# paninski-lab/deepgraphpose

Hardware: AMD Instinct MI355X
Metric: frames_per_sec (higher is better)
Workload: dtype f32

## Files before the change

deepgraphpose_amd/_lib.py:

```python
from __future__ import annotations

import ctypes as C
import os

_HERE = os.path.dirname(os.path.abspath(__file__))
LIB_PATH = os.environ.get("DGP_HIP_LIB") or os.path.join(_HERE, "libdgp_hip.so")


class DgpNetDesc(C.Structure):
    _fields_ = [("depth", C.c_int32), ("num_joints", C.c_int32), ("in_h", C.c_int32), ("in_w", C.c_int32),
                ("max_batch", C.c_int32), ("with_locref", C.c_int32), ("mean_pixel", C.c_float * 3),
                ("bn_eps", C.c_float)]


class DgpTensorView(C.Structure):
    _fields_ = [("name", C.c_char_p), ("data", C.POINTER(C.c_float)), ("ndim", C.c_int32),
                ("shape", C.c_int64 * 4)]


class DgpLossDesc(C.Structure):
    _fields_ = [(n, C.c_int32) for n in ("nt", "H", "W", "nj", "nl", "n_visible", "n_hidden", "gm2", "gm3",
                                          "gauss_len", "huber")] + \
               [(n, C.c_float) for n in ("gamma", "lengthscale", "stride", "wn_visible", "wn_hidden",
                                         "locref_loss_weight", "n_frames_total", "n_visible_frames_total")] + \
               [(n, C.c_int32) for n in ("use_wt", "Hin", "Win")] + [("wt_max", C.c_float)]


class DgpFlowParams(C.Structure):
    _fields_ = [("pyr_scale", C.c_double), ("levels", C.c_int32), ("winsize", C.c_int32), ("iterations", C.c_int32),
                ("poly_n", C.c_int32), ("poly_sigma", C.c_double), ("flags", C.c_int32)]


class DgpConvDesc(C.Structure):
    _fields_ = [(n, C.c_int32) for n in (
        "N", "H", "W", "Cin", "Cout", "KH", "KW", "stride", "rate", "pad_t", "pad_l", "Ho", "Wo", "relu",
        "res_stride", "res_H", "res_W")]


_vp, _i32, _f32, _sz = C.c_void_p, C.c_int32, C.c_float, C.c_size_t
SYMBOLS = {
    "dgp_version": (C.c_int, []),
    "dgp_tuning_build": (C.c_int, []),
    "dgp_crc32c": (C.c_uint32, [C.c_void_p, C.c_size_t, C.c_uint32]),
    "dgp_last_error": (C.c_char_p, []),
    "dgp_net_create": (C.c_int, [C.POINTER(DgpNetDesc), C.POINTER(_vp)]),
    "dgp_net_destroy": (None, [_vp]),
    "dgp_net_set_input_size": (C.c_int, [_vp, _i32, _i32]),
    "dgp_dlc_loss_fwd_bwd": (C.c_int, [_vp, _vp, _vp, _vp, _vp, _vp, _i32, _i32, _i32, _i32, C.c_float, _i32, _vp, _vp, _vp,
                                       _vp, _sz, _vp]),
    "dgp_net_load_weights": (C.c_int, [_vp, C.POINTER(DgpTensorView), _i32]),
    "dgp_net_workspace_bytes": (C.c_int, [_vp, _i32, C.POINTER(_sz)]),
    "dgp_net_output_dims": (C.c_int, [_vp] + [C.POINTER(_i32)] * 4),
    "dgp_net_stats": (C.c_int, [_vp, _i32, C.POINTER(_i32), C.POINTER(C.c_double)]),
    "dgp_forward": (C.c_int, [_vp, _vp, _i32, _vp, _sz, _vp, _vp, _vp, _vp]),
    "dgp_soft_argmax": (C.c_int, [_vp, _i32, _i32, _i32, _i32, _f32, _i32, _vp, _vp, _vp, _vp, _vp]),
    "dgp_soft_argmax_locref": (C.c_int, [_vp, _vp, _i32, _i32, _i32, _i32, _f32, _i32, _vp, _vp, _vp, _vp, _vp, _vp]),
    "dgp_hard_argmax": (C.c_int, [_vp, _vp, _i32, _i32, _i32, _i32, _vp, _vp, _vp, _vp]),
    "dgp_pmap_threshold": (C.c_int, [_vp, _i32, _i32, _i32, _i32, _f32, _vp, _vp]),
    "dgp_infer": (C.c_int, [_vp, _vp, _i32, _vp, _sz, _f32, _i32, _vp, _vp, _vp, _vp, _vp]),
    "dgp_infer_packed": (C.c_int, [_vp, _vp, _i32, _vp, _sz, _f32, _i32, _vp, _vp, _vp]),
    "dgp_infer_packed_locref": (C.c_int, [_vp, _vp, _i32, _vp, _sz, _f32, _i32, _i32, _vp, _vp, _vp, _vp]),
    "dgp_net_profile_begin": (C.c_int, [_vp, _i32]),
    "dgp_net_profile_end": (C.c_int, [_vp, C.POINTER(_i32), C.POINTER(_i32)]),
    "dgp_net_profile_launch": (C.c_int, [_vp, _i32, C.c_char_p, _i32, C.POINTER(C.c_double), C.POINTER(C.c_double)]),
    "dgp_loss_scratch_bytes": (C.c_int, [C.POINTER(DgpLossDesc), C.POINTER(_sz)]),
    "dgp_loss_fwd_bwd": (C.c_int, [C.POINTER(DgpLossDesc)] + [_vp] * 18 + [_sz, _vp]),
    "dgp_trainer_create": (C.c_int, [_vp, C.POINTER(_vp)]),
    "dgp_trainer_destroy": (None, [_vp]),
    "dgp_trainer_num_tensors": (C.c_int, [_vp, C.POINTER(_i32), C.POINTER(C.c_int64), C.POINTER(C.c_int64)]),
    "dgp_trainer_tensor_info": (C.c_int, [_vp, _i32, C.c_char_p, _i32, C.POINTER(C.c_int64), C.POINTER(C.c_int64),
                                          C.POINTER(_i32)]),
    "dgp_trainer_buffer": (_vp, [_vp, _i32]),
    "dgp_trainer_upload": (C.c_int, [_vp, _i32, C.c_int64, _vp, C.c_int64]),
    "dgp_trainer_download": (C.c_int, [_vp, _i32, C.c_int64, _vp, C.c_int64]),
    "dgp_trainer_workspace_bytes": (C.c_int, [_vp, _i32, C.POINTER(_sz)]),
    "dgp_trainer_sync_weights": (C.c_int, [_vp, _vp]),
    "dgp_train_forward": (C.c_int, [_vp, _vp, _i32, _vp, _sz, C.POINTER(_vp), C.POINTER(_vp), _vp]),
    "dgp_train_backward": (C.c_int, [_vp, _i32, _vp, _sz, _vp, _vp, _vp]),
    "dgp_sgd_momentum_clip": (C.c_int, [_vp, _f32, _f32, _f32, C.POINTER(_f32), _vp]),
    "dgp_adam_clip": (C.c_int, [_vp, _f32, _f32, _f32, _f32, _f32, C.POINTER(_f32), _vp]),
    "dgp_packed_weight_floats": (_sz, [_i32, _i32, _i32, _i32]),
    "dgp_pack_conv_weights": (C.c_int, [_vp, _i32, _i32, _i32, _i32, _vp]),
    "dgp_conv2d": (C.c_int, [C.POINTER(DgpConvDesc), _vp, _vp, _vp, _vp, _vp, _vp, _vp]),
    "dgp_conv2d_ranged": (C.c_int, [C.POINTER(DgpConvDesc), _vp, _vp, _vp, _vp, _vp, _vp, _vp, _vp, _vp, _vp]),
    "dgp_tensor_absmax": (C.c_int, [_vp, _sz, _vp, _vp]),
    "dgp_f32_to_h2": (C.c_int, [_vp, _sz, _i32, _vp, _vp]),
    "dgp_h2_to_f32": (C.c_int, [_vp, _sz, _i32, _vp, _vp]),
    "dgp_conv2d_h2": (C.c_int, [C.POINTER(DgpConvDesc), _vp, _i32, _vp, _vp, _vp, _vp, _vp, _i32, _i32, _vp, _i32, _i32, _vp, _vp, _vp]),
    "dgp_net_set_tier": (C.c_int, [_vp, _i32]),
    "dgp_net_get_tier": (C.c_int, [_vp]),
    "dgp_f32_to_h1": (C.c_int, [_vp, _sz, _i32, _vp, _vp]),
    "dgp_h1_to_f32": (C.c_int, [_vp, _sz, _i32, _vp, _vp]),
    "dgp_conv2d_h1": (C.c_int, [C.POINTER(DgpConvDesc), _vp, _i32, _vp, _vp, _vp, _vp, _vp, _i32, _vp, _i32, _i32, _vp, _vp, _vp]),
    "dgp_chain_h2": (C.c_int, [_i32] * 9 + [_vp, _i32, _vp, _i32] + [_vp] * 6 + [_vp, _i32, _vp, _i32, _vp, _vp, _vp]),
    "dgp_unit_h2": (C.c_int, [_i32] * 7 + [_vp, _i32, _vp, _i32] + [_vp] * 3 + [_i32] + [_vp] * 6 + [_vp, _i32, _vp, _i32, _vp, _vp, _vp, _vp]),
    "dgp_chain_h1": (C.c_int, [_i32] * 9 + [_vp, _i32, _vp, _i32] + [_vp] * 6 + [_vp, _i32, _vp, _i32, _vp, _vp, _vp]),
    "dgp_unit_h1": (C.c_int, [_i32] * 7 + [_vp, _i32, _vp, _i32] + [_vp] * 3 + [_i32] + [_vp] * 6 + [_vp, _i32, _vp, _i32, _vp, _vp, _vp, _vp]),
    "dgp_net_range_status": (C.c_int, [_vp, C.POINTER(_i32), C.POINTER(_i32), _vp]),
    "dgp_net_recalibrate": (C.c_int, [_vp]),
    "dgp_net_reset_scales": (C.c_int, [_vp]),
    "dgp_net_copy_scales": (C.c_int, [_vp, _vp, _vp]),
    "dgp_net_widen": (C.c_int, [_vp]),
    "dgp_conv2d_wgrad": (C.c_int, [C.POINTER(DgpConvDesc), _vp, _vp, _vp, _vp, _vp, _vp, _vp]),
    "dgp_conv2d_wgrad_shadow": (C.c_int, [C.POINTER(DgpConvDesc), _vp, _vp, _vp, _vp, _vp, _vp, _vp, _vp, _vp, _vp]),
    "dgp_trainer_set_tier": (C.c_int, [_vp, C.c_int32]),
    "dgp_trainer_get_tier": (C.c_int, [_vp]),
    "dgp_trainer_grad_groups": (C.c_int, [_vp, C.c_int32, C.POINTER(C.c_int32), C.POINTER(C.c_int64), C.POINTER(C.c_int64)]),
    "dgp_trainer_grad_group_wait": (C.c_int, [_vp, C.c_int32, _vp]),
    "dgp_trainer_step_status": (C.c_int, [_vp, _vp, C.c_int32, C.POINTER(C.c_float), C.POINTER(C.c_float), C.POINTER(C.c_int32),
                                               C.POINTER(C.c_int32), _vp]),
    "dgp_trainer_fast_mode": (C.c_int, [_vp, C.c_int32]),
    "dgp_trainer_fast_status": (C.c_int, [_vp, C.POINTER(C.c_int32), C.POINTER(C.c_int32)]),
    "dgp_conv2d_dgrad_scratch_bytes": (_sz, [C.POINTER(DgpConvDesc)]),
    "dgp_conv2d_dgrad": (C.c_int, [C.POINTER(DgpConvDesc), _vp, _vp, _vp, _vp, _vp, _i32, _vp, _vp, _i32, _vp]),
    "dgp_motion_energy": (C.c_int, [_vp, C.c_int64, C.c_int32, _vp, _vp, _vp]),
    "dgp_maxpool_3x3s2_same": (C.c_int, [_vp, _i32, _i32, _i32, _i32, _vp, _vp]),
    "dgp_preprocess_u8": (C.c_int, [_vp, C.c_int64, C.POINTER(_f32), _vp, _vp]),
    "dgp_optical_flow_scratch_bytes": (C.c_int, [_i32, _i32, _i32, C.POINTER(DgpFlowParams), C.POINTER(_sz), C.POINTER(_i32)]),
    "dgp_optical_flow": (C.c_int, [_vp, _i32, _i32, _i32, C.POINTER(DgpFlowParams), _vp, _vp, _vp, _sz, _vp]),
    "dgp_resize_plan_size": (C.c_int, [_i32, _i32, C.POINTER(_i32)]),
    "dgp_resize_plan": (C.c_int, [_i32, _i32, _vp, _vp]),
    "dgp_resize_crop_u8": (C.c_int, [_vp, _i32, _i32, _i32, _i32, _i32, C.POINTER(_i32), _vp, _vp, _vp, _i32, _i32, _vp]),
    "dgp_resize_plan_size_f": (C.c_int, [_i32, _i32, _i32, C.POINTER(_i32)]),
    "dgp_resize_plan_f": (C.c_int, [_i32, _i32, _i32, _vp, _vp]),
    "dgp_window_resize_u8": (C.c_int, [_vp, _i32, _i32, _i32, _i32, _i32, _i32, _i32, _i32, _i32, _i32, _vp, _vp, _vp, _i32, _i32, _vp]),
    "dgp_target_maps": (C.c_int, [_vp, _vp, _vp, _vp, _i32, _i32, _i32, _i32, C.c_double, C.c_double, C.c_double, C.c_double, _i32,
                                  _vp, _vp, _vp, _vp, _vp]),
    "dgp_gather_frames_u8": (C.c_int, [_vp, C.c_int64, C.c_int64, _vp, _i32, _vp, _i32, C.c_int64, _vp, _vp]),
    "dgp_aug_affine_u8": (C.c_int, [_vp, _vp, _i32, _i32, C.POINTER(C.c_double), _vp]),
    "dgp_aug_blur3_u8": (C.c_int, [_vp, _vp, _i32, _i32, C.POINTER(_f32), _vp]),
    "dgp_aug_dropout_u8": (C.c_int, [_vp, _vp, _i32, _i32, _vp, _i32, _i32, _vp]),
    "dgp_aug_elastic_u8": (C.c_int, [_vp, _vp, _i32, _i32, _vp, _i32, _i32, _vp]),
    "dgp_aug_noise_u8": (C.c_int, [_vp, _vp, _i32, _i32, _f32, _i32, C.c_uint64, _vp]),
}

_lib = None


class DgpError(RuntimeError):
    pass


def load():
    global _lib
    if _lib is not None:
        return _lib
    if not os.path.exists(LIB_PATH):
        raise DgpError(
            "libdgp_hip.so not found at %s -- build it with `python -m deepgraphpose_amd.build` "
            "(hipcc --offload-arch=gfx950); deepgraphpose_amd has no CPU fallback" % LIB_PATH)
    try:
        import torch
    except ImportError:
        pass
    lib = C.CDLL(LIB_PATH)
    for name, (res, args) in SYMBOLS.items():
        fn = getattr(lib, name)
        fn.restype = res
        fn.argtypes = args
    _lib = lib
    return lib


def check(rc: int, what: str = ""):
    if rc != 0:
        msg = load().dgp_last_error()
        raise DgpError("%s failed (%d): %s" % (what or "dgp call", rc, (msg or b"").decode()))
```

deepgraphpose_amd/arch.py:

```python
from __future__ import annotations

import math
from dataclasses import dataclass
from typing import List, Tuple

BLOCKS = {
    50: [(64, 3, 2), (128, 4, 2), (256, 6, 2), (512, 3, 1)],
    101: [(64, 3, 2), (128, 4, 2), (256, 23, 2), (512, 3, 1)],
    152: [(64, 3, 2), (128, 8, 2), (256, 36, 2), (512, 3, 1)],
}

MEAN_PIXEL = (123.68, 116.779, 103.939)
BN_EPS = 1e-5


@dataclass
class UnitPlan:
    scope: str
    depth_in: int
    depth: int
    depth_bottleneck: int
    stride: int
    rate: int
    has_shortcut_conv: bool


def resnet_units(depth: int = 50, output_stride: int = 16) -> List[UnitPlan]:
    if depth not in BLOCKS:
        raise ValueError("unsupported resnet depth %r" % (depth,))
    name = "resnet_v1_%d" % depth
    target = output_stride // 4
    current_stride, rate = 1, 1
    units: List[UnitPlan] = []
    depth_in = 64
    for bi, (base, n_units, block_stride) in enumerate(BLOCKS[depth], start=1):
        for ui in range(1, n_units + 1):
            s = block_stride if ui == n_units else 1
            d_out = base * 4
            if current_stride == target:
                unit_stride, unit_rate = 1, rate
                rate *= s
            else:
                unit_stride, unit_rate = s, 1
                current_stride *= s
            units.append(UnitPlan(
                scope="%s/block%d/unit_%d/bottleneck_v1" % (name, bi, ui),
                depth_in=depth_in, depth=d_out, depth_bottleneck=base,
                stride=unit_stride, rate=unit_rate,
                has_shortcut_conv=(depth_in != d_out)))
            depth_in = d_out
    return units


def same_out(n: int, s: int) -> int:
    return -(-n // s)


def feature_hw(h: int, w: int, depth: int = 50) -> Tuple[int, int]:
    for _ in range(4):
        h, w = same_out(h, 2), same_out(w, 2)
    return h, w


def scoremap_hw(h: int, w: int, deconv_stride: int = 2) -> Tuple[int, int]:
    fh, fw = feature_hw(h, w)
    return fh * deconv_stride, fw * deconv_stride


def conv_macs_per_frame(h: int, w: int, depth: int = 50, nj: int = 4,
                        with_locref: bool = False) -> int:
    h1, w1 = same_out(h, 2), same_out(w, 2)
    macs = h1 * w1 * 7 * 7 * 3 * 64
    hh, ww = same_out(h1, 2), same_out(w1, 2)
    for u in resnet_units(depth):
        ho, wo = same_out(hh, u.stride), same_out(ww, u.stride)
        if u.has_shortcut_conv:
            macs += ho * wo * u.depth_in * u.depth
        macs += hh * ww * u.depth_in * u.depth_bottleneck
        macs += ho * wo * 9 * u.depth_bottleneck * u.depth_bottleneck
        macs += ho * wo * u.depth_bottleneck * u.depth
        hh, ww = ho, wo
    heads = nj * (3 if with_locref else 1)
    macs += hh * ww * 9 * 2048 * heads
    return macs


def launch_algorithmic_bytes(name: str, h: int, w: int, depth: int = 50, batch: int = 1, elem_bytes: float = 4.0) -> float:
    body = name.split("|")[0]
    if not body.startswith("conv:"):
        return 0.0
    if body.endswith("/conv1+pool"):
        h1, w1 = same_out(h, 2), same_out(w, 2)
        return float(batch * h * w * 3 + elem_bytes * batch * same_out(h1, 2) * same_out(w1, 2) * 64 + 4 * 7 * 7 * 3 * 64)
    toks = body[5:].split("+")
    units = {u.scope: (i, u) for i, u in enumerate(resnet_units(depth))}
    plan = resnet_units(depth)
    h1, w1 = same_out(h, 2), same_out(w, 2)
    hh, ww = same_out(h1, 2), same_out(w1, 2)
    geo = []
    for u in plan:
        ho, wo = same_out(hh, u.stride), same_out(ww, u.stride)
        geo.append((batch * hh * ww, batch * ho * wo))
        hh, ww = ho, wo
    convs = []
    for t in toks:
        if t == "shortcut":
            convs.append((convs[-1][0], "shortcut"))
            continue
        scope, _, which = t.rpartition("/")
        if scope not in units:
            return 0.0
        convs.append((units[scope][0], which))
    have = set(convs)
    total = 0.0
    for ui, which in convs:
        u = plan[ui]
        pin, pout = geo[ui]
        if which == "conv1":
            total += u.depth_in * u.depth_bottleneck
            total += pin * u.depth_bottleneck
            if (ui - 1, "conv3") not in have:
                total += pin * u.depth_in
        elif which == "conv2":
            total += 9 * u.depth_bottleneck * u.depth_bottleneck
            total += pin * u.depth_bottleneck
            if (ui, "conv3") not in have:
                total += pout * u.depth_bottleneck
        elif which == "conv3":
            total += u.depth_bottleneck * u.depth + pout * u.depth
            if (ui, "conv2") not in have:
                total += pout * u.depth_bottleneck
            if (ui, "shortcut") in have:
                total += pin * u.depth_in
            elif u.has_shortcut_conv:
                total += pout * u.depth
            else:
                total += (pin if u.stride == 1 else pout) * u.depth
        elif which == "shortcut":
            total += u.depth_in * u.depth
            if (ui, "conv3") not in have:
                total += pin * u.depth_in + pout * u.depth
    return elem_bytes * total


def conv_algorithmic_bytes(h: int, w: int, depth: int = 50, batch: int = 1) -> dict:
    name = "resnet_v1_%d" % depth
    out = {}
    h1, w1 = same_out(h, 2), same_out(w, 2)
    out["conv:%s/conv1" % name] = 4.0 * (batch * h * w * 4 + batch * h1 * w1 * 64 + 7 * 7 * 4 * 64)
    hh, ww = same_out(h1, 2), same_out(w1, 2)
    for u in resnet_units(depth):
        ho, wo = same_out(hh, u.stride), same_out(ww, u.stride)
        pin, pout = batch * hh * ww, batch * ho * wo
        if u.has_shortcut_conv:
            out["conv:%s/shortcut" % u.scope] = 4.0 * (pin * u.depth_in + pout * u.depth + u.depth_in * u.depth)
        out["conv:%s/conv1" % u.scope] = 4.0 * (pin * u.depth_in + pin * u.depth_bottleneck + u.depth_in * u.depth_bottleneck)
        out["conv:%s/conv2" % u.scope] = 4.0 * (pin * u.depth_bottleneck + pout * u.depth_bottleneck +
                                                9 * u.depth_bottleneck * u.depth_bottleneck)
        res = pout * u.depth if u.has_shortcut_conv else (pin if u.stride == 1 else pout) * u.depth
        out["conv:%s/conv3" % u.scope] = 4.0 * (pout * u.depth_bottleneck + pout * u.depth + res + u.depth_bottleneck * u.depth)
        hh, ww = ho, wo
    return out
```

deepgraphpose_amd/csrc/dgp_chain.hip:

```cpp
#include "dgp_internal.h"
#include "dgp_device.h"

#include <cstdio>
#include <cstdlib>
#include <type_traits>

namespace dgp {

typedef float floatx4 __attribute__((ext_vector_type(4)));
typedef __attribute__((address_space(3))) void lds_void;

__device__ __forceinline__ floatx4 mma16(const uint4& a, const uint4& b, floatx4 c) {
    return __builtin_amdgcn_mfma_f32_16x16x32_f16(__builtin_bit_cast(half8, a), __builtin_bit_cast(half8, b), c, 0, 0, 0);
}
__device__ __forceinline__ uint4 ld16nt(__amdgpu_buffer_rsrc_t r, unsigned voff, int soff) {
    return __builtin_bit_cast(uint4, __builtin_amdgcn_raw_buffer_load_b128(r, (int)voff, soff, 2));
}
__device__ __forceinline__ void st16nt(__amdgpu_buffer_rsrc_t r, const uint4& v, unsigned voff, int soff) {
    __builtin_amdgcn_raw_buffer_store_b128(__builtin_bit_cast(u32x4, v), r, (int)voff, soff, 2);
}
__device__ __forceinline__ uint4 ld16(__amdgpu_buffer_rsrc_t r, unsigned voff, int soff) {
    return __builtin_bit_cast(uint4, __builtin_amdgcn_raw_buffer_load_b128(r, (int)voff, soff, 0));
}
__device__ __forceinline__ void st16(__amdgpu_buffer_rsrc_t r, const uint4& v, unsigned voff, int soff) {
    __builtin_amdgcn_raw_buffer_store_b128(__builtin_bit_cast(u32x4, v), r, (int)voff, soff, 0);
}

#ifdef DGP_DIAG
__device__ unsigned long long g_unit_diag[16];
#define UD_STAMP(x)                                                                     \
    do {                                                                                \
        __builtin_amdgcn_sched_barrier(0);                                              \
        asm volatile("s_memtime %0\n\ts_waitcnt lgkmcnt(0)" : "=s"(x)::"memory");       \
        __builtin_amdgcn_sched_barrier(0);                                              \
    } while (0)
#define UD_PARAM , unsigned long long (&ud)[12]
#define UD_ARG , ud
#else
#define UD_STAMP(x)
#define UD_PARAM
#define UD_ARG
#endif

template <int RES, int RB, bool H1 = false>
__device__ __forceinline__ void chain_fetch_res(const ChainArgs& p, uint4 (&res)[RB][2], const unsigned (&roff)[RB],
                                                const __amdgpu_buffer_rsrc_t rs_s2, int jp) {
    if constexpr (RES != 0) {
#pragma unroll
        for (int rb = 0; rb < RB; ++rb) {
            if constexpr (H1) {
                res[rb][0] = (p.nt & 1) ? ld16nt(rs_s2, roff[rb], jp * 64) : ld16(rs_s2, roff[rb], jp * 64);
            } else if (p.nt & 1) {
                res[rb][0] = ld16nt(rs_s2, roff[rb], jp * 128);
                res[rb][1] = ld16nt(rs_s2, roff[rb], jp * 128 + 16);
            } else {
                res[rb][0] = ld16(rs_s2, roff[rb], jp * 128);
                res[rb][1] = ld16(rs_s2, roff[rb], jp * 128 + 16);
            }
        }
    }
}
template <int RES, int RB, int PD, bool H1 = false>
__device__ __forceinline__ void chain_prefetch(const ChainArgs& p, uint4 (&res)[PD][RB][2], const unsigned (&roff)[RB],
                                               const __amdgpu_buffer_rsrc_t rs_s2) {
#pragma unroll
    for (int u = 0; u < PD - 1; ++u) chain_fetch_res<RES, RB, H1>(p, res[u], roff, rs_s2, u);
}

template <int C, int C1, int CIN2, int RES, int RB, int NS, int PD, int CHUNK, int WR, bool H1 = false>
__device__ __forceinline__ void chain_tail(const ChainArgs& p, const uint4* ring, int& slot, const uint4 (&ph)[RB][(C + CIN2) / 32],
                                           const uint4 (&pl)[RB][(C + CIN2) / 32], const unsigned (&xoff)[RB], const unsigned (&roff)[RB],
                                           const unsigned (&r1off)[RB], const __amdgpu_buffer_rsrc_t rs_s2, const __amdgpu_buffer_rsrc_t rs_xo,
                                           const __amdgpu_buffer_rsrc_t rs_r1, float& amax_x, float& amax_r1, const int lane,
                                           uint4 (&res)[PD][RB][2] UD_PARAM) {
#ifdef DGP_DIAG
    unsigned long long c0 = 0, c1 = 0, c2 = 0, c3 = 0, c4 = 0;
#endif
    constexpr int C4 = 4 * C, KS1 = (C + CIN2) / 32, NJP = C4 / 32, NCB = C1 / 16;
    constexpr int PL = H1 ? 1 : 2;
    constexpr int F1 = KS1 * 2 * PL, F2 = NCB * PL;
    static_assert(WR >= 2 && WR % 2 == 0, "weight fragments in flight: pairs share the ring");
    static_assert(NJP % PD == 0 && PD >= 2, "chunk loop is unrolled PD times");
    const int g = lane >> 4;
    floatx4 a2[RB][NCB];
#pragma unroll
    for (int rb = 0; rb < RB; ++rb)
#pragma unroll
        for (int cb = 0; cb < NCB; ++cb) a2[rb][cb] = floatx4{0.f, 0.f, 0.f, 0.f};
    auto fetch_res = [&](int jp, int buf) { chain_fetch_res<RES, RB, H1>(p, res[buf], roff, rs_s2, jp); };
    constexpr int CB = H1 ? 64 : 128;
    for (int jp0 = 0; jp0 < NJP; jp0 += PD) {
#pragma unroll
        for (int u = 0; u < PD; ++u) {
            const int jp = jp0 + u;
            if (jp + PD - 1 < NJP) fetch_res(jp + PD - 1, (u + PD - 1) % PD);
            UD_STAMP(c0);
            const uint4* Wc = ring + slot * (CHUNK / 16);
            const uint4* W = Wc + lane;
            floatx4 a1[RB][2];
#pragma unroll
            for (int rb = 0; rb < RB; ++rb) { a1[rb][0] = floatx4{0.f, 0.f, 0.f, 0.f}; a1[rb][1] = floatx4{0.f, 0.f, 0.f, 0.f}; }
            uint4 wq[WR];
#pragma unroll
            for (int f = 0; f < WR && f < F1 + F2; ++f) wq[f] = W[f * 64];
            __builtin_amdgcn_sched_barrier(0);
#pragma unroll
            for (int s = 0; s < KS1; ++s)
#pragma unroll
                for (int b = 0; b < 2; ++b) {
                    const int f0 = (s * 2 + b) * PL;
                    const uint4 wh = wq[f0 % WR], wl = wq[(f0 + PL - 1) % WR];
                    if constexpr (!H1) {
#pragma unroll
                    for (int rb = 0; rb < RB; ++rb) a1[rb][b] = mma16(wl, ph[rb][s], a1[rb][b]);
#pragma unroll
                    for (int rb = 0; rb < RB; ++rb) a1[rb][b] = mma16(wh, pl[rb][s], a1[rb][b]);
                    }
#pragma unroll
                    for (int rb = 0; rb < RB; ++rb) a1[rb][b] = mma16(wh, ph[rb][s], a1[rb][b]);
                    __builtin_amdgcn_sched_barrier(0);
                    if (f0 + WR < F1 + F2) wq[f0 % WR] = W[(f0 + WR) * 64];
                    if (PL == 2 && f0 + 1 + WR < F1 + F2) wq[(f0 + 1) % WR] = W[(f0 + 1 + WR) * 64];
                    __builtin_amdgcn_sched_barrier(0);
                }
            UD_STAMP(c1);
            const float4 sa = __builtin_bit_cast(float4, Wc[(F1 + F2) * 64 + 2 * g]), sb = __builtin_bit_cast(float4, Wc[(F1 + F2) * 64 + 2 * g + 1]);
            const float4 ba = __builtin_bit_cast(float4, Wc[(F1 + F2) * 64 + 8 + 2 * g]), bb = __builtin_bit_cast(float4, Wc[(F1 + F2) * 64 + 8 + 2 * g + 1]);
            const float sc[8] = {sa.x * p.post1, sa.y * p.post1, sa.z * p.post1, sa.w * p.post1,
                                 sb.x * p.post1, sb.y * p.post1, sb.z * p.post1, sb.w * p.post1};
            const float bi[8] = {ba.x, ba.y, ba.z, ba.w, bb.x, bb.y, bb.z, bb.w};
            uint4 xh[RB], xl[RB];
#pragma unroll
            for (int rb = 0; rb < RB; ++rb) {
                float o[8], r[8] = {0.f, 0.f, 0.f, 0.f, 0.f, 0.f, 0.f, 0.f};
                if constexpr (RES != 0) {
                    if constexpr (H1) h1_unpack8(res[u][rb][0], p.res_inv_scale, r);
                    else h2_unpack8(res[u][rb][0], res[u][rb][1], p.res_inv_scale, r);
                }
#pragma unroll
                for (int k = 0; k < 8; ++k) {
                    o[k] = a1[rb][k >> 2][k & 3] * sc[k] + bi[k] + r[k];
                    o[k] = fmaxf(o[k], 0.f);
                }
                if constexpr (H1) { xh[rb] = h1_pack8(o, p.xout_scale); xl[rb] = xh[rb]; }
                else h2_pack8(o, p.xout_scale, xh[rb], xl[rb]);
                if (p.nt & 2) {
                    st16nt(rs_xo, xh[rb], xoff[rb], jp * CB);
                    if constexpr (!H1) st16nt(rs_xo, xl[rb], xoff[rb], jp * CB + 16);
                } else {
                    st16(rs_xo, xh[rb], xoff[rb], jp * CB);
                    if constexpr (!H1) st16(rs_xo, xl[rb], xoff[rb], jp * CB + 16);
                }
                if (xoff[rb] != OOB) {
#pragma unroll
                    for (int k = 0; k < 8; ++k) amax_x = fmaxf(amax_x, o[k]);
                }
            }
            UD_STAMP(c2);
            __builtin_amdgcn_sched_barrier(0);
#pragma unroll
            for (int cb = 0; cb < NCB; ++cb) {
                const int f0 = F1 + cb * PL;
                const uint4 wh = wq[f0 % WR], wl = wq[(f0 + PL - 1) % WR];
                if constexpr (!H1) {
#pragma unroll
                for (int rb = 0; rb < RB; ++rb) a2[rb][cb] = mma16(wl, xh[rb], a2[rb][cb]);
#pragma unroll
                for (int rb = 0; rb < RB; ++rb) a2[rb][cb] = mma16(wh, xl[rb], a2[rb][cb]);
                }
#pragma unroll
                for (int rb = 0; rb < RB; ++rb) a2[rb][cb] = mma16(wh, xh[rb], a2[rb][cb]);
                __builtin_amdgcn_sched_barrier(0);
                if (f0 + WR < F1 + F2) wq[f0 % WR] = W[(f0 + WR) * 64];
                if (PL == 2 && f0 + 1 + WR < F1 + F2) wq[(f0 + 1) % WR] = W[(f0 + 1 + WR) * 64];
                __builtin_amdgcn_sched_barrier(0);
            }
            slot = slot + 1 == NS ? 0 : slot + 1;
            UD_STAMP(c3);
            asm volatile("s_waitcnt lgkmcnt(0)" ::: "memory");
            __builtin_amdgcn_s_barrier();
            UD_STAMP(c4);
#ifdef DGP_DIAG
            ud[4] += c1 - c0; ud[5] += c2 - c1; ud[6] += c3 - c2; ud[7] += c4 - c3;
#endif
        }
    }
    UD_STAMP(c0);
#pragma unroll
    for (int q = 0; q < NCB / 2; ++q) {
        const float4 s0 = *reinterpret_cast<const float4*>(p.sc1 + 32 * q + 8 * g), s1 = *reinterpret_cast<const float4*>(p.sc1 + 32 * q + 8 * g + 4);
        const float4 b0 = *reinterpret_cast<const float4*>(p.bi1 + 32 * q + 8 * g), b1 = *reinterpret_cast<const float4*>(p.bi1 + 32 * q + 8 * g + 4);
        const float sc[8] = {s0.x * p.post2, s0.y * p.post2, s0.z * p.post2, s0.w * p.post2,
                             s1.x * p.post2, s1.y * p.post2, s1.z * p.post2, s1.w * p.post2};
        const float bi[8] = {b0.x, b0.y, b0.z, b0.w, b1.x, b1.y, b1.z, b1.w};
#pragma unroll
        for (int rb = 0; rb < RB; ++rb) {
            float o[8];
#pragma unroll
            for (int k = 0; k < 8; ++k) o[k] = fmaxf(a2[rb][2 * q + (k >> 2)][k & 3] * sc[k] + bi[k], 0.f);
            if constexpr (H1) {
                st16(rs_r1, h1_pack8(o, p.r1_scale), r1off[rb], q * CB);
            } else {
            uint4 hi, lo;
            h2_pack8(o, p.r1_scale, hi, lo);
            st16(rs_r1, hi, r1off[rb], q * 128);
            st16(rs_r1, lo, r1off[rb], q * 128 + 16);
            }
            if (r1off[rb] != OOB) {
#pragma unroll
                for (int k = 0; k < 8; ++k) amax_r1 = fmaxf(amax_r1, o[k]);
            }
        }
    }
    UD_STAMP(c1);
#ifdef DGP_DIAG
    ud[8] += c1 - c0;
#endif
}

template <int C, int C1, int CIN2, int RES, int RB, int NCW, int NLW, int NS, int PD, int WR, bool H1 = false>
__global__ __launch_bounds__(64 * (NCW + NLW)) void chain_kernel(const ChainArgs p) {
    constexpr int C4 = 4 * C;
    constexpr int EB = H1 ? 2 : 4;
    constexpr int KSA = C / 32, KSB = CIN2 / 32, KS1 = KSA + KSB;
    constexpr int NJP = C4 / 32;
    constexpr int NCB = C1 / 16;
    constexpr int PL = H1 ? 1 : 2;
    constexpr int F1 = KS1 * 2 * PL, F2 = NCB * PL, NF = F1 + F2 + 1;
    constexpr int CHUNK = NF * 1024;
    constexpr int TILE = 16 * RB * NCW;
    static_assert(NJP % PD == 0 && PD >= 2, "chunk loop is unrolled PD times");
    static_assert(RES == 0 || CIN2 == 0, "residual or K-concatenated shortcut, not both");
    static_assert(NS == 2 || NS == 3, "ring protocols of the loader below");
    extern __shared__ __attribute__((aligned(16))) char smem[];
    const int lane = threadIdx.x & 63;
    const int wave = __builtin_amdgcn_readfirstlane(threadIdx.x >> 6);
    const int my_tiles = (p.ntiles - (int)blockIdx.x + (int)gridDim.x - 1) / (int)gridDim.x;
    const int total = my_tiles * NJP;

    if (wave >= NCW) {
        const int lw = wave - NCW;
        const __amdgpu_buffer_rsrc_t rs_w = __builtin_amdgcn_make_buffer_rsrc(const_cast<void*>(p.wfrag), 0, (int)p.w_bytes, 0x00020000);
        int jp = 0, slot = 0;
        auto run = [&](auto niw) {
            constexpr int NIW = decltype(niw)::value;
            auto issue = [&]() {
                char* dst = smem + slot * CHUNK;
                const int gbase = jp * CHUNK;
#pragma unroll
                for (int i = 0; i < NIW; ++i) {
                    const int f = lw + i * NLW;
                    __builtin_amdgcn_raw_ptr_buffer_load_lds(rs_w, (lds_void*)(dst + f * 1024), 16, lane * 16, gbase + f * 1024, 0, 0);
                }
                jp = jp + 1 == NJP ? 0 : jp + 1;
                slot = slot + 1 == NS ? 0 : slot + 1;
            };
            if constexpr (NS == 3) {
                if (total > 0) issue();
                if (total > 1) { issue(); asm volatile("s_waitcnt vmcnt(%0)" ::"n"(NIW) : "memory"); }
                else asm volatile("s_waitcnt vmcnt(0)" ::: "memory");
                __builtin_amdgcn_s_barrier();
                for (int it = 0; it < total; ++it) {
                    if (it + 2 < total) { issue(); asm volatile("s_waitcnt vmcnt(%0)" ::"n"(NIW) : "memory"); }
                    else asm volatile("s_waitcnt vmcnt(0)" ::: "memory");
                    __builtin_amdgcn_s_barrier();
                }
            } else {
                if (total > 0) issue();
                asm volatile("s_waitcnt vmcnt(0)" ::: "memory");
                __builtin_amdgcn_s_barrier();
                for (int it = 0; it < total; ++it) {
                    if (it + 1 < total) issue();
                    asm volatile("s_waitcnt vmcnt(0)" ::: "memory");
                    __builtin_amdgcn_s_barrier();
                }
            }
        };
        constexpr int NI_HI = (NF + NLW - 1) / NLW, NI_LO = NF / NLW;
        if (lw < NF % NLW || NI_HI == NI_LO) run(std::integral_constant<int, NI_HI>());
        else run(std::integral_constant<int, NI_LO>());
        return;
    }

    const int l15 = lane & 15, g = lane >> 4;
    const __amdgpu_buffer_rsrc_t rs_r2 = __builtin_amdgcn_make_buffer_rsrc(const_cast<void*>(p.r2), 0, (int)p.r2_bytes, 0x00020000);
    const __amdgpu_buffer_rsrc_t rs_s2 = __builtin_amdgcn_make_buffer_rsrc(const_cast<void*>(p.src2 ? p.src2 : p.r2), 0,
                                                                            p.src2 ? (int)p.src2_bytes : 0, 0x00020000);
    const __amdgpu_buffer_rsrc_t rs_xo = __builtin_amdgcn_make_buffer_rsrc(p.xout, 0, (int)p.xout_bytes, 0x00020000);
    const __amdgpu_buffer_rsrc_t rs_r1 = __builtin_amdgcn_make_buffer_rsrc(p.r1out, 0, (int)p.r1_bytes, 0x00020000);
    const uint4* ring = reinterpret_cast<const uint4*>(smem);
    int slot = 0;
    float amax_x = 0.f, amax_r1 = 0.f;
    __builtin_amdgcn_s_barrier();
    for (int t = blockIdx.x; t < p.ntiles; t += gridDim.x) {
        unsigned xoff[RB], roff[RB], r1off[RB];
        uint4 ph[RB][KS1], pl[RB][KS1];
#pragma unroll
        for (int rb = 0; rb < RB; ++rb) {
            const int m = t * TILE + (wave * RB + rb) * 16 + l15;
            const bool ok = m < p.M;
            xoff[rb] = ok ? (unsigned)m * (unsigned)(C4 * EB) + (unsigned)(g * 8 * EB) : OOB;
            r1off[rb] = ok ? (unsigned)m * (unsigned)(C1 * EB) + (unsigned)(g * 8 * EB) : OOB;
            if (RES == 2) {
                const int n = m / p.HoWo, rem = m - n * p.HoWo, ho = rem / p.Wo, wo = rem - ho * p.Wo;
                roff[rb] = ok ? (unsigned)((n * p.res_H + 2 * ho) * p.res_W + 2 * wo) * (unsigned)(C4 * EB) + (unsigned)(g * 8 * EB) : OOB;
            } else roff[rb] = xoff[rb];
            const unsigned aoff = ok ? (unsigned)m * (unsigned)(C * EB) + (unsigned)(g * 8 * EB) : OOB;
#pragma unroll
            for (int s = 0; s < KSA; ++s) {
                ph[rb][s] = ld16(rs_r2, aoff, s * 32 * EB);
                if constexpr (H1) pl[rb][s] = ph[rb][s]; else pl[rb][s] = ld16(rs_r2, aoff, s * 128 + 16);
            }
            if constexpr (KSB > 0) {
                const unsigned boff = ok ? (unsigned)m * (unsigned)(CIN2 * EB) + (unsigned)(g * 8 * EB) : OOB;
#pragma unroll
                for (int s = 0; s < KSB; ++s) {
                    ph[rb][KSA + s] = ld16(rs_s2, boff, s * 32 * EB);
                    if constexpr (H1) pl[rb][KSA + s] = ph[rb][KSA + s]; else pl[rb][KSA + s] = ld16(rs_s2, boff, s * 128 + 16);
                }
            }
        }
        uint4 res[PD][RB][2];
        chain_prefetch<RES, RB, PD, H1>(p, res, roff, rs_s2);
#ifdef DGP_DIAG
        unsigned long long ud[12] = {0};
#endif
        chain_tail<C, C1, CIN2, RES, RB, NS, PD, CHUNK, WR, H1>(p, ring, slot, ph, pl, xoff, roff, r1off, rs_s2, rs_xo, rs_r1, amax_x, amax_r1, lane, res UD_ARG);
#ifdef DGP_DIAG
        if (wave == 0 && lane == 0) {
            for (int i = 4; i < 9; ++i) atomicAdd(&g_unit_diag[i], ud[i]);
            atomicAdd(&g_unit_diag[9], 1ull);
        }
#endif
    }
    if (p.xout_absmax) track_absmax(p.xout_absmax, amax_x, lane, (int)(blockIdx.x * 8u + (unsigned)wave));
    if (p.r1_absmax) track_absmax(p.r1_absmax, amax_r1, lane, (int)(blockIdx.x * 8u + (unsigned)wave) + 97);
}

template <int C, int C1, int CIN2, int RES, int NCW, int NLW, int PD, int WR, int HWV = 1, bool H1 = false>
__global__ __launch_bounds__(64 * (NCW + NLW + HWV)) void unit_kernel(const ChainArgs p) {
    constexpr int NS = 3;
    constexpr int TH = NCW, TW = 16, HW = TW + 2, HPIX = (TH + 2) * HW;
    constexpr int EB = H1 ? 2 : 4;
    constexpr int PIXB = C * EB;
    constexpr int PPI = 1024 / PIXB;
    static_assert(C == 64, "one pixel of R1 = 16 (H1: 8) slots of 16 bytes (the bank swizzle)");
    constexpr int NHI = (HPIX * PIXB + 1023) / 1024;
    constexpr int HALO_BYTES = NHI * 1024;
    static_assert(NLW == 1 || NLW == 2 || NLW == 4, "one, two or four weight-loader waves");
    static_assert(HWV == 0 || HWV == 1, "at most one halo wave");
    constexpr int NHW = HWV ? 1 : NLW;
    constexpr int C4 = 4 * C, KS1 = (C + CIN2) / 32, NJP = C4 / 32, NCB = C1 / 16;
    constexpr int PL = H1 ? 1 : 2;
    constexpr int NFJ = (KS1 * 2 + NCB) * PL + 1;
    constexpr int KS2 = C / 32, NCB2 = C / 16, NF2 = KS2 * NCB2 * PL + 1;
    constexpr int NFMAX = NFJ > NF2 ? NFJ : NF2, CHUNK = NFMAX * 1024;
    constexpr int STEPS = 9 + NJP;
    constexpr int HSTEPS = HWV ? NJP - 1 : NJP;
    constexpr int HPP = (NHI + HSTEPS - 1) / HSTEPS;
    extern __shared__ __attribute__((aligned(16))) char smem[];
    char* halo = smem;
    char* ringb = smem + HALO_BYTES;
    const int lane = threadIdx.x & 63;
    const int wave = __builtin_amdgcn_readfirstlane(threadIdx.x >> 6);
    const int G = (int)gridDim.x, b = (int)blockIdx.x;
    const int vwg = (G & 7) == 0 ? (b & 7) * (G >> 3) + (b >> 3) : b;
    const int my_tiles = vwg < p.ntiles ? (p.ntiles - vwg + G - 1) / G : 0;
    const int total = my_tiles * STEPS;
    const int tpf = p.TY * p.TX;

    if (wave >= NCW) {
        auto halo_issue = [&](int tile, int i0, int i1, int hl) {
            const __amdgpu_buffer_rsrc_t rs_in = __builtin_amdgcn_make_buffer_rsrc(const_cast<void*>(p.r1in), 0, (int)p.r1in_bytes, 0x00020000);
            const int f = tile / tpf, rem = tile - f * tpf, ty = rem / p.TX, tx = rem - ty * p.TX;
            for (int i = i0 + hl; i < i1; i += NHW) {
                const int hp = PPI * i + (H1 ? (lane >> 3) : (lane >> 4));
                const int hy = (hp * 57) >> 10, hx = hp - HW * hy;
                const int gy = ty * TH - 1 + hy, gx = tx * TW - 1 + hx;
                const bool ok = hp < HPIX && (unsigned)gy < (unsigned)p.H && (unsigned)gx < (unsigned)p.W;
                const unsigned cell = H1 ? (unsigned)((lane & 7) ^ ((hp >> 1) & 7)) : (unsigned)((lane & 15) ^ (hp & 15));
                const unsigned off = ok ? (unsigned)((f * p.H + gy) * p.W + gx) * (unsigned)PIXB + (cell << 4) : OOB;
                __builtin_amdgcn_raw_ptr_buffer_load_lds(rs_in, (lds_void*)(halo + i * 1024), 16, (int)off, 0, 0, 0);
            }
        };
        auto halo_step = [&](int cur_st, int tile, int hl) {
            if (cur_st >= 9 && tile + G < p.ntiles) {
                const int i0 = (cur_st - 9) * HPP, i1 = i0 + HPP < NHI ? i0 + HPP : NHI;
                halo_issue(tile + G, i0, i1, hl);
            }
        };
        const int lw_rt = wave - NCW;
        if (HWV && lw_rt == NLW) {
            if (total > 0) halo_issue(vwg, 0, NHI, 0);
            asm volatile("s_waitcnt vmcnt(0)" ::: "memory");
            __builtin_amdgcn_s_barrier();
            int cur_st = 0, tile = vwg;
            for (int it = 0; it < total; ++it) {
                halo_step(cur_st, tile, 0);
                if (cur_st == STEPS - 1) asm volatile("s_waitcnt vmcnt(0)" ::: "memory");
                __builtin_amdgcn_s_barrier();
                if (++cur_st == STEPS) { cur_st = 0; tile += G; }
            }
            return;
        }
        auto loader = [&](auto lw_c) {
        constexpr int lw = decltype(lw_c)::value;
        const __amdgpu_buffer_rsrc_t rs_w = __builtin_amdgcn_make_buffer_rsrc(const_cast<void*>(p.wfrag), 0, (int)p.w_bytes, 0x00020000);
        int st = 0, slot = 0;
        constexpr int N2 = lw < NF2 % NLW ? (NF2 + NLW - 1) / NLW : NF2 / NLW, NJ = lw < NFJ % NLW ? (NFJ + NLW - 1) / NLW : NFJ / NLW;
        auto issue = [&]() {
            char* dst = ringb + slot * CHUNK;
            const int st2 = st, stj = st - 9;
            if (st < 9) {
#pragma unroll
                for (int k = 0; k < N2; ++k)
                    __builtin_amdgcn_raw_ptr_buffer_load_lds(rs_w, (lds_void*)(dst + (lw + k * NLW) * 1024), 16, lane * 16, st2 * (NF2 * 1024) + (lw + k * NLW) * 1024, 0, 0);
            } else {
#pragma unroll
                for (int k = 0; k < NJ; ++k)
                    __builtin_amdgcn_raw_ptr_buffer_load_lds(rs_w, (lds_void*)(dst + (lw + k * NLW) * 1024), 16, lane * 16,
                                                             9 * (NF2 * 1024) + stj * (NFJ * 1024) + (lw + k * NLW) * 1024, 0, 0);
            }
            const bool was_conv2 = st < 9;
            st = st + 1 == STEPS ? 0 : st + 1;
            slot = slot + 1 == NS ? 0 : slot + 1;
            return was_conv2;
        };
        auto wait_all_but_newest = [&](bool conv2_chunk) {
            if (conv2_chunk) asm volatile("s_waitcnt vmcnt(%0)" ::"n"(N2) : "memory");
            else asm volatile("s_waitcnt vmcnt(%0)" ::"n"(NJ) : "memory");
        };
        if (total > 0) {
            if (!HWV) halo_issue(vwg, 0, NHI, lw);
            issue();
            wait_all_but_newest(issue());
        }
        __builtin_amdgcn_s_barrier();
        int cur_st = 0, tile = vwg;
#ifdef DGP_DIAG
        unsigned long long l0 = 0, l1 = 0, l2 = 0, l3 = 0, ul[3] = {0, 0, 0}, ul3 = 0;
#endif
        for (int it = 0; it < total; ++it) {
            UD_STAMP(l0);
            if (!HWV) halo_step(cur_st, tile, lw);
#ifdef DGP_DIAG
            bool c2_ = false;
            if (it + 2 < total) c2_ = issue();
            UD_STAMP(l1);
            if (it + 2 < total) wait_all_but_newest(c2_);
            else asm volatile("s_waitcnt vmcnt(0)" ::: "memory");
            UD_STAMP(l2);
#else
            if (it + 2 < total) wait_all_but_newest(issue());
            else asm volatile("s_waitcnt vmcnt(0)" ::: "memory");
#endif
            __builtin_amdgcn_s_barrier();
            UD_STAMP(l3);
#ifdef DGP_DIAG
            if (cur_st < 9) ul[0] += l1 - l0; else ul3 += l1 - l0;
            ul[1] += l2 - l1; ul[2] += l3 - l2;
#endif
            if (++cur_st == STEPS) { cur_st = 0; tile += G; }
        }
#ifdef DGP_DIAG
        if (lw == 0 && lane == 0) {
            atomicAdd(&g_unit_diag[12], ul[0]); atomicAdd(&g_unit_diag[13], ul[1]); atomicAdd(&g_unit_diag[14], ul[2]); atomicAdd(&g_unit_diag[11], ul3);
            atomicAdd(&g_unit_diag[15], (unsigned long long)total);
        }
#endif
        };
        if (lw_rt == 0) loader(std::integral_constant<int, 0>());
        else if (NLW > 1 && lw_rt == 1) loader(std::integral_constant<int, (NLW > 1 ? 1 : 0)>());
        else if (NLW > 2 && lw_rt == 2) loader(std::integral_constant<int, (NLW > 2 ? 2 : 0)>());
        else if (NLW > 3) loader(std::integral_constant<int, (NLW > 3 ? 3 : 0)>());
        return;
    }

    const int l15 = lane & 15, g = lane >> 4;
    const __amdgpu_buffer_rsrc_t rs_s2 = __builtin_amdgcn_make_buffer_rsrc(const_cast<void*>(p.src2), 0, (int)p.src2_bytes, 0x00020000);
    const __amdgpu_buffer_rsrc_t rs_xo = __builtin_amdgcn_make_buffer_rsrc(p.xout, 0, (int)p.xout_bytes, 0x00020000);
    const __amdgpu_buffer_rsrc_t rs_r1 = __builtin_amdgcn_make_buffer_rsrc(p.r1out, 0, (int)p.r1_bytes, 0x00020000);
    const uint4* ring = reinterpret_cast<const uint4*>(ringb);
    int slot = 0;
    float amax_x = 0.f, amax_r1 = 0.f, amax_r2 = 0.f;
    __builtin_amdgcn_s_barrier();
#ifdef DGP_DIAG
    unsigned long long ud[12] = {0}, u0 = 0, u1 = 0, u2 = 0, ubeg = 0, uend = 0;
    UD_STAMP(ubeg);
#endif
    for (int tile = vwg; tile < p.ntiles; tile += G) {
        UD_STAMP(u0);
        const int f = tile / tpf, rem = tile - f * tpf, ty = rem / p.TX, tx = rem - ty * p.TX;
        const int y = ty * TH + wave, x = tx * TW + l15;
        const bool ok = y < p.H && x < p.W;
        const int m = (f * p.H + y) * p.W + x;
        unsigned xoff[1], roff[1], r1off[1];
        xoff[0] = ok ? (unsigned)m * (unsigned)(C4 * EB) + (unsigned)(g * 8 * EB) : OOB;
        roff[0] = xoff[0];
        r1off[0] = ok ? (unsigned)m * (unsigned)(C1 * EB) + (unsigned)(g * 8 * EB) : OOB;
        uint4 ph[1][KS1], pl[1][KS1];
        if constexpr (CIN2 > 0) {
            const unsigned boff = ok ? (unsigned)m * (unsigned)(CIN2 * EB) + (unsigned)(g * 8 * EB) : OOB;
#pragma unroll
            for (int s = 0; s < CIN2 / 32; ++s) {
                ph[0][KS2 + s] = ld16(rs_s2, boff, s * 32 * EB);
                if constexpr (H1) pl[0][KS2 + s] = ph[0][KS2 + s]; else pl[0][KS2 + s] = ld16(rs_s2, boff, s * 128 + 16);
            }
        }
        uint4 res[PD][1][2];
        chain_prefetch<RES, 1, PD, H1>(p, res, roff, rs_s2);
        floatx4 acc[NCB2];
#pragma unroll
        for (int cb = 0; cb < NCB2; ++cb) acc[cb] = floatx4{0.f, 0.f, 0.f, 0.f};
        uint4 aff[KS2][4];
        UD_STAMP(u1);
#ifdef DGP_DIAG
        ud[3] += u1 - u0;
#endif
#pragma unroll
        for (int t = 0; t < 9; ++t) {
            UD_STAMP(u0);
            const uint4* Wc = ring + slot * (CHUNK / 16);
            const uint4* W = Wc + lane;
            const int hp = (wave + t / 3) * HW + l15 + t % 3;
            const char* hrow = halo + hp * PIXB;
            const int sw = H1 ? ((hp >> 1) & 7) : (hp & 15);
            uint4 ah[KS2], al[KS2];
#pragma unroll
            for (int ks = 0; ks < KS2; ++ks) {
                if constexpr (H1) {
                    ah[ks] = *reinterpret_cast<const uint4*>(hrow + (((4 * ks + g) ^ sw) << 4));
                    al[ks] = ah[ks];
                } else {
                const int sl = 2 * (4 * ks + g);
                ah[ks] = *reinterpret_cast<const uint4*>(hrow + ((sl ^ sw) << 4));
                al[ks] = *reinterpret_cast<const uint4*>(hrow + (((sl + 1) ^ sw) << 4));
                }
            }
            constexpr int NW2 = KS2 * NCB2 * PL;
            uint4 wq[WR];
#pragma unroll
            for (int f = 0; f < WR && f < NW2; ++f) wq[f] = W[f * 64];
            __builtin_amdgcn_sched_barrier(0);
#pragma unroll
            for (int ks = 0; ks < KS2; ++ks) {
#pragma unroll
                for (int cb = 0; cb < NCB2; ++cb) {
                    const int f0 = (ks * NCB2 + cb) * PL;
                    const uint4 wh = wq[f0 % WR], wl = wq[(f0 + PL - 1) % WR];
                    if constexpr (!H1) {
                    acc[cb] = mma16(wl, ah[ks], acc[cb]);
                    acc[cb] = mma16(wh, al[ks], acc[cb]);
                    }
                    acc[cb] = mma16(wh, ah[ks], acc[cb]);
                    __builtin_amdgcn_sched_barrier(0);
                    if (f0 + WR < NW2) wq[f0 % WR] = W[(f0 + WR) * 64];
                    if (PL == 2 && f0 + 1 + WR < NW2) wq[(f0 + 1) % WR] = W[(f0 + 1 + WR) * 64];
                    __builtin_amdgcn_sched_barrier(0);
                }
            }
            if (t == 8) {
#pragma unroll
                for (int q = 0; q < KS2; ++q) {
                    aff[q][0] = Wc[(NF2 - 1) * 64 + 8 * q + 2 * g]; aff[q][1] = Wc[(NF2 - 1) * 64 + 8 * q + 2 * g + 1];
                    aff[q][2] = Wc[(NF2 - 1) * 64 + 16 + 8 * q + 2 * g]; aff[q][3] = Wc[(NF2 - 1) * 64 + 16 + 8 * q + 2 * g + 1];
                }
            }
            slot = slot + 1 == NS ? 0 : slot + 1;
            UD_STAMP(u1);
            asm volatile("s_waitcnt lgkmcnt(0)" ::: "memory");
            __builtin_amdgcn_s_barrier();
            UD_STAMP(u2);
#ifdef DGP_DIAG
            ud[0] += u1 - u0; ud[1] += u2 - u1;
#endif
        }
        UD_STAMP(u0);
#pragma unroll
        for (int q = 0; q < KS2; ++q) {
            const float4 sa = __builtin_bit_cast(float4, aff[q][0]), sb = __builtin_bit_cast(float4, aff[q][1]);
            const float4 ba = __builtin_bit_cast(float4, aff[q][2]), bb = __builtin_bit_cast(float4, aff[q][3]);
            const float sc[8] = {sa.x * p.post0, sa.y * p.post0, sa.z * p.post0, sa.w * p.post0, sb.x * p.post0, sb.y * p.post0, sb.z * p.post0, sb.w * p.post0};
            const float bi[8] = {ba.x, ba.y, ba.z, ba.w, bb.x, bb.y, bb.z, bb.w};
            float o[8];
#pragma unroll
            for (int k = 0; k < 8; ++k) o[k] = fmaxf(acc[2 * q + (k >> 2)][k & 3] * sc[k] + bi[k], 0.f);
            if constexpr (H1) { ph[0][q] = h1_pack8(o, p.r2_scale); pl[0][q] = ph[0][q]; }
            else h2_pack8(o, p.r2_scale, ph[0][q], pl[0][q]);
            if (ok) {
#pragma unroll
                for (int k = 0; k < 8; ++k) amax_r2 = fmaxf(amax_r2, o[k]);
            }
        }
        UD_STAMP(u1);
#ifdef DGP_DIAG
        ud[2] += u1 - u0; ud[9] += 1;
#endif
        chain_tail<C, C1, CIN2, RES, 1, NS, PD, CHUNK, WR, H1>(p, ring, slot, ph, pl, xoff, roff, r1off, rs_s2, rs_xo, rs_r1, amax_x, amax_r1, lane, res UD_ARG);
    }
#ifdef DGP_DIAG
    UD_STAMP(uend);
    ud[10] = uend - ubeg;
    if (wave == 0 && lane == 0)
        for (int i = 0; i < 11; ++i) atomicAdd(&g_unit_diag[i], ud[i]);
#endif
    if (p.xout_absmax) track_absmax(p.xout_absmax, amax_x, lane, (int)(blockIdx.x * 8u + (unsigned)wave));
    if (p.r1_absmax) track_absmax(p.r1_absmax, amax_r1, lane, (int)(blockIdx.x * 8u + (unsigned)wave) + 97);
    if (p.r2_absmax) track_absmax(p.r2_absmax, amax_r2, lane, (int)(blockIdx.x * 8u + (unsigned)wave) + 41);
}

__global__ __launch_bounds__(256) void chain_pack_kernel(const float4* __restrict__ src, int n_chunks, int f1_pairs, int f2_pairs,
                                                         float s1, float s2, uint4* __restrict__ out, int planes) {
    const int pairs = f1_pairs + f2_pairs;
    const int nf = planes * pairs + 1;
    const long long src_chunk = (long long)pairs * 128 + 64;
    const long long total = (long long)n_chunks * (pairs + 1) * 64;
    for (long long i = (long long)blockIdx.x * blockDim.x + threadIdx.x; i < total; i += (long long)gridDim.x * blockDim.x) {
        const int ln = (int)(i & 63);
        const long long fp = i >> 6;
        const int ch = (int)(fp / (pairs + 1)), pr = (int)(fp % (pairs + 1));
        uint4* o = out + ((long long)ch * nf + planes * pr) * 64 + ln;
        if (pr == pairs) {
            o[0] = __builtin_bit_cast(uint4, src[ch * src_chunk + (long long)pairs * 128 + ln]);
            continue;
        }
        const float4* sp = src + ch * src_chunk + (long long)pr * 128 + ln * 2;
        uint2 h0, l0, h1, l1;
        const float sc = pr < f1_pairs ? s1 : s2;
        split2_f16(sp[0], sc, h0, l0);
        split2_f16(sp[1], sc, h1, l1);
        o[0] = make_uint4(h0.x, h0.y, h1.x, h1.y);
        if (planes == 2) o[64] = make_uint4(l0.x, l0.y, l1.x, l1.y);
    }
}

hipError_t launch_chain_pack(const float* src, int n_chunks, int f1_pairs, int f2_pairs, float s1, float s2, void* out, hipStream_t s, int planes) {
    const long long total = (long long)n_chunks * (f1_pairs + f2_pairs + 1) * 64;
    long long blocks = (total + 255) / 256;
    if (blocks > 4096) blocks = 4096;
    hipLaunchKernelGGL(chain_pack_kernel, dim3((unsigned)blocks), dim3(256), 0, s, reinterpret_cast<const float4*>(src), n_chunks, f1_pairs,
                       f2_pairs, s1, s2, reinterpret_cast<uint4*>(out), planes);
    return hipGetLastError();
}

namespace {

template <int C, int C1, int CIN2, int RES, int RB, int NCW, int NLW, int PD, int NS = 3, int WR = 4, bool H1 = false>
hipError_t launch_chain_t(const ChainArgs& a0, hipStream_t s) {
    constexpr int NF = ((C + CIN2) / 32 * 2 + C1 / 16) * (H1 ? 1 : 2) + 1;
    constexpr int LDS = NS * NF * 1024;
    static_assert(LDS <= 160 * 1024, "ring does not fit the LDS");
    auto kern = chain_kernel<C, C1, CIN2, RES, RB, NCW, NLW, NS, PD, WR, H1>;
    static bool attr_done[16] = {};
    static int wgs_per_cu[16] = {};
    const int dev = dgp_device_slot();
    if (!attr_done[dev]) {
        hipError_t e = hipFuncSetAttribute(reinterpret_cast<const void*>(kern), hipFuncAttributeMaxDynamicSharedMemorySize, LDS);
        if (e != hipSuccess) return e;
        int occ = 0;
        e = hipOccupancyMaxActiveBlocksPerMultiprocessor(&occ, kern, 64 * (NCW + NLW), LDS);
        if (e != hipSuccess) return e;
        static const int force = dgp_tune("DGP_CHAIN_WGS", 0);
        wgs_per_cu[dev] = force > 0 ? force : (occ < 1 ? 1 : occ);
        attr_done[dev] = true;
    }
    ChainArgs a = a0;
    static const int nt_env = dgp_tune("DGP_CHAIN_NT", 0);
    a.nt = nt_env;
    constexpr int TILE = 16 * RB * NCW;
    a.ntiles = (a.M + TILE - 1) / TILE;
    int ncu = 256;
    (void)hipDeviceGetAttribute(&ncu, hipDeviceAttributeMultiprocessorCount, dev);
    int grid = ncu * wgs_per_cu[dev];
    if (grid > a.ntiles) grid = a.ntiles;
    if (grid < 1) return hipSuccess;
#ifdef DGP_DIAG
    unsigned long long hz[16] = {0};
    (void)hipMemcpyToSymbol(HIP_SYMBOL(g_unit_diag), hz, sizeof(hz));
#endif
    hipLaunchKernelGGL(kern, dim3((unsigned)grid), dim3(64 * (NCW + NLW)), LDS, s, a);
#ifdef DGP_DIAG
    (void)hipStreamSynchronize(s);
    (void)hipMemcpyFromSymbol(hz, HIP_SYMBOL(g_unit_diag), sizeof(hz));
    const double nt = (double)hz[9] > 0 ? (double)hz[9] : 1.0, ns = (double)hz[15] > 0 ? (double)hz[15] : 1.0;
    printf("[diag chain C %d C1 %d CIN2 %d] grid %d tiles %d (%.1f per workgroup) | compute wave 0, cycles per TILE: prologue %.0f | conv2: 9 x (work %.0f + barrier %.0f) "
           "epilogue %.0f | chain: %d x (conv3 %.0f + epilogue %.0f + conv1 %.0f + barrier %.0f) conv1 epilogue %.0f | tile loop %.0f per tile | "
           "loader wave 0, cycles per STEP: issue %.0f (conv2 steps) / %.0f (pointwise steps), vmcnt wait %.0f, barrier %.0f\n", C, C1, CIN2, grid, a.ntiles, (double)a.ntiles / grid,
           hz[3] / nt, hz[0] / nt / 9.0, hz[1] / nt / 9.0, hz[2] / nt, 4 * C / 32, hz[4] / nt / (4 * C / 32), hz[5] / nt / (4 * C / 32), hz[6] / nt / (4 * C / 32),
           hz[7] / nt / (4 * C / 32), hz[8] / nt, hz[10] * (double)grid / nt / grid, hz[12] / (ns * 9.0 / (9.0 + 4 * C / 32)), hz[11] / (ns * (4 * C / 32) / (9.0 + 4 * C / 32)), hz[13] / ns, hz[14] / ns);
#endif
    return hipGetLastError();
}

template <int C, int C1, int CIN2, int RES, int NCW, int NLW, int PD, int WR = 4, int HWV = 1, bool H1 = false>
hipError_t launch_unit_t(const ChainArgs& a0, int N, hipStream_t s) {
    constexpr int NFJ = ((C + CIN2) / 32 * 2 + C1 / 16) * (H1 ? 1 : 2) + 1, NF2 = (C / 32) * (C / 16) * (H1 ? 1 : 2) + 1, NFMAX = NFJ > NF2 ? NFJ : NF2;
    constexpr int LDS = ((NCW + 2) * 18 * C * (H1 ? 2 : 4) + 1023) / 1024 * 1024 + 3 * NFMAX * 1024;
    static_assert(LDS <= 160 * 1024, "halo tile + ring do not fit the LDS");
    auto kern = unit_kernel<C, C1, CIN2, RES, NCW, NLW, PD, WR, HWV, H1>;
    static bool attr_done[16] = {};
    static int wgs_per_cu[16] = {};
    const int dev = dgp_device_slot();
    if (!attr_done[dev]) {
        hipError_t e = hipFuncSetAttribute(reinterpret_cast<const void*>(kern), hipFuncAttributeMaxDynamicSharedMemorySize, LDS);
        if (e != hipSuccess) return e;
        int occ = 0;
        e = hipOccupancyMaxActiveBlocksPerMultiprocessor(&occ, kern, 64 * (NCW + NLW + HWV), LDS);
        if (e != hipSuccess) return e;
        static const int force = dgp_tune("DGP_CHAIN_WGS", 0);
        wgs_per_cu[dev] = force > 0 ? force : (occ < 1 ? 1 : occ);
        attr_done[dev] = true;
    }
    ChainArgs a = a0;
    static const int nt_env = dgp_tune("DGP_CHAIN_NT", 0);
    a.nt = nt_env;
    a.TY = (a.H + NCW - 1) / NCW; a.TX = (a.W + 15) / 16;
    a.ntiles = N * a.TY * a.TX;
    int ncu = 256;
    (void)hipDeviceGetAttribute(&ncu, hipDeviceAttributeMultiprocessorCount, dev);
    int grid = ncu * wgs_per_cu[dev];
    if (grid > a.ntiles) grid = a.ntiles;
    if (grid < 1) return hipSuccess;
#ifdef DGP_DIAG
    unsigned long long hz[16] = {0};
    (void)hipMemcpyToSymbol(HIP_SYMBOL(g_unit_diag), hz, sizeof(hz));
#endif
    hipLaunchKernelGGL(kern, dim3((unsigned)grid), dim3(64 * (NCW + NLW + HWV)), LDS, s, a);
#ifdef DGP_DIAG
    (void)hipStreamSynchronize(s);
    (void)hipMemcpyFromSymbol(hz, HIP_SYMBOL(g_unit_diag), sizeof(hz));
    const double nt = (double)hz[9] > 0 ? (double)hz[9] : 1.0, ns = (double)hz[15] > 0 ? (double)hz[15] : 1.0;
    printf("[diag unit  C %d C1 %d CIN2 %d] grid %d tiles %d (%.1f per workgroup) | compute wave 0, cycles per TILE: prologue %.0f | conv2: 9 x (work %.0f + barrier %.0f) "
           "epilogue %.0f | chain: %d x (conv3 %.0f + epilogue %.0f + conv1 %.0f + barrier %.0f) conv1 epilogue %.0f | tile loop %.0f per tile | "
           "loader wave 0, cycles per STEP: issue %.0f (conv2 steps) / %.0f (pointwise steps), vmcnt wait %.0f, barrier %.0f\n", C, C1, CIN2, grid, a.ntiles, (double)a.ntiles / grid,
           hz[3] / nt, hz[0] / nt / 9.0, hz[1] / nt / 9.0, hz[2] / nt, 4 * C / 32, hz[4] / nt / (4 * C / 32), hz[5] / nt / (4 * C / 32), hz[6] / nt / (4 * C / 32),
           hz[7] / nt / (4 * C / 32), hz[8] / nt, hz[10] * (double)grid / nt / grid, hz[12] / (ns * 9.0 / (9.0 + 4 * C / 32)), hz[11] / (ns * (4 * C / 32) / (9.0 + 4 * C / 32)), hz[13] / ns, hz[14] / ns);
#endif
    return hipGetLastError();
}

}

bool chain_supported(int C, int C1, int CIN2, int res) {
    if (C == 64 && C1 == 64 && CIN2 == 0 && res == 1) return true;
    if (C == 64 && C1 == 64 && CIN2 == 64 && res == 0) return true;
    if (C == 64 && C1 == 128 && CIN2 == 0 && res == 2) return true;
    if (C == 128 && C1 == 128 && CIN2 == 0 && res == 1) return true;
    if (C == 128 && C1 == 256 && CIN2 == 0 && res == 2) return true;
    if (C == 256 && C1 == 256 && CIN2 == 0 && res == 1) return true;
    return false;
}
// ... 82 lines not shown
```

deepgraphpose_amd/csrc/dgp_internal.h:

```cpp
#pragma once
#include <hip/hip_runtime.h>
#include <stdint.h>
#include <stddef.h>
#include <stdlib.h>
#include <string.h>

namespace dgp {

constexpr int BK = 32;

struct ConvArgs {
    const float* in;
    const float* wpk;
    const float* scale;
    const float* bias;
    const float* res;
    const float* mask;
    float*       out;
    int N, H, W, Cin, log2cin4;
    int Ho, Wo, Cout, CoutP;
    int KH, KW, stride, dil, pad_t, pad_l;
    int ntaps, nk;
    int M;
    int res_s, res_H, res_W;
    int ksplit;
    long long split_stride;
    int up;
    int relu;
    int out_mode;
    int dc_nj;
    int mtiles, ntiles;
    int tap_minor;
    int stem;
    int tap_rows;
    float* slab;
    unsigned slab_bytes;
    int n_main, tail_ksplit;
    int epi_nt;
    int st_gn, st_mc, st_mb;
    const float* in2;
    const float* in2_absmax;
    unsigned in2_bytes;
    int cin_split;
    unsigned long long* dbg;
    unsigned in_bytes, w_bytes, res_bytes, out_bytes;
    const float* in_absmax;
    const float* w_absmax;
    const void*  wh3;
    unsigned     wh3_bytes;
    float*       out_absmax;
    int   in_fmt, out_fmt, res_fmt;
    float in_scale;
    float out_scale;
    float res_inv_scale;
    float*       shadow;
    const float* shadow_prev;
    int          shadow_fmt;
    const float* in_scale_dev;
    const float* out_scale_dev;
    const float* res_scale_dev;
    int mask_fmt;
};

constexpr int ABSMAX_SLOTS = 256;

enum TileCfg { TILE_128x128 = 0, TILE_128x64 = 1, TILE_64x64 = 2, TILE_128x32 = 3, TILE_128x128_W8 = 4, TILE_128x128_LS = 5, TILE_128x64_LS = 6, TILE_128x128_S6 = 7, TILE_128x128_S3 = 8, TILE_128x64_S6 = 9, TILE_128x128_S6K16 = 10, TILE_128x128_S3K16 = 11, TILE_128x128_S6K16W8 = 12, TILE_128x128_H3K16 = 13, TILE_128x128_H3K16W8 = 14, TILE_128x64_H3 = 15, TILE_128x128_H3K32 = 16 };

hipError_t launch_conv(const ConvArgs& a, int tile_cfg, hipStream_t s);
int        pick_tile(int M, int CoutP, int K, bool have_absmax = false);
hipError_t launch_pack_h3(const float* panel, int nk, int CoutP, const float* w_absmax, void* out, hipStream_t s);
hipError_t launch_pack_h1(const float* panel, int nk, int CoutP, const float* w_absmax, void* out, hipStream_t s);
hipError_t launch_f32_to_h1(const float* x, long long n_groups8, float scale, void* out, hipStream_t s);
hipError_t launch_h1_to_f32(const void* x, long long n_groups8, float inv_scale, float* out, hipStream_t s);
struct PackH3Desc { const float* panel; int nkg; int CoutP; const float* rng; void* out; };
hipError_t launch_pack_h3_all(const PackH3Desc* table_dev, int n, hipStream_t s);
hipError_t launch_pack_h1_all(const PackH3Desc* table_dev, int n, hipStream_t s);
hipError_t launch_absmax(const float* x, long long n, float* out_slots, hipStream_t s);
const char* conv_kernel_name(const ConvArgs& a, int tile_cfg);
hipError_t launch_reduce_slabs(const float* slabs, long long n, long long stride, int nsplit, float* out, hipStream_t s);
hipError_t launch_head_gather(const float* T, const float* bias, int B, int h, int w, int njt, int ldt, float* out, hipStream_t s);
hipError_t launch_maxpool(const float* x, int N, int H, int W, int C, float* y, hipStream_t s, float h2_scale = 0.f);
hipError_t launch_f32_to_h2(const float* x, long long n_groups8, float scale, void* out, hipStream_t s);
hipError_t launch_h2_to_f32(const void* x, long long n_groups8, float inv_scale, float* out, hipStream_t s);
hipError_t launch_h2_range_check(const float* amax_slots, const int* exps, int n_layers, int* flag, hipStream_t s);
hipError_t launch_stem_pool_fused(const unsigned char* frames, int B, int H, int W, const void* wcells, const float* w_absmax,
                                  const float* bn_scale, const float* bn_bias, float m0, float m1, float m2, float out_scale,
                                  float* out, float* out_absmax, hipStream_t s, int out_h1 = 0, const float* out_prev = nullptr,
                                  unsigned char* idx = nullptr);
hipError_t launch_preprocess(const uint8_t* f, long long npix, float m0, float m1, float m2,
                             float* out, hipStream_t s);
hipError_t launch_motion_energy(const uint8_t* frames, long long frame_bytes, int n_frames, const uint8_t* prev_frame,
                                unsigned long long* sums, hipStream_t s);
constexpr size_t SOFT_ARGMAX_LDS_LIMIT = 150 * 1024;
hipError_t launch_soft_argmax(const float* scmap, int B, int H, int W, int C, float gamma,
                              int gauss_len, float* mu, float* conf, int* idx, float* pmap,
                              hipStream_t s, int record_stride = 0);
hipError_t launch_soft_argmax_locref(const float* scmap, const float* locref, int B, int H, int W, int C, float gamma,
                                     int gauss_len, float* mu, float* conf, int* idx, float* offs, float* pmap,
                                     hipStream_t s, int record_stride = 0);
hipError_t launch_hard_argmax(const float* scmap, const float* locref, int B, int H, int W, int C,
                              int* idx, float* prob, float* offs, hipStream_t s, float* rec = nullptr, int record_stride = 0);
hipError_t launch_pmap_threshold(float* pmap, int B, int H, int W, int C, float th, float* mu, hipStream_t s);

struct LossArgs {
    const float* pred;
    const float* locref_pred;
    const float* mu;
    const float* targets;
    const float* locref_map;
    const float* locref_mask;
    const int* visible_marker; const int* hidden_marker; const int* visible_in_targets;
    const float* S0; const float* ws; const float* ws_max;
    float* dpred; float* dlocref;
    float* losses;
    float* t_all; float* dLdt; int* kind; float* stats; float* norm;
    int nt, H, W, nj, nl, n_v, n_h;
    int gm2, gm3, gauss_len, huber;
    float gamma, lengthscale, stride, hidden_scale, clique_scale, locref_weight;
    const float* vector_field; const float* wt_batch; float* wt_w;
    int use_wt, Hin, Win;
    float wt_max, temporal_scale;
};
constexpr size_t LOSS_LDS_LIMIT = 150 * 1024;
hipError_t launch_loss(const LossArgs& a, hipStream_t s);

struct DlcLossArgs {
    const float *pred, *part_targets, *part_weights;
    const float *locref_pred, *locref_targets, *locref_mask;
    float *dpred, *dlocref, *losses;
    double* acc;
    long long n_part, n_loc;
    float locref_loss_weight;
    int huber;
};
hipError_t launch_dlc_loss(const DlcLossArgs& a, hipStream_t s);

struct ChainArgs {
    const void* r2;
    const void* src2;
    void* xout;
    void* r1out;
    const void* wfrag;
    const float* sc1;
    const float* bi1;
    float post1, post2;
    float res_inv_scale, xout_scale, r1_scale;
    float* xout_absmax; float* r1_absmax;
    int M, HoWo, Wo, res_H, res_W;
    int ntiles;
    unsigned r2_bytes, src2_bytes, xout_bytes, r1_bytes, w_bytes;
    const void* r1in;
    unsigned r1in_bytes;
    int H, W, TY, TX;
    float post0, r2_scale;
    float* r2_absmax;
    int nt;
    int h1;
};
bool chain_supported(int C, int C1, int CIN2, int res);
int  chain_frags_per_chunk(int C, int C1, int CIN2, int planes = 2);
hipError_t launch_chain(const ChainArgs& a, int C, int C1, int CIN2, int res, hipStream_t s);
const char* chain_kernel_name(int C, int C1, int CIN2, int res);
bool unit_supported(int C, int C1, int CIN2, int res);
hipError_t launch_unit(const ChainArgs& a, int N, int C, int C1, int CIN2, int res, hipStream_t s);
hipError_t launch_chain_pack(const float* src, int n_chunks, int f1_pairs, int f2_pairs, float s1, float s2, void* out, hipStream_t s, int planes = 2);

inline int dgp_env(const char* name, int dflt) {
    const char* v = getenv(name);
    return v ? atoi(v) : dflt;
}
inline int dgp_tune(const char* name, int dflt) {
#ifdef DGP_TUNING
    return dgp_env(name, dflt);
#else
    (void)name;
    return dflt;
#endif
}
enum class ConvMode { F16x3, BF16x6, F32, F16, Other };
inline ConvMode conv_mode() {
    static const ConvMode m = [] {
        const char* v = getenv("DGP_CONV_MODE");
        if (!v || !strcmp(v, "f16x3")) return ConvMode::F16x3;
        return !strcmp(v, "bf16x6") ? ConvMode::BF16x6 : !strcmp(v, "f32") ? ConvMode::F32 : !strcmp(v, "f16") ? ConvMode::F16 : ConvMode::Other;
    }();
    return m;
}

inline int dgp_device_slot() { int d = 0; (void)hipGetDevice(&d); return d & 15; }
inline int round_up(int x, int m) { return (x + m - 1) / m * m; }
inline int ilog2(int x) { int l = 0; while ((1 << l) < x) ++l; return l; }

}
```

deepgraphpose_amd/csrc/dgp_net.hip:

```cpp
#include "dgp_engine.h"

using namespace dgp;

static thread_local std::string g_err;
namespace dgp {
int fail(int code, const std::string& msg) {
    g_err = msg;
    return code;
}

int coutp_for(int cout) {
    if (cout <= 32) return 32;
    if (cout <= 64) return 64;
    return round_up(cout, 128);
}
int head_pw_coutp(int cpw) { const int c = coutp_for(cpw); return c < 64 ? 64 : c; }
int nk_for(int kh, int kw, int cin) { return (kh * kw * (cin / 4) + 7) / 8; }

void tf_same(int n, int k, int s, int d, int* out, int* pad_before) {
    const int keff = (k - 1) * d + 1;
    *out = (n + s - 1) / s;
    int total = (*out - 1) * s + keff - n;
    if (total < 0) total = 0;
    *pad_before = total / 2;
// ... 507 lines not shown
    size_t o = 0;
    auto take = [&](size_t nfloats) { size_t r = o; o += align256(nfloats * sizeof(float)); return r; };
    p.off_p0 = take(p0); p.off_c1 = take(c1); p.off_x0 = take(x); p.off_x1 = take(x); p.off_sc = take(sc);
    p.off_r1 = take(r1); p.off_r2 = take(r2);
    p.off_scmap = take((size_t)B * 4 * net->fh * net->fw * d.num_joints);
    p.off_locref = take((size_t)B * 4 * net->fh * net->fw * 2 * d.num_joints);
    p.off_slabs = take((size_t)HEAD_KSPLIT_MAX * B * 4 * net->fh * net->fw * 2 * d.num_joints);
    p.off_tail = take(TAIL_SLAB_FLOATS);
    p.total = o;
    return p;
}

struct ProfScope {
    dgp_net* net; hipStream_t s; int li;
    ProfScope(dgp_net* n, hipStream_t st, const std::string& name, double flops) : net(n), s(st), li(-1) {
        if (!net->prof_on || net->prof_used >= net->prof_slots) return;
        li = net->prof_cursor++;
        if (li >= net->prof_launches) { li = -1; return; }
        if (net->prof_used == 0) { net->prof_names[li] = name; net->prof_flops[li] = flops; }
        (void)hipEventRecord(net->prof_ev[((size_t)net->prof_used * net->prof_launches + li) * 2], s);
    }
    ~ProfScope() {
        if (li >= 0) (void)hipEventRecord(net->prof_ev[((size_t)net->prof_used * net->prof_launches + li) * 2 + 1], s);
    }
};

double conv_flops_of(const ConvLayer& l, int M, bool is_head) {
    if (is_head) return 2.0 * M * 9.0 * l.Cin * (l.Cout / 4);
    const int cin = (l.KH == 7) ? 3 : l.Cin;
    return 2.0 * M * (double)l.KH * l.KW * cin * l.Cout;
}

struct H2Spec { int in_fmt = 0, in_exp = 0, out_fmt = 0, out_exp = 0, res_fmt = 0, res_exp = 0; };

void apply_h2(ConvArgs& a, const H2Spec& h) {
    a.in_fmt = h.in_fmt; a.out_fmt = h.out_fmt; a.res_fmt = h.res_fmt;
    a.in_scale = ldexpf(1.f, h.in_exp); a.out_scale = ldexpf(1.f, h.out_exp); a.res_inv_scale = ldexpf(1.f, -h.res_exp);
}

struct ConvCall {
    const float* in = nullptr;
    int H = 0, W = 0, Ho = 0, Wo = 0, pad_t = 0, pad_l = 0;
    const float* res = nullptr;
    int res_s = 0, res_H = 0, res_W = 0;
    bool relu = true;
    int out_mode = 0, dc_nj = 0;
    float *out = nullptr, *slabs = nullptr;
    const float* in_absmax = nullptr;
    H2Spec h2;
    ConvCall& grid(int ho, int wo, int pt = 0, int pl = 0) { Ho = ho; Wo = wo; pad_t = pt; pad_l = pl; return *this; }
    ConvCall& residual(const float* r, int s, int rH, int rW) { res = r; res_s = s; res_H = rH; res_W = rW; return *this; }
    ConvCall& range(const float* in_rng) { in_absmax = in_rng; return *this; }
    ConvCall& cells(const H2Spec& q) { h2 = q; return *this; }
    ConvCall& linear() { relu = false; return *this; }
};
ConvCall conv_call(const float* in, int H, int W, float* out) {
    ConvCall c;
    c.in = in; c.H = c.Ho = H; c.W = c.Wo = W; c.out = out;
    return c;
}

int run_conv(dgp_net* net, const ConvLayer& l, int N, const ConvCall& c, hipStream_t s) {
    ConvArgs a{};
    const int li = (int)(&l - net->layers.data());
    const float* in_absmax = net->wmax_valid ? c.in_absmax : nullptr;
    apply_h2(a, c.h2);
    const bool ranged = in_absmax || c.h2.in_fmt;
    a.in_absmax = in_absmax; a.w_absmax = ranged ? net->wmax(li) : nullptr;
    a.out_absmax = c.out_mode == 0 ? net->amax(li) : nullptr;
    a.slab = net->tail_slab; a.slab_bytes = net->tail_slab_bytes;
    a.in = c.in; a.wpk = l.d_w; a.scale = l.has_bn ? l.d_scale : nullptr; a.bias = l.d_bias; a.res = c.res; a.out = c.out;
    dgp_conv_desc d{};
    d.N = N; d.H = c.H; d.W = c.W; d.Cin = l.Cin; d.Cout = l.Cout; d.KH = l.KH; d.KW = l.KW; d.stride = l.stride; d.rate = l.rate;
    d.pad_t = c.pad_t; d.pad_l = c.pad_l; d.Ho = c.Ho; d.Wo = c.Wo; d.relu = c.relu; d.res_stride = c.res ? c.res_s : 0; d.res_H = c.res_H; d.res_W = c.res_W;
    if (int rc = fill_conv_geometry(a, d, TOO_BIG)) return rc;
    if (c.out_mode == 0 && (l.Cout & 3)) return fail(DGP_ERR_INVALID, "conv: Cout must be a multiple of 4");
    a.out_mode = c.out_mode; a.dc_nj = c.dc_nj;
    static const bool stem_rows = (dgp_tune("DGP_STEM_ROWS", 1) != 0);
    if (li == net->conv1 && l.d_w_rows && net->wmax_valid && stem_rows && conv_mode() != ConvMode::F32 && l.CoutP % 64 == 0) {
        a.stem = 1; a.tap_rows = 8; a.KH = 7; a.KW = 1; a.ntaps = 7; a.nk = 7; a.wpk = l.d_w_rows;
        a.w_bytes = (unsigned)((size_t)7 * 8 * l.CoutP * 16);
    }
    static const bool use_cells = (dgp_tune("DGP_PRESPLIT_WEIGHTS", 1) != 0);
    if (use_cells && ranged && l.d_wh3 && (li != net->conv1 || a.stem)) { a.wh3 = l.d_wh3; a.wh3_bytes = a.w_bytes; }
    if (c.h2.in_fmt == 2) { a.wh3 = l.d_wh1; a.wh3_bytes = a.w_bytes; }
    const int tile_cfg = pick_tile(a.M, a.CoutP, a.nk * BK, ranged && a.w_absmax);
    ProfScope ps(net, s, "conv:" + l.scope + "|" + conv_kernel_name(a, tile_cfg), conv_flops_of(l, a.M, c.out_mode == 1));
    const long long out_n = (long long)N * 4 * c.Ho * c.Wo * c.dc_nj;
    int ks = 1;
    if (c.out_mode == 1 && c.slabs && (out_n & 3) == 0)
        while (ks < HEAD_KSPLIT_MAX && (a.M + 127) / 128 * ks < 1024 && l.nk % (ks * 2) == 0) ks *= 2;
    if (ks > 1) { a.ksplit = ks; a.split_stride = out_n; a.out = c.slabs; }
    hipError_t e = launch_conv(a, tile_cfg, s);
    if (ks > 1 && e == hipSuccess) e = launch_reduce_slabs(c.slabs, out_n, out_n, ks, c.out, s);
    if (e != hipSuccess) return fail(DGP_ERR_HIP, std::string(ks > 1 ? "head conv (" : "conv launch (") + l.scope + "): " + hipGetErrorString(e));
    return DGP_OK;
}

int run_head_pointwise(dgp_net* net, const ConvLayer& l, const float* feat, int B, int h, int w, int njt, float* out, hipStream_t s,
                       float* T, const float* feat_absmax, const H2Spec& h2 = H2Spec()) {
    const int li = (int)(&l - net->layers.data());
    const int nl = (int)net->layers.size();
    ConvArgs a = head_pointwise_args(l, feat, B, h, w, T, feat_absmax, net->d_wmax + (size_t)(nl + li) * ABSMAX_SLOTS);
    apply_h2(a, h2);
    if (h2.in_fmt == 2) a.wh3 = l.d_wh1_pw;
    a.slab = net->tail_slab; a.slab_bytes = net->tail_slab_bytes;
    const int tile_cfg = pick_tile(a.M, a.CoutP, a.nk * BK, true);
    hipError_t e;
    {
        ProfScope ps(net, s, "conv:" + l.scope + "(pointwise+gather)|" + conv_kernel_name(a, tile_cfg), conv_flops_of(l, a.M, true));
        e = launch_conv(a, tile_cfg, s);
        if (e == hipSuccess) e = launch_head_gather(T, l.d_bias, B, h, w, njt, l.coutp_pw, out, s);
    }
    if (e != hipSuccess) return fail(DGP_ERR_HIP, std::string("head (") + l.scope + "): " + hipGetErrorString(e));
    return DGP_OK;
}

int run_conv_fused_shortcut(dgp_net* net, const Unit& u, const float* r2, const float* x, int N, int H, int W, float* out,
                            hipStream_t s, const float* r2_absmax, const float* x_absmax, const H2Spec& h2 = H2Spec()) {
    const ConvLayer& l = net->layers[u.c3];
    const ConvLayer& ls = net->layers[u.sc];
    const int nl = (int)net->layers.size();
    if (!net->wmax_valid) { r2_absmax = nullptr; x_absmax = nullptr; }
    ConvArgs a{};
    apply_h2(a, h2);
    a.in = r2; a.in2 = x; a.cin_split = l.Cin; a.Cin = l.Cin + l.cin2; a.log2cin4 = 0;
    a.wpk = l.d_w_fused; a.scale = nullptr; a.bias = l.d_bias_fused; a.res = nullptr; a.out = out;
    a.N = N; a.H = H; a.W = W; a.Ho = H; a.Wo = W; a.Cout = l.Cout; a.CoutP = l.CoutP;
    a.KH = 1; a.KW = 1; a.stride = 1; a.dil = 1; a.pad_t = 0; a.pad_l = 0; a.ntaps = 1; a.nk = l.nk_fused; a.M = N * H * W;
    a.relu = 1; a.out_mode = 0;
    const double inb = (double)a.M * l.Cin * 4, in2b = (double)a.M * l.cin2 * 4, outb = (double)a.M * l.Cout * 4;
    if (!fits_descriptor({inb, in2b, outb})) return fail(DGP_ERR_INVALID, TOO_BIG);
    a.in_bytes = (unsigned)inb; a.in2_bytes = (unsigned)in2b; a.out_bytes = (unsigned)outb;
    a.w_bytes = (unsigned)((size_t)l.nk_fused * 8 * l.CoutP * 16);
    if ((r2_absmax && x_absmax) || h2.in_fmt) {
        a.in_absmax = r2_absmax; a.in2_absmax = x_absmax; a.w_absmax = net->wmax(nl + u.c3);
        a.wh3 = h2.in_fmt == 2 ? l.d_wh1_fused : l.d_wh3_fused; a.wh3_bytes = a.w_bytes;
    }
    a.out_absmax = net->amax(u.c3);
    a.slab = net->tail_slab; a.slab_bytes = net->tail_slab_bytes;
    const int tile_cfg = pick_tile(a.M, a.CoutP, a.nk * BK, (a.in_absmax || a.in_fmt) && a.w_absmax);
    ProfScope ps(net, s, "conv:" + l.scope + "+shortcut|" + conv_kernel_name(a, tile_cfg),
                 conv_flops_of(l, a.M, false) + conv_flops_of(ls, a.M, false));
    hipError_t e = launch_conv(a, tile_cfg, s);
    if (e != hipSuccess) return fail(DGP_ERR_HIP, std::string("fused conv3+shortcut (") + l.scope + "): " + hipGetErrorString(e));
    return DGP_OK;
}

struct ChainIo {
    bool h1; int N, Ho, Wo, H, W;
    const void *r2, *src2, *r1in; void *xout, *r1out;
    int r1in_exp, r2_exp, src2_exp, xout_exp, r1out_exp;
    float *r2_absmax, *xout_absmax, *r1_absmax;
};

int fill_chain_args(ChainArgs& a, const ChainPlan& cp, const ChainIo& io) {
    a.h1 = io.h1 ? 1 : 0;
    const double EB = io.h1 ? 2.0 : 4.0;
    const bool unit = io.r1in != nullptr;
    const unsigned skip = unit ? 0 : io.h1 ? cp.head_bytes_h1 : cp.head_bytes;
    a.r2 = io.r2; a.src2 = io.src2; a.xout = io.xout; a.r1out = io.r1out; a.sc1 = cp.d_sc1; a.bi1 = cp.d_bi1;
    a.wfrag = (const char*)(io.h1 ? cp.d_frags_h1 : cp.d_frags) + skip;
    a.w_bytes = (io.h1 ? cp.frag_bytes_h1 : cp.frag_bytes) - skip;
    a.M = io.N * io.Ho * io.Wo; a.HoWo = io.Ho * io.Wo; a.Wo = io.Wo; a.res_H = io.H; a.res_W = io.W;
    if (unit) {
        a.r1in = io.r1in; a.H = io.H; a.W = io.W; a.r2_absmax = io.r2_absmax;
        a.post0 = ldexpf(1.f, -(io.r1in_exp + cp.w2_exp)); a.r2_scale = ldexpf(1.f, io.r2_exp);
    }
    a.post1 = ldexpf(1.f, -(io.r2_exp + cp.w3_exp)); a.post2 = ldexpf(1.f, -(io.xout_exp + cp.w1_exp));
    a.res_inv_scale = ldexpf(1.f, -io.src2_exp); a.xout_scale = ldexpf(1.f, io.xout_exp); a.r1_scale = ldexpf(1.f, io.r1out_exp);
    a.xout_absmax = io.xout_absmax; a.r1_absmax = io.r1_absmax;
    const double r2b = (double)a.M * cp.C * EB, xob = (double)a.M * cp.C * 4 * EB, r1b = (double)a.M * cp.C1 * EB;
    const double s2b = cp.res == 0 ? (double)a.M * cp.CIN2 * EB : (double)io.N * io.H * io.W * cp.C * 4 * EB;
    const double r1inb = unit ? (double)io.N * io.H * io.W * cp.C * EB : 0.0;
    if (!fits_descriptor({r2b, xob, r1b, s2b, r1inb})) return fail(DGP_ERR_INVALID, TOO_BIG);
    a.r2_bytes = (unsigned)r2b; a.xout_bytes = (unsigned)xob; a.r1_bytes = (unsigned)r1b; a.src2_bytes = (unsigned)s2b; a.r1in_bytes = (unsigned)r1inb;
    return DGP_OK;
}

int run_chain(dgp_net* net, int ui, const float* r2, const float* x, int N, float* xout, float* r1out, hipStream_t s, int x_exp,
              const float* r1in = nullptr) {
    const ChainPlan& cp = net->chains[ui];
    const Unit &u = net->units[ui], &un = net->units[ui + 1];
    const ConvLayer &l3 = net->layers[u.c3], &l1 = net->layers[un.c1];
    const ChainIo io{net->tier != 0, N, u.ho, u.wo, u.h, u.w, r2, x, r1in, xout, r1out,
                     net->act_exp[u.c1], net->act_exp[u.c2], x_exp, net->act_exp[u.c3], net->act_exp[un.c1],
                     net->amax(u.c2), net->amax(u.c3), net->amax(un.c1)};
    ChainArgs a{};
    if (int rc = fill_chain_args(a, cp, io)) return rc;
    double flops = conv_flops_of(l3, a.M, false) + conv_flops_of(l1, a.M, false);
    if (u.sc >= 0) flops += conv_flops_of(net->layers[u.sc], a.M, false);
    if (r1in) flops += conv_flops_of(net->layers[u.c2], a.M, false);
    std::string kname = chain_kernel_name(cp.C, cp.C1, cp.CIN2, cp.res);
    if (r1in) kname = "unit" + kname.substr(5);
    if (a.h1) kname = "h1_" + kname;
    ProfScope ps(net, s, "conv:" + (r1in ? net->layers[u.c2].scope + "+" : std::string()) + l3.scope + (u.sc >= 0 ? "+shortcut" : "") + "+" + l1.scope + "|" + kname, flops);
    hipError_t e = r1in ? launch_unit(a, N, cp.C, cp.C1, cp.CIN2, cp.res, s) : launch_chain(a, cp.C, cp.C1, cp.CIN2, cp.res, s);
    if (e != hipSuccess) return fail(DGP_ERR_HIP, std::string("chain launch (") + l3.scope + "): " + hipGetErrorString(e));
    return DGP_OK;
}

struct FwdCtx {
    dgp_net* net; hipStream_t s; int B; const uint8_t* frames;
    float *P0, *C1, *X[2], *SC, *R1, *R2, *scmap_ws, *slabs;
    bool h2, calib, stem_fused, f16_mode, head_pw, fuse_on, unit_on;
    int tier, FMT;
    bool chain_tier, chain_on;
    int cur, x_exp;
    const float* x_rng;
    float *Ra, *Rb;
    bool r1_ready;

    int exp_for(float mx) const {
        return (mx > 0.f && std::isfinite(mx)) ? pow2_exp_for_max(mx) - net->h2_head : 0;
    }
    int read_range(int li, float* mx) const {
        float host[ABSMAX_SLOTS];
        HIP_TRY(hipStreamSynchronize(s));
        HIP_TRY(hipMemcpy(host, net->amax(li), sizeof host, hipMemcpyDeviceToHost));
        *mx = 0.f;
        for (float v : host) *mx = (v > *mx || v != v) ? v : *mx;
        return DGP_OK;
    }
    template <class Launch>
    int layer(int li, Launch&& launch, int forced_exp = dgp_net::H2_NONE, bool* forced_ok = nullptr) const {
        int r = launch();
        if (r || !calib) return r;
        float mx = 0.f;
        if ((r = read_range(li, &mx))) return r;
        int e = exp_for(mx);
        if (forced_exp != dgp_net::H2_NONE) {
            const bool ok = forced_exp <= e + net->h2_head - 1 && forced_exp >= e - 6;
            if (forced_ok) *forced_ok = ok;
            if (ok) e = forced_exp;
        }
        if (e != net->act_exp[li]) {
            net->act_exp[li] = e;
            HIP_TRY(hipMemsetAsync(net->amax(li), 0, ABSMAX_SLOTS * sizeof(float), s));
            r = launch();
        }
        return r;
    }
    H2Spec spec(int in_exp, int out_li, bool with_res = false, int res_exp = 0) const {
        H2Spec q;
        q.in_fmt = FMT; q.in_exp = in_exp; q.out_fmt = FMT; q.out_exp = net->act_exp[out_li]; q.res_fmt = with_res ? FMT : 0; q.res_exp = res_exp;
        return q;
    }
    bool can_fuse(int ui) const {
        const Unit& u = net->units[ui];
        return fuse_on && u.sc >= 0 && net->layers[u.c3].d_w_fused && u.stride == 1 && u.ho == u.h && u.wo == u.w && net->layers[u.c3].CoutP % 64 == 0;
    }
    int conv(int li, const ConvCall& call) const { return run_conv(net, net->layers[li], B, call, s); }
};

int fwd_context(FwdCtx& c, dgp_net* net, const uint8_t* frames, int B, char* ws, const Plan& pl, hipStream_t s) {
    static const bool h2_env = (dgp_env("DGP_H2", 1) != 0);
    static const bool head_pw = (dgp_tune("DGP_HEAD_PW", 1) != 0);
    static const bool fuse_env = (dgp_env("DGP_FUSE_SHORTCUT", 1) != 0);
    static const bool cells_env = (dgp_tune("DGP_PRESPLIT_WEIGHTS", 1) != 0);
    static const bool stem_fused_env = (dgp_tune("DGP_STEM_FUSED", 1) != 0);
    static const bool chain_env = (dgp_env("DGP_CHAIN", 1) != 0);
    static const bool chain_h1_env = (dgp_env("DGP_CHAIN_H1", 1) != 0);
    static const bool unit_env = (dgp_tune("DGP_UNIT", 1) != 0);
    c = FwdCtx{};
    c.net = net; c.s = s; c.B = B; c.frames = frames;
    c.P0 = (float*)(ws + pl.off_p0); c.C1 = (float*)(ws + pl.off_c1); c.X[0] = (float*)(ws + pl.off_x0); c.X[1] = (float*)(ws + pl.off_x1);
    c.SC = (float*)(ws + pl.off_sc); c.R1 = (float*)(ws + pl.off_r1); c.R2 = (float*)(ws + pl.off_r2);
    c.scmap_ws = (float*)(ws + pl.off_scmap); c.slabs = (float*)(ws + pl.off_slabs);
    const ConvLayer& lpart = net->layers[net->head_part];
    const ConvLayer* lloc = net->head_locref < 0 ? nullptr : &net->layers[net->head_locref];
    c.f16_mode = conv_mode() == ConvMode::F16x3 || conv_mode() == ConvMode::F16;
    c.head_pw = head_pw; c.unit_on = unit_env;
    c.fuse_on = fuse_env && conv_mode() != ConvMode::F32 && net->wmax_valid;
    c.tier = net->tier; c.FMT = c.tier ? 2 : 1;
    c.h2 = h2_env && cells_env && c.f16_mode && head_pw && net->wmax_valid && net->d_exps && lpart.d_wh3_pw && (!lloc || lloc->d_wh3_pw) &&
           net->act_exp.size() == net->layers.size();
    if (c.tier) {
        bool ok = c.h2 && lpart.d_wh1_pw && (!lloc || lloc->d_wh1_pw);
        for (const Unit& u : net->units) {
            ok = ok && net->layers[u.c1].d_wh1 && net->layers[u.c2].d_wh1 && net->layers[u.c3].d_wh1 && (u.sc < 0 || net->layers[u.sc].d_wh1);
            if (u.sc >= 0 && net->layers[u.c3].d_w_fused && !net->layers[u.c3].d_wh1_fused) ok = false;
        }
        if (!ok) return fail(DGP_ERR_STATE, "dgp_forward: the 16-bit tier needs the H2 engine's switches at their defaults (DGP_H2, DGP_PRESPLIT_WEIGHTS, "
                                            "DGP_HEAD_PW, DGP_CONV_MODE unset or f16) and weights loaded by dgp_net_load_weights");
    }
    c.calib = c.h2 && !net->h2_calibrated;
    const ConvLayer& lstem = net->layers[net->conv1];
    c.stem_fused = c.h2 && (stem_fused_env || c.tier) && lstem.d_wh3 && lstem.d_w_rows && lstem.CoutP == 64 && lstem.d_scale && lstem.d_bias;
    if (c.tier && !c.stem_fused) return fail(DGP_ERR_STATE, "dgp_forward: the 16-bit tier needs the fused root block");
    c.chain_tier = chain_env && (!c.tier || chain_h1_env);
    c.chain_on = c.h2 && !c.calib && c.chain_tier && net->chains.size() == net->units.size();
    return DGP_OK;
}

int forward_root(FwdCtx& c) {
    dgp_net* net = c.net;
    const dgp_net_desc& d = net->desc;
    const ConvLayer& lstem = net->layers[net->conv1];
    int rc;
    if (c.stem_fused) {
        rc = c.layer(net->conv1, [&] {
            ProfScope ps(net, c.s, "conv:" + lstem.scope + "+pool|stem_pool_fused", conv_flops_of(lstem, c.B * net->h1 * net->w1, false));
            hipError_t e2 = launch_stem_pool_fused(c.frames, c.B, d.in_h, d.in_w, lstem.d_wh3, net->wmax(net->conv1), lstem.d_scale, lstem.d_bias,
                                                   d.mean_pixel[0], d.mean_pixel[1], d.mean_pixel[2],
                                                   ldexpf(1.f, net->act_exp[net->conv1]), c.X[0], net->amax(net->conv1), c.s, c.tier ? 1 : 0);
            return e2 == hipSuccess ? (int)DGP_OK : fail(DGP_ERR_HIP, std::string("stem + pool: ") + hipGetErrorString(e2));
        });
        if (rc) return rc;
    } else {
        hipError_t e;
        {
            ProfScope ps(net, c.s, "preprocess_u8", 0.0);
            e = launch_preprocess(c.frames, (long long)c.B * d.in_h * d.in_w, d.mean_pixel[0], d.mean_pixel[1], d.mean_pixel[2], c.P0, c.s);
        }
        if (e != hipSuccess) return fail(DGP_ERR_HIP, std::string("preprocess: ") + hipGetErrorString(e));
        if ((rc = c.conv(net->conv1, conv_call(c.P0, d.in_h, d.in_w, c.C1).grid(net->h1, net->w1, 3, 3).range(net->d_inmax)))) return rc;
        if (c.calib) {
            float mx = 0.f;
            if ((rc = c.read_range(net->conv1, &mx))) return rc;
            net->act_exp[net->conv1] = c.exp_for(mx);
        }
        {
            ProfScope ps(net, c.s, "maxpool3x3s2", 0.0);
            e = launch_maxpool(c.C1, c.B, net->h1, net->w1, 64, c.X[0], c.s, c.h2 ? ldexpf(1.f, net->act_exp[net->conv1]) : 0.f);
        }
        if (e != hipSuccess) return fail(DGP_ERR_HIP, std::string("maxpool: ") + hipGetErrorString(e));
    }
    c.cur = 0; c.Ra = c.R1; c.Rb = c.R2; c.r1_ready = false;
    c.x_rng = net->amax(net->conv1);
    c.x_exp = c.h2 ? net->act_exp[net->conv1] : 0;
    return DGP_OK;
}

int forward_unit_f32(FwdCtx& c, int ui) {
    dgp_net* net = c.net;
    const Unit& u = net->units[ui];
    const float *xin = c.X[c.cur], *r1_rng = net->amax(u.c1), *r2_rng = net->amax(u.c2);
    float* xout = c.X[c.cur ^ 1];
    const bool fuse = c.can_fuse(ui);
    ConvCall c3 = conv_call(c.R2, u.ho, u.wo, xout).range(r2_rng).residual(xin, u.stride, u.h, u.w);
    int rc = DGP_OK;
    if (u.sc >= 0 && !fuse) {
        rc = c.conv(u.sc, conv_call(xin, u.h, u.w, c.SC).grid(u.ho, u.wo).linear().range(c.x_rng));
        c3.residual(c.SC, 1, u.ho, u.wo);
    }
    if (!rc) rc = c.conv(u.c1, conv_call(xin, u.h, u.w, c.R1).range(c.x_rng));
    if (!rc) rc = c.conv(u.c2, conv_call(c.R1, u.h, u.w, c.R2).grid(u.ho, u.wo, u.pb_h, u.pb_w).range(r1_rng));
    if (!rc) rc = fuse ? run_conv_fused_shortcut(net, u, c.R2, xin, c.B, u.h, u.w, xout, c.s, r2_rng, c.x_rng) : c.conv(u.c3, c3);
    c.x_rng = net->amax(u.c3);
    c.cur ^= 1;
    return rc;
}

int forward_unit_cells(FwdCtx& c, int ui) {
    dgp_net* net = c.net;
    const Unit& u = net->units[ui];
    const float* xin = c.X[c.cur];
    float* xout = c.X[c.cur ^ 1];
    const int x_exp = c.x_exp;
    const bool can_fuse = c.can_fuse(ui);
    bool fuse = can_fuse && (c.calib || net->unit_fuse_ok[ui]);
    int rc;
    if (!c.r1_ready) {
        rc = c.layer(u.c1, [&] { return c.conv(u.c1, conv_call(xin, u.h, u.w, c.Ra).cells(c.spec(x_exp, u.c1))); });
        if (rc) return rc;
    }
    const bool chain_ok = c.chain_on && (size_t)ui + 1 < net->units.size() && net->chains[ui].ok;
    const bool unit_k = chain_ok && c.unit_on && net->chains[ui].unit && (net->chains[ui].res != 0 || fuse);
    bool share_ok = true;
    if (!unit_k) {
        rc = c.layer(u.c2, [&] { return c.conv(u.c2, conv_call(c.Ra, u.h, u.w, c.Rb).grid(u.ho, u.wo, u.pb_h, u.pb_w).cells(c.spec(net->act_exp[u.c1], u.c2))); },
                     (fuse && c.calib) ? x_exp : dgp_net::H2_NONE, &share_ok);
        if (rc) return rc;
    }
    if (c.calib && can_fuse) { net->unit_fuse_ok[ui] = share_ok ? 1 : 0; fuse = share_ok; }
    const bool chain = chain_ok && (net->chains[ui].res != 0 || fuse);
    ConvCall c3 = conv_call(c.Rb, u.ho, u.wo, xout).residual(xin, u.stride, u.h, u.w);
    int res_exp = x_exp;
    if (u.sc >= 0 && !fuse) {
        rc = c.layer(u.sc, [&] { return c.conv(u.sc, conv_call(xin, u.h, u.w, c.SC).grid(u.ho, u.wo).linear().cells(c.spec(x_exp, u.sc))); });
        if (rc) return rc;
        c3.residual(c.SC, 1, u.ho, u.wo);
        res_exp = net->act_exp[u.sc];
    }
    if (unit_k) rc = run_chain(net, ui, nullptr, xin, c.B, xout, c.Rb, c.s, x_exp, c.Ra);
    else if (chain) rc = run_chain(net, ui, c.Rb, xin, c.B, xout, c.Ra, c.s, x_exp);
    else if (fuse)
        rc = c.layer(u.c3, [&] { return run_conv_fused_shortcut(net, u, c.Rb, xin, c.B, u.h, u.w, xout, c.s, nullptr, nullptr, c.spec(x_exp, u.c3)); });
    else
        rc = c.layer(u.c3, [&] { return c.conv(u.c3, c3.cells(c.spec(net->act_exp[u.c2], u.c3, true, res_exp))); });
    if (unit_k) std::swap(c.Ra, c.Rb);
    c.r1_ready = unit_k || chain;
    c.x_exp = net->act_exp[u.c3];
    c.x_rng = net->amax(u.c3);
    c.cur ^= 1;
    return rc;
}

int forward_heads(const FwdCtx& c, float* scmap, float* locref, float* features) {
    dgp_net* net = c.net;
    const int B = c.B, h = net->fh, w = net->fw, nj = net->desc.num_joints;
    const float* feat = c.X[c.cur];
    if (features) {
        if (c.h2) {
            const hipError_t e = c.tier ? launch_h1_to_f32(feat, (long long)B * h * w * 2048 / 8, ldexpf(1.f, -c.x_exp), features, c.s)
                                        : launch_h2_to_f32(feat, (long long)B * h * w * 2048 / 8, ldexpf(1.f, -c.x_exp), features, c.s);
            if (e != hipSuccess) return fail(DGP_ERR_HIP, std::string("features: ") + hipGetErrorString(e));
        } else
            HIP_TRY(hipMemcpyAsync(features, feat, (size_t)B * h * w * 2048 * sizeof(float), hipMemcpyDeviceToDevice, c.s));
    }
    H2Spec hs;
    if (c.h2) { hs.in_fmt = c.FMT; hs.in_exp = c.x_exp; }
    const bool pw = c.h2 || (c.head_pw && c.f16_mode && net->wmax_valid && c.x_rng && net->layers[net->head_part].d_wh3_pw);
    auto head = [&](int li, int njt, float* out) {
        const ConvLayer& l = net->layers[li];
        if (pw && l.d_wh3_pw) return run_head_pointwise(net, l, feat, B, h, w, njt, out, c.s, c.R1, c.x_rng, hs);
        ConvCall hc = conv_call(feat, h, w, out).grid(h, w, 1, 1).linear();
        hc.out_mode = 1; hc.dc_nj = njt; hc.slabs = c.slabs;
        return c.conv(li, hc);
    };
    if (int rc = head(net->head_part, nj, scmap ? scmap : c.scmap_ws)) return rc;
    return locref ? head(net->head_locref, 2 * nj, locref) : (int)DGP_OK;
}

int upload_scales(dgp_net* net, hipStream_t s) {
    std::vector<int> ex(net->layers.size(), dgp_net::H2_NONE);
    ex[net->conv1] = net->act_exp[net->conv1];
    for (const Unit& u : net->units) {
        ex[u.c1] = net->act_exp[u.c1]; ex[u.c2] = net->act_exp[u.c2]; ex[u.c3] = net->act_exp[u.c3];
        if (u.sc >= 0) ex[u.sc] = net->act_exp[u.sc];
    }
    HIP_TRY(hipStreamSynchronize(s));
    HIP_TRY(hipMemcpy(net->d_exps, ex.data(), ex.size() * sizeof(int), hipMemcpyHostToDevice));
    net->h2_calibrated = true; ++net->h2_calibrations;
    return DGP_OK;
}

int freeze_scales(const FwdCtx& c) {
    if (!c.h2) return DGP_OK;
    if (c.calib) if (int rc = upload_scales(c.net, c.s)) return rc;
    const hipError_t e = launch_h2_range_check(c.net->d_amax, c.net->d_exps, (int)c.net->layers.size(), c.net->d_flag, c.s);
    if (e != hipSuccess) return fail(DGP_ERR_HIP, std::string("range check: ") + hipGetErrorString(e));
    return DGP_OK;
}

template <class X, class Y>
int convert_cells(const std::string& who, hipError_t (*launch)(X, long long, float, Y, hipStream_t), X x, size_t n_floats, float scale, Y out, void* stream) {
    if (!x || !out || (n_floats & 7)) return fail(DGP_ERR_INVALID, who + ": null argument / length not a multiple of 8");
    const hipError_t e = launch(x, (long long)(n_floats / 8), scale, out, (hipStream_t)stream);
    return e == hipSuccess ? (int)DGP_OK : fail(DGP_ERR_HIP, who + ": " + hipGetErrorString(e));
}

}

extern "C" {

int dgp_net_workspace_bytes(const dgp_net* net, int32_t batch, size_t* out_bytes) {
    if (!net || !out_bytes || batch < 1 || batch > net->desc.max_batch)
        return fail(DGP_ERR_INVALID, "dgp_net_workspace_bytes: bad argument (batch > max_batch?)");
    *out_bytes = make_plan(net, batch).total;
    return DGP_OK;
}

int dgp_net_output_dims(const dgp_net* net, int32_t* out_h, int32_t* out_w, int32_t* feat_h, int32_t* feat_w) {
    if (!net) return fail(DGP_ERR_INVALID, "dgp_net_output_dims: null net");
    if (out_h) *out_h = 2 * net->fh;
    if (out_w) *out_w = 2 * net->fw;
    if (feat_h) *feat_h = net->fh;
    if (feat_w) *feat_w = net->fw;
    return DGP_OK;
}

int dgp_net_stats(const dgp_net* net, int32_t batch, int32_t* n_launches, double* conv_flops) {
    if (!net) return fail(DGP_ERR_INVALID, "dgp_net_stats: null net");
    double macs = (double)net->h1 * net->w1 * 49 * 3 * 64;
    int launches = 3;
    for (const Unit& u : net->units) {
        if (u.sc >= 0) { macs += (double)u.ho * u.wo * u.depth_in * u.depth; ++launches; }
        macs += (double)u.h * u.w * u.depth_in * u.depth_bn;
        macs += (double)u.ho * u.wo * 9 * u.depth_bn * u.depth_bn;
        macs += (double)u.ho * u.wo * u.depth_bn * u.depth;
        launches += 3;
    }
    const int heads = net->desc.num_joints * (net->desc.with_locref ? 3 : 1);
    macs += (double)net->fh * net->fw * 9 * 2048 * heads;
    launches += net->desc.with_locref ? 2 : 1;
    if (n_launches) *n_launches = launches;
    if (conv_flops) *conv_flops = 2.0 * macs * batch;
    return DGP_OK;
}

int dgp_forward(dgp_net* net, const uint8_t* frames, int32_t batch, void* workspace, size_t workspace_bytes,
                float* scmap, float* locref, float* features, void* stream) {
    if (!net || !frames || !workspace) return fail(DGP_ERR_INVALID, "dgp_forward: null argument");
    if (!net->loaded) return fail(DGP_ERR_STATE, "dgp_forward: weights not loaded");
    if (batch < 1 || batch > net->desc.max_batch) return fail(DGP_ERR_INVALID, "dgp_forward: batch out of range");
    const Plan pl = make_plan(net, batch);
    if (workspace_bytes < pl.total) return fail(DGP_ERR_INVALID, "dgp_forward: workspace too small");
    if (locref && net->head_locref < 0) return fail(DGP_ERR_INVALID, "dgp_forward: net built without locref head");
    if (net->owner_sync) { const int rco = net->owner_sync(net->owner, stream); if (rco) return rco; }
    hipStream_t s = (hipStream_t)stream;
    char* ws = (char*)workspace;
    for (bool again = true; again;) {
        net->prof_cursor = 0;
        net->tail_slab = (float*)(ws + pl.off_tail); net->tail_slab_bytes = (unsigned)(TAIL_SLAB_FLOATS * sizeof(float));
        if (net->d_amax) HIP_TRY(hipMemsetAsync(net->d_amax, 0, net->layers.size() * ABSMAX_SLOTS * sizeof(float), s));
        FwdCtx c;
        int rc = fwd_context(c, net, frames, batch, ws, pl, s);
        if (!rc) rc = forward_root(c);
        for (int ui = 0; !rc && ui < (int)net->units.size(); ++ui) rc = c.h2 ? forward_unit_cells(c, ui) : forward_unit_f32(c, ui);
        if (!rc) rc = forward_heads(c, scmap, locref, features);
        if (!rc) rc = freeze_scales(c);
        if (rc) return rc;
        again = c.calib && c.chain_tier;
    }
    if (net->prof_on && net->prof_used < net->prof_slots && !net->prof_in_infer) ++net->prof_used;
    return DGP_OK;
}

int dgp_soft_argmax(const float* scmap, int32_t B, int32_t H, int32_t W, int32_t C, float gamma, int32_t gauss_len,
                    float* mu, float* conf, int32_t* idx, float* pmap, void* stream) {
    if (!scmap || !mu || !conf || !idx) return fail(DGP_ERR_INVALID, "dgp_soft_argmax: null argument");
    if (B < 0 || H < 1 || W < 1 || C < 1) return fail(DGP_ERR_INVALID, "dgp_soft_argmax: bad shape");
    if (gauss_len < 1 || gauss_len > 7)
        return fail(DGP_ERR_INVALID, "dgp_soft_argmax: gauss_len must be 1..7");
    if (B == 0) return DGP_OK;
    hipError_t e = launch_soft_argmax(scmap, B, H, W, C, gamma, gauss_len, mu, conf, idx, pmap, (hipStream_t)stream);
    if (e != hipSuccess) return fail(DGP_ERR_HIP, std::string("soft_argmax: ") + hipGetErrorString(e));
    return DGP_OK;
}

int dgp_soft_argmax_locref(const float* scmap, const float* locref, int32_t B, int32_t H, int32_t W, int32_t C, float gamma,
                           int32_t gauss_len, float* mu, float* conf, int32_t* idx, float* offs, float* pmap, void* stream) {
    if (!scmap || !locref || !mu || !conf || !idx || !offs) return fail(DGP_ERR_INVALID, "dgp_soft_argmax_locref: null argument");
    if (B < 0 || H < 1 || W < 1 || C < 1) return fail(DGP_ERR_INVALID, "dgp_soft_argmax_locref: bad shape");
    if (gauss_len < 1 || gauss_len > 7)
        return fail(DGP_ERR_INVALID, "dgp_soft_argmax_locref: gauss_len must be 1..7");
    if (reinterpret_cast<uintptr_t>(locref) & 7u)
        return fail(DGP_ERR_INVALID, "dgp_soft_argmax_locref: locref must be 8-byte aligned");
// ... 220 lines not shown
int dgp_tensor_absmax(const float* x, size_t n, float* absmax_dev, void* stream) {
    if (!x || !absmax_dev) return fail(DGP_ERR_INVALID, "dgp_tensor_absmax: null argument");
    hipError_t e = launch_absmax(x, (long long)n, absmax_dev, (hipStream_t)stream);
    if (e != hipSuccess) return fail(DGP_ERR_HIP, std::string("absmax: ") + hipGetErrorString(e));
    return DGP_OK;
}

int dgp_conv2d(const dgp_conv_desc* d, const float* x, const float* packed_w, const float* scale, const float* bias,
               const float* residual, float* y, void* stream) {
    return dgp_conv2d_ranged(d, x, packed_w, scale, bias, residual, y, nullptr, nullptr, nullptr, stream);
}

int dgp_conv2d_ranged(const dgp_conv_desc* d, const float* x, const float* packed_w, const float* scale, const float* bias,
                      const float* residual, float* y, const float* x_absmax, const float* w_absmax, float* y_absmax,
                      void* stream) {
    if (!d || !x || !packed_w || !y) return fail(DGP_ERR_INVALID, "dgp_conv2d: null argument");
    if (d->Cin < 4 || (d->Cin & 3) || ((d->Cin / 4) & (d->Cin / 4 - 1)))
        return fail(DGP_ERR_INVALID, "dgp_conv2d: Cin must be 4 * 2^k");
    if (d->res_stride > 0 && !residual) return fail(DGP_ERR_INVALID, "dgp_conv2d: residual missing");
    if (d->Cout & 3) return fail(DGP_ERR_INVALID, "dgp_conv2d: Cout must be a multiple of 4");
    ConvArgs a{};
    a.in = x; a.wpk = packed_w; a.scale = scale; a.bias = bias; a.res = d->res_stride > 0 ? residual : nullptr; a.out = y;
    if (int rc = fill_conv_geometry(a, *d, "dgp_conv2d: tensor exceeds 4 GiB")) return rc;
    a.in_absmax = x_absmax; a.w_absmax = w_absmax; a.out_absmax = y_absmax;
    static const bool cells_env = (dgp_env("DGP_CONV2D_CELLS", 0) != 0);
    if (cells_env && x_absmax && w_absmax && d->Cin >= 32) {
        static void* cells = nullptr;
        static size_t cells_bytes = 0;
        if (cells_bytes < a.w_bytes) {
            if (cells) { (void)hipDeviceSynchronize(); (void)hipFree(cells); }
            if (hipMalloc(&cells, a.w_bytes) != hipSuccess) return fail(DGP_ERR_HIP, "dgp_conv2d: cell scratch");
            cells_bytes = a.w_bytes;
        }
        hipError_t pe = launch_pack_h3(packed_w, a.nk, a.CoutP, w_absmax, cells, (hipStream_t)stream);
        if (pe != hipSuccess) return fail(DGP_ERR_HIP, std::string("dgp_conv2d: pack cells: ") + hipGetErrorString(pe));
        a.wh3 = cells; a.wh3_bytes = a.w_bytes;
    }
    hipError_t e = launch_conv(a, pick_tile(a.M, a.CoutP, a.nk * BK, x_absmax && w_absmax), (hipStream_t)stream);
    if (e != hipSuccess) return fail(DGP_ERR_HIP, std::string("dgp_conv2d: ") + hipGetErrorString(e));
    return DGP_OK;
}

int dgp_f32_to_h2(const float* x, size_t n_floats, int32_t scale_exp, void* out, void* stream) {
    return convert_cells("dgp_f32_to_h2", launch_f32_to_h2, x, n_floats, ldexpf(1.f, scale_exp), out, stream);
}
int dgp_h2_to_f32(const void* x, size_t n_floats, int32_t scale_exp, float* out, void* stream) {
    return convert_cells("dgp_h2_to_f32", launch_h2_to_f32, x, n_floats, ldexpf(1.f, -scale_exp), out, stream);
}
int dgp_f32_to_h1(const float* x, size_t n_floats, int32_t scale_exp, void* out, void* stream) {
    return convert_cells("dgp_f32_to_h1", launch_f32_to_h1, x, n_floats, ldexpf(1.f, scale_exp), out, stream);
}
int dgp_h1_to_f32(const void* x, size_t n_floats, int32_t scale_exp, float* out, void* stream) {
    return convert_cells("dgp_h1_to_f32", launch_h1_to_f32, x, n_floats, ldexpf(1.f, -scale_exp), out, stream);
}

static int conv2d_cells(int fmt, const dgp_conv_desc* d, const void* x_h2, int32_t x_exp, const float* packed_w, const float* w_absmax,
                        const float* scale, const float* bias, const void* residual, int32_t res_is_h2, int32_t res_exp, void* y,
                        int32_t y_is_h2, int32_t y_exp, float* y_absmax, void* cells_scratch, void* stream) {
    if (!d || !x_h2 || !packed_w || !w_absmax || !y || !cells_scratch) return fail(DGP_ERR_INVALID, "dgp_conv2d_h2: null argument");
    if (d->Cin < 32 || (d->Cin & 7) || ((d->Cin / 4) & (d->Cin / 4 - 1)) || (d->Cout & 7))
        return fail(DGP_ERR_INVALID, "dgp_conv2d_h2: Cin must be 4 * 2^k >= 32, Cout a multiple of 8");
    if (d->res_stride > 0 && !residual) return fail(DGP_ERR_INVALID, "dgp_conv2d_h2: residual missing");
    if (d->res_stride > 0 && res_is_h2 && !y_is_h2)
        return fail(DGP_ERR_INVALID, "dgp_conv2d_h2: an H2 residual needs an H2 output (the fp32-output epilogue adds fp32 residuals only)");
    ConvArgs a{};
    a.in = (const float*)x_h2; a.wpk = packed_w; a.scale = scale; a.bias = bias; a.res = d->res_stride > 0 ? (const float*)residual : nullptr;
    a.out = (float*)y;
    if (int rc = fill_conv_geometry(a, *d, "dgp_conv2d_h2: tensor exceeds 4 GiB")) return rc;
    H2Spec h; h.in_fmt = fmt; h.in_exp = x_exp; h.out_fmt = y_is_h2 ? fmt : 0; h.out_exp = y_exp; h.res_fmt = (a.res && res_is_h2) ? fmt : 0; h.res_exp = res_exp;
    apply_h2(a, h);
    a.w_absmax = w_absmax; a.out_absmax = y_absmax;
    hipError_t pe = fmt == 2 ? launch_pack_h1(packed_w, a.nk, a.CoutP, w_absmax, cells_scratch, (hipStream_t)stream)
                             : launch_pack_h3(packed_w, a.nk, a.CoutP, w_absmax, cells_scratch, (hipStream_t)stream);
    if (pe != hipSuccess) return fail(DGP_ERR_HIP, std::string("dgp_conv2d_h2: pack cells: ") + hipGetErrorString(pe));
    a.wh3 = cells_scratch; a.wh3_bytes = a.w_bytes;
    hipError_t e = launch_conv(a, pick_tile(a.M, a.CoutP, a.nk * BK, true), (hipStream_t)stream);
    if (e != hipSuccess) return fail(DGP_ERR_HIP, std::string("dgp_conv2d_h2: ") + hipGetErrorString(e));
    return DGP_OK;
}

int dgp_conv2d_h2(const dgp_conv_desc* d, const void* x_h2, int32_t x_exp, const float* packed_w, const float* w_absmax,
                  const float* scale, const float* bias, const void* residual, int32_t res_is_h2, int32_t res_exp, void* y,
                  int32_t y_is_h2, int32_t y_exp, float* y_absmax, void* cells_scratch, void* stream) {
    return conv2d_cells(1, d, x_h2, x_exp, packed_w, w_absmax, scale, bias, residual, res_is_h2, res_exp, y, y_is_h2, y_exp, y_absmax,
                        cells_scratch, stream);
}

int dgp_conv2d_h1(const dgp_conv_desc* d, const void* x_h1, int32_t x_exp, const float* packed_w, const float* w_absmax,
                  const float* scale, const float* bias, const void* residual_h1, int32_t res_exp, void* y,
                  int32_t y_is_h1, int32_t y_exp, float* y_absmax, void* cells_scratch, void* stream) {
    if (d && (d->Cin & 63)) return fail(DGP_ERR_INVALID, "dgp_conv2d_h1: Cin must be a multiple of 64 (a K-step is 64 channels)");
    return conv2d_cells(2, d, x_h1, x_exp, packed_w, w_absmax, scale, bias, residual_h1, 1, res_exp, y, y_is_h1, y_exp, y_absmax,
                        cells_scratch, stream);
}

struct LayerWeights { const float *w2, *scale2, *bias2, *w3cat, *scale3, *bias3, *w1, *scale1, *bias1; };
static int launch_layer(const std::string& who, const ChainIo& io, int C, int C1, int CIN2, int res_mode, const LayerWeights& w, hipStream_t s) {
    const bool unit = w.w2 != nullptr;
    if (!(unit ? io.r1in : io.r2) || !io.src2 || !w.w3cat || !w.w1 || !io.xout || !io.r1out) return fail(DGP_ERR_INVALID, who + ": null argument");
    if (!(unit ? unit_supported(C, C1, CIN2, res_mode) : chain_supported(C, C1, CIN2, res_mode)))
        return fail(DGP_ERR_INVALID, who + ": no kernel instance for this (C, C1, CIN2, res_mode)");
    if (res_mode == 0 && io.src2_exp != io.r2_exp) return fail(DGP_ERR_INVALID, who + ": the K-concatenated source must share R2's scale");
    if (unit && io.r1in == io.r1out) return fail(DGP_ERR_INVALID, who + ": r1out must not alias r1 (halo reads)");
    ChainPlan cp;
    int rc = build_chain_plan(cp, C, C1, CIN2, res_mode, w.w3cat, w.scale3, w.bias3, w.w1, w.scale1, w.bias1, w.w2, w.scale2, w.bias2);
    if (rc) return rc;
    ChainArgs a{};
    rc = fill_chain_args(a, cp, io);
    hipError_t e = hipSuccess;
    if (!rc) e = unit ? launch_unit(a, io.N, C, C1, CIN2, res_mode, s) : launch_chain(a, C, C1, CIN2, res_mode, s);
    if (!rc && e == hipSuccess) e = hipStreamSynchronize(s);
    free_chain_plan(cp);
    return e != hipSuccess ? fail(DGP_ERR_HIP, who + ": " + hipGetErrorString(e)) : rc;
}

int dgp_chain_h2(int32_t N, int32_t Ho, int32_t Wo, int32_t C, int32_t C1, int32_t CIN2, int32_t res_mode, int32_t res_H, int32_t res_W,
                 const void* r2_h2, int32_t r2_exp, const void* src2_h2, int32_t src2_exp,
                 const float* w3cat, const float* scale3, const float* bias3, const float* w1, const float* scale1, const float* bias1,
                 void* xout_h2, int32_t xout_exp, void* r1_h2, int32_t r1_exp, float* xout_absmax, float* r1_absmax, void* stream) {
    const ChainIo io{false, N, Ho, Wo, res_H, res_W, r2_h2, src2_h2, nullptr, xout_h2, r1_h2, 0, r2_exp, src2_exp, xout_exp, r1_exp,
                     nullptr, xout_absmax, r1_absmax};
    return launch_layer("dgp_chain_h2", io, C, C1, CIN2, res_mode, {nullptr, nullptr, nullptr, w3cat, scale3, bias3, w1, scale1, bias1}, (hipStream_t)stream);
}
int dgp_chain_h1(int32_t N, int32_t Ho, int32_t Wo, int32_t C, int32_t C1, int32_t CIN2, int32_t res_mode, int32_t res_H, int32_t res_W,
                 const void* r2_h1, int32_t r2_exp, const void* src2_h1, int32_t src2_exp,
                 const float* w3cat, const float* scale3, const float* bias3, const float* w1, const float* scale1, const float* bias1,
                 void* xout_h1, int32_t xout_exp, void* r1_h1, int32_t r1_exp, float* xout_absmax, float* r1_absmax, void* stream) {
    const ChainIo io{true, N, Ho, Wo, res_H, res_W, r2_h1, src2_h1, nullptr, xout_h1, r1_h1, 0, r2_exp, src2_exp, xout_exp, r1_exp,
                     nullptr, xout_absmax, r1_absmax};
    return launch_layer("dgp_chain_h1", io, C, C1, CIN2, res_mode, {nullptr, nullptr, nullptr, w3cat, scale3, bias3, w1, scale1, bias1}, (hipStream_t)stream);
}
int dgp_unit_h2(int32_t N, int32_t H, int32_t W, int32_t C, int32_t C1, int32_t CIN2, int32_t res_mode,
                const void* r1_h2, int32_t r1_exp, const void* src2_h2, int32_t src2_exp,
                const float* w2, const float* scale2, const float* bias2, int32_t r2_exp,
                const float* w3cat, const float* scale3, const float* bias3, const float* w1, const float* scale1, const float* bias1,
                void* xout_h2, int32_t xout_exp, void* r1out_h2, int32_t r1out_exp, float* r2_absmax, float* xout_absmax, float* r1_absmax,
                void* stream) {
    if (!w2) return fail(DGP_ERR_INVALID, "dgp_unit_h2: null argument");
    const ChainIo io{false, N, H, W, H, W, nullptr, src2_h2, r1_h2, xout_h2, r1out_h2, r1_exp, r2_exp, src2_exp, xout_exp, r1out_exp,
                     r2_absmax, xout_absmax, r1_absmax};
    return launch_layer("dgp_unit_h2", io, C, C1, CIN2, res_mode, {w2, scale2, bias2, w3cat, scale3, bias3, w1, scale1, bias1}, (hipStream_t)stream);
}
int dgp_unit_h1(int32_t N, int32_t H, int32_t W, int32_t C, int32_t C1, int32_t CIN2, int32_t res_mode,
                const void* r1_h1, int32_t r1_exp, const void* src2_h1, int32_t src2_exp,
                const float* w2, const float* scale2, const float* bias2, int32_t r2_exp,
                const float* w3cat, const float* scale3, const float* bias3, const float* w1, const float* scale1, const float* bias1,
                void* xout_h1, int32_t xout_exp, void* r1out_h1, int32_t r1out_exp, float* r2_absmax, float* xout_absmax, float* r1_absmax,
                void* stream) {
    if (!w2) return fail(DGP_ERR_INVALID, "dgp_unit_h1: null argument");
    const ChainIo io{true, N, H, W, H, W, nullptr, src2_h1, r1_h1, xout_h1, r1out_h1, r1_exp, r2_exp, src2_exp, xout_exp, r1out_exp,
                     r2_absmax, xout_absmax, r1_absmax};
    return launch_layer("dgp_unit_h1", io, C, C1, CIN2, res_mode, {w2, scale2, bias2, w3cat, scale3, bias3, w1, scale1, bias1}, (hipStream_t)stream);
}

int dgp_net_range_status(dgp_net* net, int32_t* overflow, int32_t* calibrations, void* stream) {
    if (!net) return fail(DGP_ERR_INVALID, "dgp_net_range_status: null net");
    int flag[2] = {0, 0};
    if (net->d_flag) {
        HIP_TRY(hipStreamSynchronize((hipStream_t)stream));
        HIP_TRY(hipMemcpy(flag, net->d_flag, sizeof flag, hipMemcpyDeviceToHost));
        if (flag[0]) {
            HIP_TRY(hipMemset(net->d_flag, 0, sizeof flag));
            net->h2_calibrated = false;
            net->h2_head = std::min(net->h2_head + 3, 12);
        }
    }
    if (overflow) *overflow = flag[0] ? 1 : 0;
    if (calibrations) *calibrations = net->h2_calibrations;
    return DGP_OK;
}

int dgp_net_recalibrate(dgp_net* net) {
    if (!net) return fail(DGP_ERR_INVALID, "dgp_net_recalibrate: null net");
    net->h2_calibrated = false;
    return DGP_OK;
}

int dgp_net_widen(dgp_net* net) {
    if (!net) return fail(DGP_ERR_INVALID, "dgp_net_widen: null net");
    net->h2_calibrated = false;
    net->h2_head = std::min(net->h2_head + 3, 12);
    return DGP_OK;
}

int dgp_net_copy_scales(dgp_net* dst, const dgp_net* src, void* stream) {
    if (!dst || !src) return fail(DGP_ERR_INVALID, "dgp_net_copy_scales: null net");
    if (!src->h2_calibrated) return fail(DGP_ERR_STATE, "dgp_net_copy_scales: the source engine is not calibrated");
    if (!dst->loaded || !dst->d_exps || dst->layers.size() != src->layers.size() || dst->units.size() != src->units.size() || dst->tier != src->tier ||
        dst->desc.in_h != src->desc.in_h || dst->desc.in_w != src->desc.in_w)
        return fail(DGP_ERR_INVALID, "dgp_net_copy_scales: the engines differ (layers, tier or frame size)");
    dst->act_exp = src->act_exp;
    dst->unit_fuse_ok = src->unit_fuse_ok;
    dst->h2_head = src->h2_head;
    return upload_scales(dst, (hipStream_t)stream);
}

int dgp_net_reset_scales(dgp_net* net) {
    if (!net) return fail(DGP_ERR_INVALID, "dgp_net_reset_scales: null net");
    net->h2_calibrated = false;
    net->h2_head = 4;
    return DGP_OK;
}

int dgp_maxpool_3x3s2_same(const float* x, int32_t N, int32_t H, int32_t W, int32_t C, float* y, void* stream) {
    if (!x || !y || (C & 3)) return fail(DGP_ERR_INVALID, "dgp_maxpool_3x3s2_same: bad argument (C % 4)");
    hipError_t e = launch_maxpool(x, N, H, W, C, y, (hipStream_t)stream);
    if (e != hipSuccess) return fail(DGP_ERR_HIP, std::string("maxpool: ") + hipGetErrorString(e));
    return DGP_OK;
}

int dgp_preprocess_u8(const uint8_t* frames, int64_t n_pixels, const float mean[3], float* out_nhwc4, void* stream) {
    if (!frames || !mean || !out_nhwc4) return fail(DGP_ERR_INVALID, "dgp_preprocess_u8: null argument");
    hipError_t e = launch_preprocess(frames, n_pixels, mean[0], mean[1], mean[2], out_nhwc4, (hipStream_t)stream);
    if (e != hipSuccess) return fail(DGP_ERR_HIP, std::string("preprocess: ") + hipGetErrorString(e));
    return DGP_OK;
}

int dgp_motion_energy(const uint8_t* frames, int64_t frame_bytes, int32_t n_frames, const uint8_t* prev_frame, uint64_t* sums,
                      void* stream) {
    if (!frames || !sums || frame_bytes <= 0 || n_frames <= 0) return fail(DGP_ERR_INVALID, "dgp_motion_energy: bad argument");
    hipError_t e = launch_motion_energy(frames, frame_bytes, n_frames, prev_frame, (unsigned long long*)sums, (hipStream_t)stream);
    if (e != hipSuccess) return fail(DGP_ERR_HIP, std::string("motion energy: ") + hipGetErrorString(e));
    return DGP_OK;
}

}
```

deepgraphpose_amd/engine.py:

```python
from __future__ import annotations

import ctypes as C
from typing import Dict, NamedTuple, Optional, Tuple

import numpy as np
import torch

from . import _lib
from .arch import MEAN_PIXEL, BN_EPS


def _ptr(t: Optional[torch.Tensor]):
    return None if t is None else C.c_void_p(t.data_ptr())


def _stream(device) -> C.c_void_p:
    return C.c_void_p(torch.cuda.current_stream(device).cuda_stream)


def _need_cuda(t: torch.Tensor, dtype, name: str):
    if not t.is_cuda:
        raise _lib.DgpError("%s must be a device (cuda/HIP) tensor" % name)
    if t.dtype != dtype:
        raise _lib.DgpError("%s must have dtype %s, got %s" % (name, dtype, t.dtype))
# ... 454 lines not shown
    d = _conv_desc(x.shape, (ksize, ksize, Cin, Cout), stride, rate, pad_t, pad_l, (Ho, Wo))
    dw = torch.empty((ksize, ksize, Cin, Cout), dtype=torch.float32, device=dev)
    cs = torch.empty(2 * Cout, dtype=torch.float32, device=dev)
    rng = torch.zeros((2, ABSMAX_SLOTS), dtype=torch.float32, device=dev)
    if ranged:
        _lib.check(lib.dgp_tensor_absmax(_ptr(x), x.numel(), _ptr(rng[0]), _stream(dev)), "dgp_tensor_absmax")
        _lib.check(lib.dgp_tensor_absmax(_ptr(dy), dy.numel(), _ptr(rng[1]), _stream(dev)), "dgp_tensor_absmax")
    _lib.check(lib.dgp_conv2d_wgrad(C.byref(d), _ptr(x), _ptr(dy), _ptr(rng[0]) if ranged else None,
                                    _ptr(rng[1]) if ranged else None, _ptr(dw), _ptr(cs), _stream(dev)), "dgp_conv2d_wgrad")
    return dw, cs[:Cout]


def conv2d_wgrad_shadow(x: torch.Tensor, dy: torch.Tensor, ksize: int, stride: int = 1, rate: int = 1, pad_t: int = 0, pad_l: int = 0,
                        prev_ratio: Tuple[float, float] = (1.0, 1.0)):
    lib = _lib.load()
    _need_cuda(x, torch.float32, "x")
    _need_cuda(dy, torch.float32, "dy")
    dev = x.device
    N, H, W, Cin = x.shape
    _, Ho, Wo, Cout = dy.shape
    d = _conv_desc(x.shape, (ksize, ksize, Cin, Cout), stride, rate, pad_t, pad_l, (Ho, Wo))
    dw = torch.empty((ksize, ksize, Cin, Cout), dtype=torch.float32, device=dev)
    cs = torch.empty(2 * Cout, dtype=torch.float32, device=dev)
    rng = torch.zeros((2, ABSMAX_SLOTS), dtype=torch.float32, device=dev)
    _lib.check(lib.dgp_tensor_absmax(_ptr(x), x.numel(), _ptr(rng[0]), _stream(dev)), "dgp_tensor_absmax")
    _lib.check(lib.dgp_tensor_absmax(_ptr(dy), dy.numel(), _ptr(rng[1]), _stream(dev)), "dgp_tensor_absmax")
    prev = torch.stack([rng[0] * float(prev_ratio[0]), rng[1] * float(prev_ratio[1])]).contiguous()
    scratch = torch.empty(x.numel() + dy.numel(), dtype=torch.float32, device=dev)
    _lib.check(lib.dgp_conv2d_wgrad_shadow(C.byref(d), _ptr(x), _ptr(dy), _ptr(rng[0]), _ptr(rng[1]), _ptr(prev[0]), _ptr(prev[1]),
                                           _ptr(scratch), _ptr(dw), _ptr(cs), _stream(dev)), "dgp_conv2d_wgrad_shadow")
    return dw, cs[:Cout]


def conv2d_dgrad(dy: torch.Tensor, w_hwio: torch.Tensor, x_hw: Tuple[int, int], stride: int = 1, rate: int = 1, pad_t: int = 0,
                 pad_l: int = 0, scale: Optional[torch.Tensor] = None, mask: Optional[torch.Tensor] = None,
                 dx_add: Optional[torch.Tensor] = None, add_mode: int = 1, ranged: bool = True, mask_h2: bool = False) -> torch.Tensor:
    lib = _lib.load()
    _need_cuda(dy, torch.float32, "dy")
    _need_cuda(w_hwio, torch.float32, "w_hwio")
    dev = dy.device
    N, Ho, Wo, Cout = dy.shape
    kh, kw, Cin, _ = w_hwio.shape
    H, W = x_hw
    d = _conv_desc((N, H, W, Cin), w_hwio.shape, stride, rate, pad_t, pad_l, (Ho, Wo))
    dx = torch.empty((N, H, W, Cin), dtype=torch.float32, device=dev)
    scratch = torch.empty(lib.dgp_conv2d_dgrad_scratch_bytes(C.byref(d)), dtype=torch.uint8, device=dev)
    flags = int(bool(ranged))
    if mask_h2 and mask is not None:
        mask = f32_to_h2(mask.contiguous(), h2_exp_for(float(mask.abs().max())))
        flags |= 2
    _lib.check(lib.dgp_conv2d_dgrad(C.byref(d), _ptr(dy), _ptr(w_hwio), _ptr(scale), _ptr(mask), _ptr(dx_add), add_mode, _ptr(dx),
                                    _ptr(scratch), flags, _stream(dev)), "dgp_conv2d_dgrad")
    return dx


def h2_exp_for(absmax: float, headroom_bits: int = 4) -> int:
    import math
    if not (absmax > 0) or not math.isfinite(absmax):
        return 0
    return (14 - headroom_bits) - (math.frexp(absmax)[1] - 1)


def f32_to_h2(x: torch.Tensor, scale_exp: int) -> torch.Tensor:
    lib = _lib.load()
    _need_cuda(x, torch.float32, "x")
    out = torch.empty_like(x)
    _lib.check(lib.dgp_f32_to_h2(_ptr(x), x.numel(), int(scale_exp), _ptr(out), _stream(x.device)), "dgp_f32_to_h2")
    return out


def h2_to_f32(x: torch.Tensor, scale_exp: int) -> torch.Tensor:
    lib = _lib.load()
    _need_cuda(x, torch.float32, "x")
    out = torch.empty_like(x)
    _lib.check(lib.dgp_h2_to_f32(_ptr(x), x.numel(), int(scale_exp), _ptr(out), _stream(x.device)), "dgp_h2_to_f32")
    return out


def conv2d_h2(x_h2: torch.Tensor, x_exp: int, w_hwio: np.ndarray, stride: int = 1, rate: int = 1, pad_t: int = 0, pad_l: int = 0,
              out_hw: Optional[Tuple[int, int]] = None, scale=None, bias=None, residual: Optional[torch.Tensor] = None,
              res_stride: int = 0, res_is_h2: bool = False, res_exp: int = 0, relu: bool = False, y_is_h2: bool = True,
              y_exp: int = 0):
    lib = _lib.load()
    _need_cuda(x_h2, torch.float32, "x_h2")
    N, H, W, Cin = x_h2.shape
    kh, kw, cin2, cout = w_hwio.shape
    assert cin2 == Cin
    dev = x_h2.device
    if out_hw is None:
        keh, kew = (kh - 1) * rate + 1, (kw - 1) * rate + 1
        out_hw = ((H + 2 * pad_t - keh) // stride + 1, (W + 2 * pad_l - kew) // stride + 1)
    Ho, Wo = out_hw
    wp = torch.from_numpy(pack_conv_weights(w_hwio)).to(dev)
    sc = None if scale is None else torch.as_tensor(scale, dtype=torch.float32).contiguous().to(dev)
    bi = None if bias is None else torch.as_tensor(bias, dtype=torch.float32).contiguous().to(dev)
    y = torch.empty((N, Ho, Wo, cout), dtype=torch.float32, device=dev)
    rh, rw = (residual.shape[1], residual.shape[2]) if residual is not None else (0, 0)
    d = _lib.DgpConvDesc(N, H, W, Cin, cout, kh, kw, stride, rate, pad_t, pad_l, Ho, Wo, int(relu),
                         res_stride if residual is not None else 0, rh, rw)
    rng = torch.zeros((2, ABSMAX_SLOTS), dtype=torch.float32, device=dev)
    _lib.check(lib.dgp_tensor_absmax(_ptr(wp), wp.numel(), _ptr(rng[0]), _stream(dev)), "dgp_tensor_absmax")
    cells = torch.empty(wp.numel(), dtype=torch.float32, device=dev)
    _lib.check(lib.dgp_conv2d_h2(C.byref(d), _ptr(x_h2), int(x_exp), _ptr(wp), _ptr(rng[0]), _ptr(sc), _ptr(bi), _ptr(residual),
                                 int(res_is_h2), int(res_exp), _ptr(y), int(y_is_h2), int(y_exp), _ptr(rng[1]), _ptr(cells),
                                 _stream(dev)), "dgp_conv2d_h2")
    return y, rng[1]


def f32_to_h1(x: torch.Tensor, scale_exp: int) -> torch.Tensor:
    _need_cuda(x, torch.float32, "x")
    out = torch.empty(x.shape, dtype=torch.float16, device=x.device)
    _lib.check(_lib.load().dgp_f32_to_h1(_ptr(x), x.numel(), int(scale_exp), _ptr(out), _stream(x.device)), "dgp_f32_to_h1")
    return out


def h1_to_f32(x: torch.Tensor, scale_exp: int) -> torch.Tensor:
    _need_cuda(x, torch.float16, "x")
    out = torch.empty(x.shape, dtype=torch.float32, device=x.device)
    _lib.check(_lib.load().dgp_h1_to_f32(_ptr(x), x.numel(), int(scale_exp), _ptr(out), _stream(x.device)), "dgp_h1_to_f32")
    return out


def conv2d_h1(x_h1: torch.Tensor, x_exp: int, w_hwio: np.ndarray, stride: int = 1, rate: int = 1, pad_t: int = 0, pad_l: int = 0,
              out_hw: Optional[Tuple[int, int]] = None, scale=None, bias=None, residual: Optional[torch.Tensor] = None,
              res_stride: int = 0, res_exp: int = 0, relu: bool = False, y_is_h1: bool = True, y_exp: int = 0):
    lib = _lib.load()
    _need_cuda(x_h1, torch.float16, "x_h1")
    N, H, W, Cin = x_h1.shape
    kh, kw, cin2, cout = w_hwio.shape
    assert cin2 == Cin
    dev = x_h1.device
    if out_hw is None:
        keh, kew = (kh - 1) * rate + 1, (kw - 1) * rate + 1
        out_hw = ((H + 2 * pad_t - keh) // stride + 1, (W + 2 * pad_l - kew) // stride + 1)
    Ho, Wo = out_hw
    wp = torch.from_numpy(pack_conv_weights(w_hwio)).to(dev)
    sc = None if scale is None else torch.as_tensor(scale, dtype=torch.float32).contiguous().to(dev)
    bi = None if bias is None else torch.as_tensor(bias, dtype=torch.float32).contiguous().to(dev)
    y = torch.empty((N, Ho, Wo, cout), dtype=torch.float16 if y_is_h1 else torch.float32, device=dev)
    if residual is not None:
        _need_cuda(residual, torch.float16, "residual")
    rh, rw = (residual.shape[1], residual.shape[2]) if residual is not None else (0, 0)
    d = _lib.DgpConvDesc(N, H, W, Cin, cout, kh, kw, stride, rate, pad_t, pad_l, Ho, Wo, int(relu),
                         res_stride if residual is not None else 0, rh, rw)
    rng = torch.zeros((2, ABSMAX_SLOTS), dtype=torch.float32, device=dev)
    _lib.check(lib.dgp_tensor_absmax(_ptr(wp), wp.numel(), _ptr(rng[0]), _stream(dev)), "dgp_tensor_absmax")
    cells = torch.empty(wp.numel(), dtype=torch.float16, device=dev)
    _lib.check(lib.dgp_conv2d_h1(C.byref(d), _ptr(x_h1), int(x_exp), _ptr(wp), _ptr(rng[0]), _ptr(sc), _ptr(bi), _ptr(residual),
                                 int(res_exp), _ptr(y), int(y_is_h1), int(y_exp), _ptr(rng[1]), _ptr(cells), _stream(dev)),
               "dgp_conv2d_h1")
    return y, rng[1]


def chain_h2(r2_h2: torch.Tensor, r2_exp: int, src2_h2: torch.Tensor, src2_exp: int, w3cat: np.ndarray, scale3, bias3,
             w1: np.ndarray, scale1, bias1, res_mode: int, xout_exp: int, r1_exp: int, h1: bool = False):
    lib = _lib.load()
    dt = torch.float16 if h1 else torch.float32
    _need_cuda(r2_h2, dt, "r2_h2")
    _need_cuda(src2_h2, dt, "src2_h2")
    N, Ho, Wo, Cc = r2_h2.shape
    K, C4 = w3cat.shape
    C1 = w1.shape[1]
    assert C4 == 4 * Cc and w1.shape[0] == C4
    cin2 = K - Cc
    dev = r2_h2.device
    xo = torch.empty((N, Ho, Wo, C4), dtype=dt, device=dev)
    r1 = torch.empty((N, Ho, Wo, C1), dtype=dt, device=dev)
    rng = torch.zeros((2, ABSMAX_SLOTS), dtype=torch.float32, device=dev)
    f = lambda a: None if a is None else np.ascontiguousarray(a, dtype=np.float32)
    w3c, s3, b3, w1c, s1, b1 = f(w3cat), f(scale3), f(bias3), f(w1), f(scale1), f(bias1)
    hp = lambda a: None if a is None else a.ctypes.data_as(C.c_void_p)
    _lib.check((lib.dgp_chain_h1 if h1 else lib.dgp_chain_h2)(N, Ho, Wo, Cc, C1, cin2, int(res_mode), src2_h2.shape[1], src2_h2.shape[2], _ptr(r2_h2), int(r2_exp),
                                _ptr(src2_h2), int(src2_exp), hp(w3c), hp(s3), hp(b3), hp(w1c), hp(s1), hp(b1), _ptr(xo), int(xout_exp),
                                _ptr(r1), int(r1_exp), _ptr(rng[0]), _ptr(rng[1]), _stream(dev)), "dgp_chain_h2")
    return xo, r1, rng[0], rng[1]


def unit_h2(r1_h2: torch.Tensor, r1_exp: int, src2_h2: torch.Tensor, src2_exp: int, w2: np.ndarray, scale2, bias2, r2_exp: int,
            w3cat: np.ndarray, scale3, bias3, w1: np.ndarray, scale1, bias1, res_mode: int, xout_exp: int, r1out_exp: int, h1: bool = False):
    lib = _lib.load()
    dt = torch.float16 if h1 else torch.float32
    _need_cuda(r1_h2, dt, "r1_h2")
    _need_cuda(src2_h2, dt, "src2_h2")
    N, H, W, Cc = r1_h2.shape
    K, C4 = w3cat.shape
    C1 = w1.shape[1]
    assert C4 == 4 * Cc and w1.shape[0] == C4 and w2.shape == (3, 3, Cc, Cc)
    cin2 = K - Cc
    dev = r1_h2.device
    xo = torch.empty((N, H, W, C4), dtype=dt, device=dev)
    r1o = torch.empty((N, H, W, C1), dtype=dt, device=dev)
    rng = torch.zeros((3, ABSMAX_SLOTS), dtype=torch.float32, device=dev)
    f = lambda a: None if a is None else np.ascontiguousarray(a, dtype=np.float32)
    arrs = [f(a) for a in (w2, scale2, bias2, w3cat, scale3, bias3, w1, scale1, bias1)]
    hp = lambda a: None if a is None else a.ctypes.data_as(C.c_void_p)
    _lib.check((lib.dgp_unit_h1 if h1 else lib.dgp_unit_h2)(N, H, W, Cc, C1, cin2, int(res_mode), _ptr(r1_h2), int(r1_exp), _ptr(src2_h2), int(src2_exp),
                               hp(arrs[0]), hp(arrs[1]), hp(arrs[2]), int(r2_exp), hp(arrs[3]), hp(arrs[4]), hp(arrs[5]), hp(arrs[6]),
                               hp(arrs[7]), hp(arrs[8]), _ptr(xo), int(xout_exp), _ptr(r1o), int(r1out_exp), _ptr(rng[0]), _ptr(rng[1]),
                               _ptr(rng[2]), _stream(dev)), "dgp_unit_h2")
    return xo, r1o, rng[0], rng[1], rng[2]


def maxpool_3x3s2_same(x: torch.Tensor) -> torch.Tensor:
    lib = _lib.load()
    _need_cuda(x, torch.float32, "x")
    N, H, W, Cn = x.shape
    y = torch.empty((N, (H + 1) // 2, (W + 1) // 2, Cn), dtype=torch.float32, device=x.device)
    _lib.check(lib.dgp_maxpool_3x3s2_same(_ptr(x), N, H, W, Cn, _ptr(y), _stream(x.device)), "dgp_maxpool")
    return y


def preprocess_u8(frames: torch.Tensor, mean=MEAN_PIXEL) -> torch.Tensor:
    lib = _lib.load()
    _need_cuda(frames, torch.uint8, "frames")
    out = torch.empty(tuple(frames.shape[:-1]) + (4,), dtype=torch.float32, device=frames.device)
    m = (C.c_float * 3)(*mean)
    _lib.check(lib.dgp_preprocess_u8(_ptr(frames), frames.numel() // 3, m, _ptr(out), _stream(frames.device)),
               "dgp_preprocess_u8")
    return out


def motion_energy(frames: torch.Tensor, prev: Optional[torch.Tensor] = None) -> np.ndarray:
    lib = _lib.load()
    _need_cuda(frames, torch.uint8, "frames")
    frames = frames.contiguous()
    T = frames.shape[0]
    fb = frames.numel() // max(T, 1)
    if T == 0:
        return np.zeros(0, dtype=np.float64)
    if prev is not None:
        _need_cuda(prev, torch.uint8, "prev")
        prev = prev.contiguous()
        if prev.numel() != fb:
            raise _lib.DgpError("motion_energy: prev has %d bytes, a frame has %d" % (prev.numel(), fb))
    sums = torch.empty(T, dtype=torch.int64, device=frames.device)
    _lib.check(lib.dgp_motion_energy(_ptr(frames), fb, T, _ptr(prev), _ptr(sums), _stream(frames.device)), "dgp_motion_energy")
    return sums.cpu().numpy().astype(np.float64) / float(fb)


FLOW_OUTPUTS = ("magnitude", "flow", "both")


def optical_flow(frames: torch.Tensor, *, pyr_scale: float = 0.5, levels: int = 3, winsize: int = 15, iterations: int = 3,
                 poly_n: int = 5, poly_sigma: float = 1.2, output: str = "magnitude"):
    lib = _lib.load()
    if output not in FLOW_OUTPUTS:
        raise ValueError("optical_flow: output must be one of %s, not %r" % ("|".join(FLOW_OUTPUTS), output))
    _need_cuda(frames, torch.uint8, "frames")
    if frames.dim() != 4 or frames.shape[-1] != 3:
        raise _lib.DgpError("optical_flow: frames must be [T, H, W, 3], got %s" % (tuple(frames.shape),))
    T, H, W = (int(v) for v in frames.shape[:3])
    P = max(T - 1, 0)
    dev = frames.device
    mag = torch.empty((P, H, W), dtype=torch.float32, device=dev) if output in ("magnitude", "both") else None
    flow = torch.empty((P, H, W, 2), dtype=torch.float32, device=dev) if output in ("flow", "both") else None
    if P > 0:
        prm = _lib.DgpFlowParams(float(pyr_scale), int(levels), int(winsize), int(iterations), int(poly_n), float(poly_sigma), 0)
        nb, used = C.c_size_t(), C.c_int32()
        _lib.check(lib.dgp_optical_flow_scratch_bytes(T, H, W, C.byref(prm), C.byref(nb), C.byref(used)), "dgp_optical_flow_scratch_bytes")
        scratch = torch.empty(nb.value, dtype=torch.uint8, device=dev)
        _lib.check(lib.dgp_optical_flow(_ptr(frames), T, H, W, C.byref(prm), _ptr(flow), _ptr(mag), _ptr(scratch), nb.value,
                                        _stream(dev)), "dgp_optical_flow")
    if output == "magnitude":
        return mag
    if output == "flow":
        return flow
    return mag, flow


_RESIZE_PLANS: Dict[tuple, tuple] = {}


def resize_plan(in_size: int, out_size: int) -> Tuple[int, np.ndarray, np.ndarray]:
    lib = _lib.load()
    ks = C.c_int32()
    _lib.check(lib.dgp_resize_plan_size(int(in_size), int(out_size), C.byref(ks)), "dgp_resize_plan_size")
    bounds = np.empty((int(out_size), 2), np.int32)
    coeffs = np.empty((int(out_size), ks.value), np.int32)
    _lib.check(lib.dgp_resize_plan(int(in_size), int(out_size), bounds.ctypes.data_as(C.c_void_p), coeffs.ctypes.data_as(C.c_void_p)),
               "dgp_resize_plan")
    return ks.value, bounds, coeffs


def _device_resize_plans(dev, H: int, W: int, rh: int, rw: int):
    key = (str(dev), H, W, rh, rw)
    if key not in _RESIZE_PLANS:
        plans = []
        for n_in, n_out in ((W, rw), (H, rh)):
            ks, bounds, coeffs = resize_plan(n_in, n_out)
            plans.append((torch.from_numpy(np.concatenate([bounds.ravel(), coeffs.ravel()])).to(dev), ks))
        if len(_RESIZE_PLANS) >= 16:
            old = next(iter(_RESIZE_PLANS))
            torch.cuda.synchronize(_RESIZE_PLANS[old][0].device)
            del _RESIZE_PLANS[old]
        _RESIZE_PLANS[key] = (plans[0][0], plans[1][0], plans[0][1], plans[1][1])
    return _RESIZE_PLANS[key]


def resize_output_shape(H: int, W: int, new_size=None, crop_size=None) -> Tuple[int, int]:
    oh, ow = (int(new_size[0]), int(new_size[1])) if new_size is not None else (int(H), int(W))
    if crop_size is not None:
        l, u, r, b = (int(round(v)) for v in crop_size)
        oh, ow = b - u, r - l
    return oh, ow


def resize_frames(frames: torch.Tensor, new_size=None, crop_size=None, out: Optional[torch.Tensor] = None) -> torch.Tensor:
    lib = _lib.load()
    _need_cuda(frames, torch.uint8, "frames")
    if frames.dim() != 4 or frames.shape[-1] != 3:
        raise _lib.DgpError("resize_frames: frames must be [B, H, W, 3], got %s" % (tuple(frames.shape),))
    if new_size is not None and len(new_size) != 2:
        raise ValueError("resize_frames: new_size must be (rows, cols), not %r" % (new_size,))
    if crop_size is not None and len(crop_size) != 4:
        raise ValueError("resize_frames: crop_size must be (left, upper, right, lower), not %r" % (crop_size,))
    B, H, W = (int(v) for v in frames.shape[:3])
    rh, rw = (int(new_size[0]), int(new_size[1])) if new_size is not None else (H, W)
    oh, ow = resize_output_shape(H, W, new_size, crop_size)
    if min(rh, rw, oh, ow) <= 0:
        raise ValueError("resize_frames: empty result for new_size %r, crop_size %r" % (new_size, crop_size))
    dev = frames.device
    if out is None:
        out = torch.empty((B, oh, ow, 3), dtype=torch.uint8, device=dev)
    else:
        _need_cuda(out, torch.uint8, "out")
        if tuple(out.shape) != (B, oh, ow, 3) or out.device != dev:
            raise _lib.DgpError("resize_frames: out must be %s on %s, got %s on %s" % ((B, oh, ow, 3), dev, tuple(out.shape), out.device))
    plan_x, plan_y, ksx, ksy = _device_resize_plans(dev, H, W, rh, rw)
    box = (C.c_int32 * 4)(*(int(round(v)) for v in crop_size)) if crop_size is not None else None
    _lib.check(lib.dgp_resize_crop_u8(_ptr(frames), B, H, W, rh, rw, box, _ptr(out), _ptr(plan_x), _ptr(plan_y), ksx, ksy, _stream(dev)),
               "dgp_resize_crop_u8")
    return out


RESIZE_FILTERS = {"box": 4, "bilinear": 2, "bicubic": 3}


def _filter_id(filter) -> int:
    if filter in RESIZE_FILTERS:
        return RESIZE_FILTERS[filter]
    if filter in RESIZE_FILTERS.values():
        return int(filter)
    raise ValueError("resize filter must be one of %s, not %r" % ("|".join(RESIZE_FILTERS), filter))


def resize_plan_f(in_size: int, out_size: int, filter) -> Tuple[int, np.ndarray, np.ndarray]:
    lib = _lib.load()
    fid = _filter_id(filter)
    ks = C.c_int32()
    _lib.check(lib.dgp_resize_plan_size_f(int(in_size), int(out_size), fid, C.byref(ks)), "dgp_resize_plan_size_f")
    bounds = np.empty((int(out_size), 2), np.int32)
    coeffs = np.empty((int(out_size), ks.value), np.int32)
# ... 280 lines not shown
```

include/dgp_hip.h:

```cpp
#ifndef DGP_HIP_H
#define DGP_HIP_H

#include <stddef.h>
#include <stdint.h>

#ifdef __cplusplus
extern "C" {
#endif

#define DGP_ABI_VERSION 1

typedef enum dgp_status {
    DGP_OK = 0,
    DGP_ERR_INVALID = -1,
    DGP_ERR_HIP = -2,
    DGP_ERR_MISSING = -3,
    DGP_ERR_STATE = -4
} dgp_status;

typedef struct dgp_net dgp_net;

typedef struct dgp_net_desc {
    int32_t depth;
    int32_t num_joints;
// ... 25 lines not shown
int  dgp_net_stats(const dgp_net* net, int32_t batch, int32_t* n_launches, double* conv_flops);

int  dgp_forward(dgp_net* net, const uint8_t* frames, int32_t batch, void* workspace,
                 size_t workspace_bytes, float* scmap, float* locref, float* features,
                 void* stream);

int  dgp_soft_argmax(const float* scmap, int32_t B, int32_t H, int32_t W, int32_t C,
                     float gamma, int32_t gauss_len, float* mu, float* conf, int32_t* idx,
                     float* pmap, void* stream);

int  dgp_soft_argmax_locref(const float* scmap, const float* locref, int32_t B, int32_t H, int32_t W, int32_t C,
                            float gamma, int32_t gauss_len, float* mu, float* conf, int32_t* idx, float* offs,
                            float* pmap, void* stream);

int  dgp_pmap_threshold(float* pmap, int32_t B, int32_t H, int32_t W, int32_t C, float th, float* mu, void* stream);

int  dgp_hard_argmax(const float* scmap, const float* locref, int32_t B, int32_t H, int32_t W,
                     int32_t C, int32_t* idx, float* prob, float* offs, void* stream);

int  dgp_infer(dgp_net* net, const uint8_t* frames, int32_t batch, void* workspace,
               size_t workspace_bytes, float gamma, int32_t gauss_len, float* mu, float* conf,
               int32_t* idx, float* scmap_out, void* stream);

int  dgp_infer_packed(dgp_net* net, const uint8_t* frames, int32_t batch, void* workspace,
                      size_t workspace_bytes, float gamma, int32_t gauss_len, float* traj,
                      float* scmap_out, void* stream);

int  dgp_infer_packed_locref(dgp_net* net, const uint8_t* frames, int32_t batch, void* workspace,
                             size_t workspace_bytes, float gamma, int32_t gauss_len, int32_t mode, float* traj,
                             float* scmap_out, float* locref_out, void* stream);

int  dgp_net_set_input_size(dgp_net* net, int32_t in_h, int32_t in_w);

int  dgp_net_profile_begin(dgp_net* net, int32_t max_steps);
int  dgp_net_profile_end(dgp_net* net, int32_t* n_steps, int32_t* n_launches);
int  dgp_net_profile_launch(dgp_net* net, int32_t launch, char* name, int32_t name_cap,
                            double* flops, double* avg_ms);

typedef struct dgp_loss_desc {
    int32_t nt, H, W, nj, nl;
    int32_t n_visible, n_hidden;
    int32_t gm2, gm3;
    int32_t gauss_len, huber;
    float   gamma, lengthscale, stride;
    float   wn_visible, wn_hidden, locref_loss_weight;
    float   n_frames_total, n_visible_frames_total;
    int32_t use_wt, Hin, Win;
    float   wt_max;
} dgp_loss_desc;

int  dgp_loss_scratch_bytes(const dgp_loss_desc* d, size_t* out_bytes);
int  dgp_loss_fwd_bwd(const dgp_loss_desc* d, const float* pred, const float* locref_pred, const float* targets,
                      const float* locref_map, const float* locref_mask, const int32_t* visible_marker,
                      const int32_t* hidden_marker, const int32_t* visible_in_targets, const float* S0,
                      const float* ws, const float* ws_max, const float* vector_field ,
                      const float* wt_batch , float* dpred, float* dlocref,
                      float* mu, float* losses, void* scratch, size_t scratch_bytes, void* stream);

int  dgp_dlc_loss_fwd_bwd(const float* pred, const float* locref_pred, const float* part_targets,
                          const float* part_weights, const float* locref_targets, const float* locref_mask, int32_t nt,
                          int32_t H, int32_t W, int32_t nj, float locref_loss_weight, int32_t huber, float* dpred,
                          float* dlocref, float* losses, void* scratch, size_t scratch_bytes, void* stream);

typedef struct dgp_trainer dgp_trainer;
int    dgp_trainer_create(dgp_net* net, dgp_trainer** out);
void   dgp_trainer_destroy(dgp_trainer* tr);
int    dgp_trainer_num_tensors(const dgp_trainer* tr, int32_t* n_tensors, int64_t* n_trainable_floats,
                               int64_t* n_stat_floats);
int    dgp_trainer_tensor_info(const dgp_trainer* tr, int32_t i, char* name, int32_t cap, int64_t* offset,
                               int64_t* size, int32_t* is_stat);
float* dgp_trainer_buffer(dgp_trainer* tr, int32_t which);
int    dgp_trainer_upload(dgp_trainer* tr, int32_t which, int64_t offset, const float* host, int64_t n);
int    dgp_trainer_download(dgp_trainer* tr, int32_t which, int64_t offset, float* host, int64_t n);
int    dgp_trainer_workspace_bytes(const dgp_trainer* tr, int32_t nt, size_t* out_bytes);
int    dgp_trainer_sync_weights(dgp_trainer* tr, void* stream);
int    dgp_train_forward(dgp_trainer* tr, const uint8_t* frames, int32_t nt, void* workspace, size_t workspace_bytes,
                         float** scmap, float** locref, void* stream);
int    dgp_train_backward(dgp_trainer* tr, int32_t nt, void* workspace, size_t workspace_bytes, const float* dscmap,
                          const float* dlocref, void* stream);
int    dgp_sgd_momentum_clip(dgp_trainer* tr, float lr, float momentum, float clip_norm, float* gnorm_host_or_null,
                             void* stream);
int    dgp_adam_clip(dgp_trainer* tr, float lr, float beta1, float beta2, float eps, float clip_norm, float* gnorm_host_or_null,
                     void* stream);
int    dgp_trainer_set_tier(dgp_trainer* tr, int32_t tier);
int    dgp_trainer_get_tier(const dgp_trainer* tr);
int    dgp_trainer_grad_groups(dgp_trainer* tr, int32_t max_groups, int32_t* n_groups, int64_t* lo, int64_t* hi);
int    dgp_trainer_grad_group_wait(dgp_trainer* tr, int32_t k, void* stream);
int    dgp_trainer_fast_mode(dgp_trainer* tr, int32_t enable);
int    dgp_trainer_fast_status(dgp_trainer* tr, int32_t* was_fast, int32_t* failed);
int    dgp_trainer_step_status(dgp_trainer* tr, const float* d_losses, int32_t n_losses, float* losses, float* gnorm,
                               int32_t* was_fast, int32_t* failed, void* stream);


typedef struct dgp_conv_desc {
    int32_t N, H, W, Cin;
    int32_t Cout;
    int32_t KH, KW, stride, rate;
    int32_t pad_t, pad_l;
    int32_t Ho, Wo;
    int32_t relu;
    int32_t res_stride;
    int32_t res_H, res_W;
} dgp_conv_desc;

size_t dgp_packed_weight_floats(int32_t KH, int32_t KW, int32_t Cin, int32_t Cout);
int  dgp_pack_conv_weights(const float* hwio, int32_t KH, int32_t KW, int32_t Cin,
                           int32_t Cout, float* packed);
int  dgp_conv2d(const dgp_conv_desc* d, const float* x, const float* packed_w,
                const float* scale , const float* bias ,
                const float* residual, float* y, void* stream);
#define DGP_ABSMAX_SLOTS 256
int  dgp_conv2d_ranged(const dgp_conv_desc* d, const float* x, const float* packed_w, const float* scale, const float* bias,
                       const float* residual, float* y, const float* x_absmax, const float* w_absmax, float* y_absmax,
                       void* stream);
int    dgp_conv2d_wgrad(const dgp_conv_desc* d, const float* x, const float* dy, const float* x_absmax, const float* dy_absmax,
                        float* dw_raw, float* colsum, void* stream);
int    dgp_conv2d_wgrad_shadow(const dgp_conv_desc* d, const float* x, const float* dy, const float* x_absmax, const float* dy_absmax,
                               const float* x_prev, const float* dy_prev, void* scratch, float* dw_raw, float* colsum, void* stream);
size_t dgp_conv2d_dgrad_scratch_bytes(const dgp_conv_desc* d);
int    dgp_conv2d_dgrad(const dgp_conv_desc* d, const float* dy, const float* w_hwio, const float* scale, const float* mask,
                        const float* dx_add, int32_t add_mode, float* dx, void* scratch, int32_t ranged, void* stream);
int  dgp_f32_to_h2(const float* x, size_t n_floats, int32_t scale_exp, void* out, void* stream);
int  dgp_h2_to_f32(const void* x, size_t n_floats, int32_t scale_exp, float* out, void* stream);
int  dgp_conv2d_h2(const dgp_conv_desc* d, const void* x_h2, int32_t x_exp, const float* packed_w, const float* w_absmax,
                   const float* scale, const float* bias, const void* residual, int32_t res_is_h2, int32_t res_exp, void* y,
                   int32_t y_is_h2, int32_t y_exp, float* y_absmax, void* cells_scratch, void* stream);
int  dgp_net_set_tier(dgp_net* net, int32_t tier);
int  dgp_net_get_tier(const dgp_net* net);
int  dgp_f32_to_h1(const float* x, size_t n_floats, int32_t scale_exp, void* out, void* stream);
int  dgp_h1_to_f32(const void* x, size_t n_floats, int32_t scale_exp, float* out, void* stream);
int  dgp_conv2d_h1(const dgp_conv_desc* d, const void* x_h1, int32_t x_exp, const float* packed_w, const float* w_absmax,
                   const float* scale, const float* bias, const void* residual_h1, int32_t res_exp, void* y,
                   int32_t y_is_h1, int32_t y_exp, float* y_absmax, void* cells_scratch, void* stream);
int  dgp_chain_h2(int32_t N, int32_t Ho, int32_t Wo, int32_t C, int32_t C1, int32_t CIN2, int32_t res_mode, int32_t res_H, int32_t res_W,
                  const void* r2_h2, int32_t r2_exp, const void* src2_h2, int32_t src2_exp,
                  const float* w3cat, const float* scale3, const float* bias3, const float* w1, const float* scale1, const float* bias1,
                  void* xout_h2, int32_t xout_exp, void* r1_h2, int32_t r1_exp, float* xout_absmax, float* r1_absmax, void* stream);
int  dgp_unit_h2(int32_t N, int32_t H, int32_t W, int32_t C, int32_t C1, int32_t CIN2, int32_t res_mode,
                 const void* r1_h2, int32_t r1_exp, const void* src2_h2, int32_t src2_exp,
                 const float* w2, const float* scale2, const float* bias2, int32_t r2_exp,
                 const float* w3cat, const float* scale3, const float* bias3, const float* w1, const float* scale1, const float* bias1,
                 void* xout_h2, int32_t xout_exp, void* r1out_h2, int32_t r1out_exp, float* r2_absmax, float* xout_absmax, float* r1_absmax,
                 void* stream);
int  dgp_chain_h1(int32_t N, int32_t Ho, int32_t Wo, int32_t C, int32_t C1, int32_t CIN2, int32_t res_mode, int32_t res_H, int32_t res_W,
                  const void* r2_h1, int32_t r2_exp, const void* src2_h1, int32_t src2_exp,
                  const float* w3cat, const float* scale3, const float* bias3, const float* w1, const float* scale1, const float* bias1,
                  void* xout_h1, int32_t xout_exp, void* r1_h1, int32_t r1_exp, float* xout_absmax, float* r1_absmax, void* stream);
int  dgp_unit_h1(int32_t N, int32_t H, int32_t W, int32_t C, int32_t C1, int32_t CIN2, int32_t res_mode,
                 const void* r1_h1, int32_t r1_exp, const void* src2_h1, int32_t src2_exp,
                 const float* w2, const float* scale2, const float* bias2, int32_t r2_exp,
                 const float* w3cat, const float* scale3, const float* bias3, const float* w1, const float* scale1, const float* bias1,
                 void* xout_h1, int32_t xout_exp, void* r1out_h1, int32_t r1out_exp, float* r2_absmax, float* xout_absmax, float* r1_absmax,
                 void* stream);
int  dgp_net_range_status(dgp_net* net, int32_t* overflow, int32_t* calibrations, void* stream);
int  dgp_net_recalibrate(dgp_net* net);
int  dgp_net_widen(dgp_net* net);
int  dgp_net_reset_scales(dgp_net* net);
int  dgp_net_copy_scales(dgp_net* dst, const dgp_net* src, void* stream);

int  dgp_tensor_absmax(const float* x, size_t n, float* absmax_dev, void* stream);
int  dgp_maxpool_3x3s2_same(const float* x, int32_t N, int32_t H, int32_t W, int32_t C,
                            float* y, void* stream);
int  dgp_preprocess_u8(const uint8_t* frames, int64_t n_pixels, const float mean[3],
                       float* out_nhwc4, void* stream);
int  dgp_motion_energy(const uint8_t* frames, int64_t frame_bytes, int32_t n_frames, const uint8_t* prev_frame,
                       uint64_t* sums, void* stream);

typedef struct dgp_flow_params {
    double  pyr_scale;
    int32_t levels, winsize, iterations, poly_n;
    double  poly_sigma;
    int32_t flags;
} dgp_flow_params;

int  dgp_optical_flow_scratch_bytes(int32_t n_frames, int32_t H, int32_t W, const dgp_flow_params* p, size_t* bytes,
                                    int32_t* levels_used);
int  dgp_optical_flow(const uint8_t* frames, int32_t n_frames, int32_t H, int32_t W, const dgp_flow_params* p, float* flow,
                      float* magnitude, void* scratch, size_t scratch_bytes, void* stream);


int  dgp_resize_plan_size(int32_t in_size, int32_t out_size, int32_t* ksize);
int  dgp_resize_plan(int32_t in_size, int32_t out_size, int32_t* bounds, int32_t* coeffs);
int  dgp_resize_crop_u8(const uint8_t* src, int32_t B, int32_t H, int32_t W, int32_t RH, int32_t RW, const int32_t* box, uint8_t* dst,
                        const int32_t* d_plan_x, const int32_t* d_plan_y, int32_t ksize_x, int32_t ksize_y, void* stream);

enum { DGP_FILTER_BILINEAR = 2, DGP_FILTER_BICUBIC = 3, DGP_FILTER_BOX = 4 };
int  dgp_resize_plan_size_f(int32_t in_size, int32_t out_size, int32_t filter, int32_t* ksize);
int  dgp_resize_plan_f(int32_t in_size, int32_t out_size, int32_t filter, int32_t* bounds, int32_t* coeffs);
int  dgp_window_resize_u8(const uint8_t* src, int32_t src_H, int32_t src_W, int32_t x0, int32_t y0, int32_t x1, int32_t y1,
                          int32_t RH, int32_t RW, int32_t filter, int32_t mirror, uint8_t* dst, const int32_t* d_plan_x,
                          const int32_t* d_plan_y, int32_t ksize_x, int32_t ksize_y, void* stream);

int  dgp_target_maps(const double* d_entries, const int32_t* d_offsets, const double* h_entries, const int32_t* h_offsets,
                     int32_t n_frames, int32_t H, int32_t W, int32_t nj, double stride, double pos_dist_thresh, double scale,
                     double locref_stdev, int32_t weigh_only_present_joints, float* scmap, float* weights, float* lmap, float* lmask,
                     void* stream);

int  dgp_gather_frames_u8(const uint8_t* store, int64_t n_slots, int64_t slot_stride, const uint8_t* patch, int32_t m,
                          const int32_t* h_src, int32_t nt, int64_t frame_bytes, uint8_t* out, void* stream);

int  dgp_aug_affine_u8(const uint8_t* src, uint8_t* dst, int32_t H, int32_t W, const double* coef, void* stream);
int  dgp_aug_blur3_u8(const uint8_t* src, uint8_t* dst, int32_t H, int32_t W, const float* k, void* stream);
int  dgp_aug_dropout_u8(const uint8_t* src, uint8_t* dst, int32_t H, int32_t W, const uint8_t* d_mask, int32_t h, int32_t w, void* stream);
int  dgp_aug_elastic_u8(const uint8_t* src, uint8_t* dst, int32_t H, int32_t W, const float* d_field, int32_t hc, int32_t wc, void* stream);
int  dgp_aug_noise_u8(const uint8_t* src, uint8_t* dst, int32_t H, int32_t W, float scale, int32_t per_channel, uint64_t key, void* stream);

#ifdef __cplusplus
}
#endif
#endif
```

Before: 4754.

## Skip writing unused odd-position xout pixels before stride-2 identity units

When the next unit has stride 2 and an identity shortcut, only even (ho,wo) positions of the chained xout tensor are later read. The fused chain/unit kernels now compute a per-wave ballot mask and redirect stores for odd positions out of bounds, and whole waves on odd rows skip the store. The intent is to cut xout write bandwidth by roughly three quarters at those units. The cost is extra index arithmetic per tile, and the buffer keeps unwritten garbage at odd positions, which is only safe if no other consumer reads them.

```diff
diff --git a/deepgraphpose_amd/_lib.py b/deepgraphpose_amd/_lib.py
--- a/deepgraphpose_amd/_lib.py
+++ b/deepgraphpose_amd/_lib.py
@@ -96,6 +96,8 @@
     "dgp_unit_h2": (C.c_int, [_i32] * 7 + [_vp, _i32, _vp, _i32] + [_vp] * 3 + [_i32] + [_vp] * 6 + [_vp, _i32, _vp, _i32, _vp, _vp, _vp, _vp]),
     "dgp_chain_h1": (C.c_int, [_i32] * 9 + [_vp, _i32, _vp, _i32] + [_vp] * 6 + [_vp, _i32, _vp, _i32, _vp, _vp, _vp]),
     "dgp_unit_h1": (C.c_int, [_i32] * 7 + [_vp, _i32, _vp, _i32] + [_vp] * 3 + [_i32] + [_vp] * 6 + [_vp, _i32, _vp, _i32, _vp, _vp, _vp, _vp]),
+    "dgp_chain_xkeep": (C.c_int, [_i32] * 11 + [_vp, _i32, _vp, _i32] + [_vp] * 6 + [_vp, _i32, _vp, _i32, _vp, _vp, _vp]),
+    "dgp_unit_xkeep": (C.c_int, [_i32] * 9 + [_vp, _i32, _vp, _i32] + [_vp] * 3 + [_i32] + [_vp] * 6 + [_vp, _i32, _vp, _i32, _vp, _vp, _vp, _vp]),
     "dgp_net_range_status": (C.c_int, [_vp, C.POINTER(_i32), C.POINTER(_i32), _vp]),
     "dgp_net_recalibrate": (C.c_int, [_vp]),
     "dgp_net_reset_scales": (C.c_int, [_vp]),
diff --git a/deepgraphpose_amd/arch.py b/deepgraphpose_amd/arch.py
--- a/deepgraphpose_amd/arch.py
+++ b/deepgraphpose_amd/arch.py
@@ -127,7 +127,14 @@
             if (ui, "conv3") not in have:
                 total += pout * u.depth_bottleneck
         elif which == "conv3":
-            total += u.depth_bottleneck * u.depth + pout * u.depth
+            total += u.depth_bottleneck * u.depth
+            un = plan[ui + 1] if ui + 2 < len(plan) else None
+            if (ui + 1, "conv1") in have and un is not None and un.stride == 2 and not un.has_shortcut_conv:
+                pin_n, pout_n = geo[ui + 1]
+                assert pin_n == pout
+                total += pout_n * u.depth
+            else:
+                total += pout * u.depth
             if (ui, "conv2") not in have:
                 total += pout * u.depth_bottleneck
             if (ui, "shortcut") in have:
diff --git a/deepgraphpose_amd/csrc/dgp_chain.hip b/deepgraphpose_amd/csrc/dgp_chain.hip
--- a/deepgraphpose_amd/csrc/dgp_chain.hip
+++ b/deepgraphpose_amd/csrc/dgp_chain.hip
@@ -70,7 +70,8 @@
 template <int C, int C1, int CIN2, int RES, int RB, int NS, int PD, int CHUNK, int WR, bool H1 = false>
 __device__ __forceinline__ void chain_tail(const ChainArgs& p, const uint4* ring, int& slot, const uint4 (&ph)[RB][(C + CIN2) / 32],
                                            const uint4 (&pl)[RB][(C + CIN2) / 32], const unsigned (&xoff)[RB], const unsigned (&roff)[RB],
-                                           const unsigned (&r1off)[RB], const __amdgpu_buffer_rsrc_t rs_s2, const __amdgpu_buffer_rsrc_t rs_xo,
+                                           const unsigned (&r1off)[RB], const unsigned long long (&xkeep)[RB], const bool xwave,
+                                           const __amdgpu_buffer_rsrc_t rs_s2, const __amdgpu_buffer_rsrc_t rs_xo,
                                            const __amdgpu_buffer_rsrc_t rs_r1, float& amax_x, float& amax_r1, const int lane,
                                            uint4 (&res)[PD][RB][2] UD_PARAM) {
 #ifdef DGP_DIAG
@@ -144,12 +145,15 @@
                 }
                 if constexpr (H1) { xh[rb] = h1_pack8(o, p.xout_scale); xl[rb] = xh[rb]; }
                 else h2_pack8(o, p.xout_scale, xh[rb], xl[rb]);
-                if (p.nt & 2) {
-                    st16nt(rs_xo, xh[rb], xoff[rb], jp * CB);
-                    if constexpr (!H1) st16nt(rs_xo, xl[rb], xoff[rb], jp * CB + 16);
-                } else {
-                    st16(rs_xo, xh[rb], xoff[rb], jp * CB);
-                    if constexpr (!H1) st16(rs_xo, xl[rb], xoff[rb], jp * CB + 16);
+                if (xwave) {
+                    const unsigned so = __builtin_amdgcn_inverse_ballot_w64(xkeep[rb]) ? xoff[rb] : OOB;
+                    if (p.nt & 2) {
+                        st16nt(rs_xo, xh[rb], so, jp * CB);
+                        if constexpr (!H1) st16nt(rs_xo, xl[rb], so, jp * CB + 16);
+                    } else {
+                        st16(rs_xo, xh[rb], so, jp * CB);
+                        if constexpr (!H1) st16(rs_xo, xl[rb], so, jp * CB + 16);
+                    }
                 }
                 if (xoff[rb] != OOB) {
 #pragma unroll
@@ -294,6 +298,19 @@
     __builtin_amdgcn_s_barrier();
     for (int t = blockIdx.x; t < p.ntiles; t += gridDim.x) {
         unsigned xoff[RB], roff[RB], r1off[RB];
+        unsigned long long xkeep[RB];
+#pragma unroll
+        for (int rb = 0; rb < RB; ++rb) xkeep[rb] = ~0ull;
+        if (p.xkeep == 2) {
+            unsigned HoWo = (unsigned)p.HoWo, Wo = (unsigned)p.Wo;
+            asm volatile("" : "+s"(HoWo), "+s"(Wo));
+#pragma unroll
+            for (int rb = 0; rb < RB; ++rb) {
+                const unsigned m = (unsigned)(t * TILE + (wave * RB + rb) * 16 + l15);
+                const unsigned rem = m % HoWo, ho = rem / Wo, wo = rem - ho * Wo;
+                xkeep[rb] = __builtin_amdgcn_ballot_w64(((ho | wo) & 1) == 0);
+            }
+        }
         uint4 ph[RB][KS1], pl[RB][KS1];
 #pragma unroll
         for (int rb = 0; rb < RB; ++rb) {
@@ -325,7 +342,7 @@
 #ifdef DGP_DIAG
         unsigned long long ud[12] = {0};
 #endif
-        chain_tail<C, C1, CIN2, RES, RB, NS, PD, CHUNK, WR, H1>(p, ring, slot, ph, pl, xoff, roff, r1off, rs_s2, rs_xo, rs_r1, amax_x, amax_r1, lane, res UD_ARG);
+        chain_tail<C, C1, CIN2, RES, RB, NS, PD, CHUNK, WR, H1>(p, ring, slot, ph, pl, xoff, roff, r1off, xkeep, true, rs_s2, rs_xo, rs_r1, amax_x, amax_r1, lane, res UD_ARG);
 #ifdef DGP_DIAG
         if (wave == 0 && lane == 0) {
             for (int i = 4; i < 9; ++i) atomicAdd(&g_unit_diag[i], ud[i]);
@@ -498,6 +515,9 @@
         xoff[0] = ok ? (unsigned)m * (unsigned)(C4 * EB) + (unsigned)(g * 8 * EB) : OOB;
         roff[0] = xoff[0];
         r1off[0] = ok ? (unsigned)m * (unsigned)(C1 * EB) + (unsigned)(g * 8 * EB) : OOB;
+        const bool xsub = p.xkeep == 2;
+        const bool xwave = !(xsub && (y & 1));
+        const unsigned long long xkeep[1] = {xsub ? __builtin_amdgcn_ballot_w64((x & 1) == 0) : ~0ull};
         uint4 ph[1][KS1], pl[1][KS1];
         if constexpr (CIN2 > 0) {
             const unsigned boff = ok ? (unsigned)m * (unsigned)(CIN2 * EB) + (unsigned)(g * 8 * EB) : OOB;
@@ -596,7 +616,7 @@
 #ifdef DGP_DIAG
         ud[2] += u1 - u0; ud[9] += 1;
 #endif
-        chain_tail<C, C1, CIN2, RES, 1, NS, PD, CHUNK, WR, H1>(p, ring, slot, ph, pl, xoff, roff, r1off, rs_s2, rs_xo, rs_r1, amax_x, amax_r1, lane, res UD_ARG);
+        chain_tail<C, C1, CIN2, RES, 1, NS, PD, CHUNK, WR, H1>(p, ring, slot, ph, pl, xoff, roff, r1off, xkeep, xwave, rs_s2, rs_xo, rs_r1, amax_x, amax_r1, lane, res UD_ARG);
     }
 #ifdef DGP_DIAG
     UD_STAMP(uend);
diff --git a/deepgraphpose_amd/csrc/dgp_internal.h b/deepgraphpose_amd/csrc/dgp_internal.h
--- a/deepgraphpose_amd/csrc/dgp_internal.h
+++ b/deepgraphpose_amd/csrc/dgp_internal.h
@@ -156,6 +156,7 @@
     float* r2_absmax;
     int nt;
     int h1;
+    int xkeep;
 };
 bool chain_supported(int C, int C1, int CIN2, int res);
 int  chain_frags_per_chunk(int C, int C1, int CIN2, int planes = 2);
diff --git a/deepgraphpose_amd/csrc/dgp_net.hip b/deepgraphpose_amd/csrc/dgp_net.hip
--- a/deepgraphpose_amd/csrc/dgp_net.hip
+++ b/deepgraphpose_amd/csrc/dgp_net.hip
@@ -683,6 +683,7 @@
     const void *r2, *src2, *r1in; void *xout, *r1out;
     int r1in_exp, r2_exp, src2_exp, xout_exp, r1out_exp;
     float *r2_absmax, *xout_absmax, *r1_absmax;
+    int xkeep;
 };
 
 int fill_chain_args(ChainArgs& a, const ChainPlan& cp, const ChainIo& io) {
@@ -701,6 +702,7 @@
     a.post1 = ldexpf(1.f, -(io.r2_exp + cp.w3_exp)); a.post2 = ldexpf(1.f, -(io.xout_exp + cp.w1_exp));
     a.res_inv_scale = ldexpf(1.f, -io.src2_exp); a.xout_scale = ldexpf(1.f, io.xout_exp); a.r1_scale = ldexpf(1.f, io.r1out_exp);
     a.xout_absmax = io.xout_absmax; a.r1_absmax = io.r1_absmax;
+    a.xkeep = io.xkeep;
     const double r2b = (double)a.M * cp.C * EB, xob = (double)a.M * cp.C * 4 * EB, r1b = (double)a.M * cp.C1 * EB;
     const double s2b = cp.res == 0 ? (double)a.M * cp.CIN2 * EB : (double)io.N * io.H * io.W * cp.C * 4 * EB;
     const double r1inb = unit ? (double)io.N * io.H * io.W * cp.C * EB : 0.0;
@@ -710,13 +712,13 @@
 }
 
 int run_chain(dgp_net* net, int ui, const float* r2, const float* x, int N, float* xout, float* r1out, hipStream_t s, int x_exp,
-              const float* r1in = nullptr) {
+              const float* r1in = nullptr, int xkeep = 1) {
     const ChainPlan& cp = net->chains[ui];
     const Unit &u = net->units[ui], &un = net->units[ui + 1];
     const ConvLayer &l3 = net->layers[u.c3], &l1 = net->layers[un.c1];
     const ChainIo io{net->tier != 0, N, u.ho, u.wo, u.h, u.w, r2, x, r1in, xout, r1out,
                      net->act_exp[u.c1], net->act_exp[u.c2], x_exp, net->act_exp[u.c3], net->act_exp[un.c1],
-                     net->amax(u.c2), net->amax(u.c3), net->amax(un.c1)};
+                     net->amax(u.c2), net->amax(u.c3), net->amax(un.c1), xkeep};
     ChainArgs a{};
     if (int rc = fill_chain_args(a, cp, io)) return rc;
     double flops = conv_flops_of(l3, a.M, false) + conv_flops_of(l1, a.M, false);
@@ -737,6 +739,7 @@
     bool h2, calib, stem_fused, f16_mode, head_pw, fuse_on, unit_on;
     int tier, FMT;
     bool chain_tier, chain_on;
+    bool xsub_on;
     int cur, x_exp;
     const float* x_rng;
     float *Ra, *Rb;
@@ -793,6 +796,7 @@
     static const bool chain_env = (dgp_env("DGP_CHAIN", 1) != 0);
     static const bool chain_h1_env = (dgp_env("DGP_CHAIN_H1", 1) != 0);
     static const bool unit_env = (dgp_tune("DGP_UNIT", 1) != 0);
+    static const bool xsub_env = (dgp_env("DGP_XOUT_SUBSAMPLE", 1) != 0);
     c = FwdCtx{};
     c.net = net; c.s = s; c.B = B; c.frames = frames;
     c.P0 = (float*)(ws + pl.off_p0); c.C1 = (float*)(ws + pl.off_c1); c.X[0] = (float*)(ws + pl.off_x0); c.X[1] = (float*)(ws + pl.off_x1);
@@ -801,7 +805,7 @@
     const ConvLayer& lpart = net->layers[net->head_part];
     const ConvLayer* lloc = net->head_locref < 0 ? nullptr : &net->layers[net->head_locref];
     c.f16_mode = conv_mode() == ConvMode::F16x3 || conv_mode() == ConvMode::F16;
-    c.head_pw = head_pw; c.unit_on = unit_env;
+    c.head_pw = head_pw; c.unit_on = unit_env; c.xsub_on = xsub_env;
     c.fuse_on = fuse_env && conv_mode() != ConvMode::F32 && net->wmax_valid;
     c.tier = net->tier; c.FMT = c.tier ? 2 : 1;
     c.h2 = h2_env && cells_env && c.f16_mode && head_pw && net->wmax_valid && net->d_exps && lpart.d_wh3_pw && (!lloc || lloc->d_wh3_pw) &&
@@ -914,8 +918,13 @@
         c3.residual(c.SC, 1, u.ho, u.wo);
         res_exp = net->act_exp[u.sc];
     }
-    if (unit_k) rc = run_chain(net, ui, nullptr, xin, c.B, xout, c.Rb, c.s, x_exp, c.Ra);
-    else if (chain) rc = run_chain(net, ui, c.Rb, xin, c.B, xout, c.Ra, c.s, x_exp);
+    int xkeep = 1;
+    if ((unit_k || chain) && c.xsub_on && (size_t)ui + 2 < net->units.size()) {
+        const Unit& un = net->units[ui + 1];
+        if (un.stride == 2 && un.sc < 0) xkeep = 2;
+    }
+    if (unit_k) rc = run_chain(net, ui, nullptr, xin, c.B, xout, c.Rb, c.s, x_exp, c.Ra, xkeep);
+    else if (chain) rc = run_chain(net, ui, c.Rb, xin, c.B, xout, c.Ra, c.s, x_exp, nullptr, xkeep);
     else if (fuse)
         rc = c.layer(u.c3, [&] { return run_conv_fused_shortcut(net, u, c.Rb, xin, c.B, u.h, u.w, xout, c.s, nullptr, nullptr, c.spec(x_exp, u.c3)); });
     else
@@ -1442,6 +1451,27 @@
                      r2_absmax, xout_absmax, r1_absmax};
     return launch_layer("dgp_unit_h1", io, C, C1, CIN2, res_mode, {w2, scale2, bias2, w3cat, scale3, bias3, w1, scale1, bias1}, (hipStream_t)stream);
 }
+int dgp_chain_xkeep(int32_t h1, int32_t xout_keep, int32_t N, int32_t Ho, int32_t Wo, int32_t C, int32_t C1, int32_t CIN2, int32_t res_mode,
+                    int32_t res_H, int32_t res_W, const void* r2, int32_t r2_exp, const void* src2, int32_t src2_exp,
+                    const float* w3cat, const float* scale3, const float* bias3, const float* w1, const float* scale1, const float* bias1,
+                    void* xout, int32_t xout_exp, void* r1, int32_t r1_exp, float* xout_absmax, float* r1_absmax, void* stream) {
+    if (xout_keep != 1 && xout_keep != 2) return fail(DGP_ERR_INVALID, "dgp_chain_xkeep: xout_keep must be 1 or 2");
+    const ChainIo io{h1 != 0, N, Ho, Wo, res_H, res_W, r2, src2, nullptr, xout, r1, 0, r2_exp, src2_exp, xout_exp, r1_exp,
+                     nullptr, xout_absmax, r1_absmax, xout_keep};
+    return launch_layer("dgp_chain_xkeep", io, C, C1, CIN2, res_mode, {nullptr, nullptr, nullptr, w3cat, scale3, bias3, w1, scale1, bias1}, (hipStream_t)stream);
+}
+int dgp_unit_xkeep(int32_t h1, int32_t xout_keep, int32_t N, int32_t H, int32_t W, int32_t C, int32_t C1, int32_t CIN2, int32_t res_mode,
+                   const void* r1, int32_t r1_exp, const void* src2, int32_t src2_exp,
+                   const float* w2, const float* scale2, const float* bias2, int32_t r2_exp,
+                   const float* w3cat, const float* scale3, const float* bias3, const float* w1, const float* scale1, const float* bias1,
+                   void* xout, int32_t xout_exp, void* r1out, int32_t r1out_exp, float* r2_absmax, float* xout_absmax, float* r1_absmax,
+                   void* stream) {
+    if (xout_keep != 1 && xout_keep != 2) return fail(DGP_ERR_INVALID, "dgp_unit_xkeep: xout_keep must be 1 or 2");
+    if (!w2) return fail(DGP_ERR_INVALID, "dgp_unit_xkeep: null argument");
+    const ChainIo io{h1 != 0, N, H, W, H, W, nullptr, src2, r1, xout, r1out, r1_exp, r2_exp, src2_exp, xout_exp, r1out_exp,
+                     r2_absmax, xout_absmax, r1_absmax, xout_keep};
+    return launch_layer("dgp_unit_xkeep", io, C, C1, CIN2, res_mode, {w2, scale2, bias2, w3cat, scale3, bias3, w1, scale1, bias1}, (hipStream_t)stream);
+}
 
 int dgp_net_range_status(dgp_net* net, int32_t* overflow, int32_t* calibrations, void* stream) {
     if (!net) return fail(DGP_ERR_INVALID, "dgp_net_range_status: null net");
diff --git a/deepgraphpose_amd/engine.py b/deepgraphpose_amd/engine.py
--- a/deepgraphpose_amd/engine.py
+++ b/deepgraphpose_amd/engine.py
@@ -630,8 +630,17 @@
     return y, rng[1]
 
 
+def _xout_buffer(xout, shape, dt, dev) -> torch.Tensor:
+    if xout is None:
+        return torch.empty(shape, dtype=dt, device=dev)
+    _need_cuda(xout, dt, "xout")
+    assert tuple(xout.shape) == tuple(shape) and xout.is_contiguous() and xout.device == dev
+    return xout
+
+
 def chain_h2(r2_h2: torch.Tensor, r2_exp: int, src2_h2: torch.Tensor, src2_exp: int, w3cat: np.ndarray, scale3, bias3,
-             w1: np.ndarray, scale1, bias1, res_mode: int, xout_exp: int, r1_exp: int, h1: bool = False):
+             w1: np.ndarray, scale1, bias1, res_mode: int, xout_exp: int, r1_exp: int, h1: bool = False, xout_keep: int = 1,
+             xout: Optional[torch.Tensor] = None):
     lib = _lib.load()
     dt = torch.float16 if h1 else torch.float32
     _need_cuda(r2_h2, dt, "r2_h2")
@@ -642,20 +651,25 @@
     assert C4 == 4 * Cc and w1.shape[0] == C4
     cin2 = K - Cc
     dev = r2_h2.device
-    xo = torch.empty((N, Ho, Wo, C4), dtype=dt, device=dev)
+    xo = _xout_buffer(xout, (N, Ho, Wo, C4), dt, dev)
     r1 = torch.empty((N, Ho, Wo, C1), dtype=dt, device=dev)
     rng = torch.zeros((2, ABSMAX_SLOTS), dtype=torch.float32, device=dev)
     f = lambda a: None if a is None else np.ascontiguousarray(a, dtype=np.float32)
     w3c, s3, b3, w1c, s1, b1 = f(w3cat), f(scale3), f(bias3), f(w1), f(scale1), f(bias1)
     hp = lambda a: None if a is None else a.ctypes.data_as(C.c_void_p)
-    _lib.check((lib.dgp_chain_h1 if h1 else lib.dgp_chain_h2)(N, Ho, Wo, Cc, C1, cin2, int(res_mode), src2_h2.shape[1], src2_h2.shape[2], _ptr(r2_h2), int(r2_exp),
-                                _ptr(src2_h2), int(src2_exp), hp(w3c), hp(s3), hp(b3), hp(w1c), hp(s1), hp(b1), _ptr(xo), int(xout_exp),
-                                _ptr(r1), int(r1_exp), _ptr(rng[0]), _ptr(rng[1]), _stream(dev)), "dgp_chain_h2")
+    args = (N, Ho, Wo, Cc, C1, cin2, int(res_mode), src2_h2.shape[1], src2_h2.shape[2], _ptr(r2_h2), int(r2_exp),
+            _ptr(src2_h2), int(src2_exp), hp(w3c), hp(s3), hp(b3), hp(w1c), hp(s1), hp(b1), _ptr(xo), int(xout_exp),
+            _ptr(r1), int(r1_exp), _ptr(rng[0]), _ptr(rng[1]), _stream(dev))
+    if xout_keep == 1:
+        _lib.check((lib.dgp_chain_h1 if h1 else lib.dgp_chain_h2)(*args), "dgp_chain_h2")
+    else:
+        _lib.check(lib.dgp_chain_xkeep(int(h1), int(xout_keep), *args), "dgp_chain_xkeep")
     return xo, r1, rng[0], rng[1]
 
 
 def unit_h2(r1_h2: torch.Tensor, r1_exp: int, src2_h2: torch.Tensor, src2_exp: int, w2: np.ndarray, scale2, bias2, r2_exp: int,
-            w3cat: np.ndarray, scale3, bias3, w1: np.ndarray, scale1, bias1, res_mode: int, xout_exp: int, r1out_exp: int, h1: bool = False):
+            w3cat: np.ndarray, scale3, bias3, w1: np.ndarray, scale1, bias1, res_mode: int, xout_exp: int, r1out_exp: int, h1: bool = False,
+            xout_keep: int = 1, xout: Optional[torch.Tensor] = None):
     lib = _lib.load()
     dt = torch.float16 if h1 else torch.float32
     _need_cuda(r1_h2, dt, "r1_h2")
@@ -666,16 +680,20 @@
     assert C4 == 4 * Cc and w1.shape[0] == C4 and w2.shape == (3, 3, Cc, Cc)
     cin2 = K - Cc
     dev = r1_h2.device
-    xo = torch.empty((N, H, W, C4), dtype=dt, device=dev)
+    xo = _xout_buffer(xout, (N, H, W, C4), dt, dev)
     r1o = torch.empty((N, H, W, C1), dtype=dt, device=dev)
     rng = torch.zeros((3, ABSMAX_SLOTS), dtype=torch.float32, device=dev)
     f = lambda a: None if a is None else np.ascontiguousarray(a, dtype=np.float32)
     arrs = [f(a) for a in (w2, scale2, bias2, w3cat, scale3, bias3, w1, scale1, bias1)]
     hp = lambda a: None if a is None else a.ctypes.data_as(C.c_void_p)
-    _lib.check((lib.dgp_unit_h1 if h1 else lib.dgp_unit_h2)(N, H, W, Cc, C1, cin2, int(res_mode), _ptr(r1_h2), int(r1_exp), _ptr(src2_h2), int(src2_exp),
-                               hp(arrs[0]), hp(arrs[1]), hp(arrs[2]), int(r2_exp), hp(arrs[3]), hp(arrs[4]), hp(arrs[5]), hp(arrs[6]),
-                               hp(arrs[7]), hp(arrs[8]), _ptr(xo), int(xout_exp), _ptr(r1o), int(r1out_exp), _ptr(rng[0]), _ptr(rng[1]),
-                               _ptr(rng[2]), _stream(dev)), "dgp_unit_h2")
+    args = (N, H, W, Cc, C1, cin2, int(res_mode), _ptr(r1_h2), int(r1_exp), _ptr(src2_h2), int(src2_exp),
+            hp(arrs[0]), hp(arrs[1]), hp(arrs[2]), int(r2_exp), hp(arrs[3]), hp(arrs[4]), hp(arrs[5]), hp(arrs[6]),
+            hp(arrs[7]), hp(arrs[8]), _ptr(xo), int(xout_exp), _ptr(r1o), int(r1out_exp), _ptr(rng[0]), _ptr(rng[1]),
+            _ptr(rng[2]), _stream(dev))
+    if xout_keep == 1:
+        _lib.check((lib.dgp_unit_h1 if h1 else lib.dgp_unit_h2)(*args), "dgp_unit_h2")
+    else:
+        _lib.check(lib.dgp_unit_xkeep(int(h1), int(xout_keep), *args), "dgp_unit_xkeep")
     return xo, r1o, rng[0], rng[1], rng[2]
 
 
diff --git a/include/dgp_hip.h b/include/dgp_hip.h
--- a/include/dgp_hip.h
+++ b/include/dgp_hip.h
@@ -201,6 +201,16 @@
                  const float* w3cat, const float* scale3, const float* bias3, const float* w1, const float* scale1, const float* bias1,
                  void* xout_h1, int32_t xout_exp, void* r1out_h1, int32_t r1out_exp, float* r2_absmax, float* xout_absmax, float* r1_absmax,
                  void* stream);
+int  dgp_chain_xkeep(int32_t h1, int32_t xout_keep, int32_t N, int32_t Ho, int32_t Wo, int32_t C, int32_t C1, int32_t CIN2, int32_t res_mode,
+                     int32_t res_H, int32_t res_W, const void* r2, int32_t r2_exp, const void* src2, int32_t src2_exp,
+                     const float* w3cat, const float* scale3, const float* bias3, const float* w1, const float* scale1, const float* bias1,
+                     void* xout, int32_t xout_exp, void* r1, int32_t r1_exp, float* xout_absmax, float* r1_absmax, void* stream);
+int  dgp_unit_xkeep(int32_t h1, int32_t xout_keep, int32_t N, int32_t H, int32_t W, int32_t C, int32_t C1, int32_t CIN2, int32_t res_mode,
+                    const void* r1, int32_t r1_exp, const void* src2, int32_t src2_exp,
+                    const float* w2, const float* scale2, const float* bias2, int32_t r2_exp,
+                    const float* w3cat, const float* scale3, const float* bias3, const float* w1, const float* scale1, const float* bias1,
+                    void* xout, int32_t xout_exp, void* r1out, int32_t r1out_exp, float* r2_absmax, float* xout_absmax, float* r1_absmax,
+                    void* stream);
 int  dgp_net_range_status(dgp_net* net, int32_t* overflow, int32_t* calibrations, void* stream);
 int  dgp_net_recalibrate(dgp_net* net);
 int  dgp_net_widen(dgp_net* net);
```

Measured after the change: 4816, median of 6. +1.3%, better.
